# jeffpeterson/hypermerge

Hardware: AMD Instinct MI355X
Metric: merged changes/sec (1M docs×8 actors) at 1/2/4/8 GPUs + % HBM roofline (higher is better)
Workload: dtype u32; 1 GPU; C4: 1000000 docs/GPU x 8 actors x 64 changes/doc, map LWW sets; docs_per_gpu=1000000, changes_per_gpu=64000000, ops_per_gpu=96000538, parallelism=doc-shard1

## Files before the change

hypermerge_amd/csrc/engine.cpp:

```cpp
#include <hip/hip_runtime.h>
#include <cstdio>
#include <cstring>
#include <cstdlib>
#include <string>
#include <vector>
#include <algorithm>
#include <new>
#include "../../include/hypermerge_amd.h"
#include "merge_kernels.h"
#include "engine_internal.h"
#include "waiting_kernels.h"

struct hm_engine {
    int device = 0;
    int flags = 0;
    hipStream_t stream = nullptr;
    hipEvent_t ev[4] = {};
    float last_ms[2] = {0, 0};
    int n_last = 0;
    int num_cus = 256;
    std::string err;
    void *dbuf = nullptr;
    size_t dbuf_size = 0;
    void *pool = nullptr;
    size_t pool_size = 0;
    hipStream_t h2d = nullptr, d2h = nullptr;
    const char *last_scratch = nullptr;
};

namespace {

int fail(hm_engine *e, int status, const std::string &msg) {
    if (e) e->err = msg;
    return status;
}

int hip_fail(hm_engine *e, hipError_t r, const char *what) {
    return fail(e, HM_ERR_DEVICE, std::string(what) + ": " + hipGetErrorString(r));
}

#define HIPCHK(e, call)                                   \
    do {                                                  \
        hipError_t _r = (call);                           \
        if (_r != hipSuccess) return hip_fail(e, _r, #call); \
    } while (0)

struct Caps { uint32_t opl, cls; bool lists, counters; };

Caps launch_caps(const hm_batch *b) {
    Caps c;
    uint32_t mo = b->max_ops;
    c.opl = mo <= 64 ? 1 : (mo <= 128 ? 2 : (mo <= 192 ? 3 : 4));
    c.cls = (b->max_regs && b->max_objs && b->max_deps) ? hm_small_class(b->max_regs, b->max_objs, b->max_deps) : 1u;
    c.lists = (b->doc_flags & HM_DOC_HAS_LISTS) != 0;
    c.counters = (b->doc_flags & HM_DOC_HAS_COUNTERS) != 0;
    return c;
}

int launch_merge(hm_engine *e, const hm_batch *b, const hm_results *o, hipStream_t s, const uint32_t *doc_slot,
                 const hm_extents *ext, void *scratch, uint32_t *epos = nullptr) {
    Caps c = launch_caps(b);
    SmallParams p;
    p.res_epos = epos;
    p.docs = b->docs; p.changes = b->changes; p.deps = b->deps; p.ops = b->ops; p.min_clock = b->min_clock;
    p.res_docs = o->docs; p.res_clock = o->clock; p.res_back_clock = o->back_clock; p.res_heads = o->heads;
    p.res_hist = o->hist; p.res_all_deps = o->all_deps; p.res_regs = o->regs; p.res_surv = o->surv;
    p.n_docs = b->n_docs; p.a_stride = b->a_stride; p.cap_regs = 0; p.cap_objs = 0; p.cap_deps = 0;
    p.counters = c.counters ? 1u : 0u;
    p.general_only = (e->flags & HM_CFG_GENERAL_ONLY) ? 1u : 0u;
    {
        static const int remap = [] { const char *v = getenv("HM_XCD_REMAP"); return v ? atoi(v) : 1; }();
        p.xcd_remap = remap ? 1u : 0u;
    }
    p.doc_slot = doc_slot;
    p.lim_changes = ext ? ext->n_changes : b->n_changes; p.lim_deps = ext ? ext->n_deps : b->n_deps;
    p.lim_ops = ext ? ext->n_ops : b->n_ops; p.lim_regs = ext ? ext->n_regs : b->n_regs;
    if (b->n_docs == 0) { e->n_last = 0; return HM_OK; }
    const size_t list_bytes = ((size_t)b->n_docs * 4 + 255) & ~(size_t)255;
    const size_t need = hm_launch_scratch_bytes(b);
    const size_t pool_bytes = need - 256 - list_bytes;
    char *pb = (char *)scratch;
    if (!pb) {
        if (need > e->pool_size) {
            if (e->pool) { HIPCHK(e, hipDeviceSynchronize()); HIPCHK(e, hipFree(e->pool)); }
            e->pool = nullptr; e->pool_size = 0;
            if (hipMalloc(&e->pool, need) != hipSuccess) return fail(e, HM_ERR_NOMEM, "hipMalloc scratch pool");
            e->pool_size = need;
        }
        pb = (char *)e->pool;
    }
    p.large_cursor = (uint32_t *)pb;
    unsigned long long *pool_used = (unsigned long long *)(pb + 8);
    p.n_deferred = (uint32_t *)(pb + 16);
    p.deferred = (uint32_t *)(pb + 256);
    HIPCHK(e, hipMemsetAsync(pb, 0, 32, s));
    const uint32_t per_cu = hm_small_occupancy(c.opl, c.cls, c.lists, c.counters);
    uint32_t grid = std::min<uint32_t>(b->n_docs, (uint32_t)e->num_cus * per_cu);
    HIPCHK(e, hipEventRecord(e->ev[0], s));
    hipError_t r = hm_launch_small(p, c.opl, c.cls, c.lists, grid, s);
    if (r != hipSuccess) return hip_fail(e, r, "merge_small_kernel launch");
    HIPCHK(e, hipEventRecord(e->ev[1], s));
    HIPCHK(e, hipEventRecord(e->ev[2], s));
    r = hm_launch_large(p, pb + 256 + list_bytes, pool_bytes, pool_used, (uint32_t)e->num_cus * 4, s);
    if (r != hipSuccess) return hip_fail(e, r, "merge_large_kernel launch");
    HIPCHK(e, hipEventRecord(e->ev[3], s));
    e->n_last = 2;
    e->last_scratch = scratch ? nullptr : pb;
    return HM_OK;
}

}

size_t hm_launch_scratch_bytes(const hm_batch *b) {
    const size_t list_bytes = ((size_t)b->n_docs * 4 + 255) & ~(size_t)255;
    return 256 + list_bytes + hm_large_scratch_bound(b);
}

namespace {

uint32_t host_chunks(const hm_batch *b) {
    const uint32_t per = 1u << 16;
    if (b->n_docs < 2 * per || !b->docs || !b->changes || !b->ops) return 1;
    uint64_t c = 0, p = 0, o = 0, r = 0;
    for (uint32_t i = 0; i < b->n_docs; i++) {
        const hm_doc_row &d = b->docs[i];
        if (d.change_off != c || d.dep_off != p || d.op_off != o || d.reg_off != r) return 1;
        c += d.n_changes; p += d.n_deps; o += d.n_ops; r += d.n_regs;
    }
    if (c != b->n_changes || p != b->n_deps || o != b->n_ops) return 1;
    return std::min<uint32_t>(16, b->n_docs / per);
}

int check_batch(hm_engine *e, const hm_batch *b) {
    if (!b || b->a_stride == 0 || b->a_stride > HM_MAX_STRIDE) return fail(e, HM_ERR_INVALID, "a_stride must be in [1,256]");
    if (b->n_docs && !b->docs) return fail(e, HM_ERR_INVALID, "docs table missing");
    if ((b->n_changes && !b->changes) || (b->n_deps && !b->deps) || (b->n_ops && !b->ops))
        return fail(e, HM_ERR_INVALID, "row table missing");
    return HM_OK;
}

}

int hm_engine_launch_merge(hm_engine *e, const hm_batch *b, const hm_results *o, const uint32_t *doc_slot,
                           const hm_extents *ext, uint32_t *epos) {
    return launch_merge(e, b, o, e->stream, doc_slot, ext, nullptr, epos);
}
hipStream_t hm_engine_stream(hm_engine *e) { return e->stream; }
int hm_engine_device(hm_engine *e) { return e->device; }
int hm_engine_fail(hm_engine *e, int status, const char *msg) { return fail(e, status, msg); }

extern "C" {

uint32_t hm_abi_version(void) { return HM_ABI_VERSION; }

const char *hm_status_message(int status) {
    switch (status) {
    case HM_OK: return "ok";
    case HM_ERR_INCONSISTENT_SEQ: return "Inconsistent reuse of sequence number";
    case HM_ERR_UNKNOWN_OBJECT: return "Modification of unknown object";
    case HM_ERR_DUPLICATE_OBJECT: return "Duplicate creation of object";
    case HM_ERR_DUPLICATE_ELEM: return "Duplicate list element ID";
    case HM_ERR_MISSING_ELEM: return "Missing index entry for list element";
    case HM_ERR_UNSUPPORTED: return "document outside the engine envelope";
    case HM_ERR_INVALID: return "invalid batch";
    case HM_ERR_DEVICE: return "HIP device error";
    case HM_ERR_NOMEM: return "out of memory";
    default: return "unknown status";
    }
}

int hm_engine_create(const hm_config *cfg, hm_engine **out) {
    if (!out) return HM_ERR_INVALID;
    *out = nullptr;
    hm_engine *e = new (std::nothrow) hm_engine();
    if (!e) return HM_ERR_NOMEM;
    e->device = cfg ? cfg->device : 0;
    e->flags = cfg ? cfg->flags : 0;
    int n = 0;
    auto fail = [&](const char *what, hipError_t r) {
        fprintf(stderr, "hm_engine_create: %s failed: %s (device %d, %d devices)\n", what, hipGetErrorString(r), e->device, n);
        delete e;
        return HM_ERR_DEVICE;
    };
    hipError_t r = hipGetDeviceCount(&n);
    if (r != hipSuccess) return fail("hipGetDeviceCount", r);
    if (n <= e->device) return fail("device ordinal", hipErrorInvalidDevice);
    if ((r = hipSetDevice(e->device)) != hipSuccess) return fail("hipSetDevice", r);
    hipDeviceProp_t prop;
    if (hipGetDeviceProperties(&prop, e->device) == hipSuccess) e->num_cus = prop.multiProcessorCount;
    {
        size_t lim = 0, need = hm_large_stack_bytes();
        if (hipDeviceGetLimit(&lim, hipLimitStackSize) == hipSuccess && need > lim &&
            (r = hipDeviceSetLimit(hipLimitStackSize, need)) != hipSuccess) return fail("hipDeviceSetLimit(stack)", r);
    }
    if ((r = hipStreamCreateWithFlags(&e->stream, hipStreamNonBlocking)) != hipSuccess) return fail("hipStreamCreate", r);
    for (auto &ev : e->ev)
        if ((r = hipEventCreate(&ev)) != hipSuccess) return fail("hipEventCreate", r);
    *out = e;
    return HM_OK;
}

void hm_engine_destroy(hm_engine *e) {
    if (!e) return;
    (void)hipSetDevice(e->device);
    if (e->dbuf) (void)hipFree(e->dbuf);
    if (e->pool) (void)hipFree(e->pool);
    for (auto &ev : e->ev) if (ev) (void)hipEventDestroy(ev);
    if (e->stream) (void)hipStreamDestroy(e->stream);
    if (e->h2d) (void)hipStreamDestroy(e->h2d);
    if (e->d2h) (void)hipStreamDestroy(e->d2h);
    delete e;
}

const char *hm_engine_last_error(const hm_engine *e) { return e ? e->err.c_str() : "no engine"; }

size_t hm_scratch_bytes(const hm_batch *b) { return b ? hm_launch_scratch_bytes(b) : 0; }

int hm_merge_device(hm_engine *e, const hm_batch *b, const hm_results *o, void *scratch, void *stream) {
    try {
        if (!e || !o) return HM_ERR_INVALID;
        int st = check_batch(e, b);
        if (st) return st;
        if (b->n_docs && (!b->max_changes && !b->max_ops && !b->max_regs && !b->max_objs))
            return fail(e, HM_ERR_INVALID, "device batches must carry max_* launch hints");
        HIPCHK(e, hipSetDevice(e->device));
        return launch_merge(e, b, o, stream ? (hipStream_t)stream : e->stream, nullptr, nullptr, scratch);
    } catch (...) {
        return fail(e, HM_ERR_DEVICE, "exception in hm_merge_device");
    }
}

int hm_merge_host(hm_engine *e, const hm_batch *hb, const hm_results *ho) {
    try {
        if (!e || !hb || !ho) return HM_ERR_INVALID;
        int st = check_batch(e, hb);
        if (st) return st;
        HIPCHK(e, hipSetDevice(e->device));
        hm_batch b = *hb;
        if (!b.max_changes && !b.max_ops && !b.max_regs && !b.max_objs) {
            for (uint32_t d = 0; d < b.n_docs; d++) {
                b.max_changes = std::max(b.max_changes, hb->docs[d].n_changes);
                b.max_ops = std::max(b.max_ops, hb->docs[d].n_ops);
                b.max_regs = std::max(b.max_regs, hb->docs[d].n_regs);
                b.max_objs = std::max(b.max_objs, hb->docs[d].n_objs);
                b.max_deps = std::max(b.max_deps, hb->docs[d].n_deps);
                b.doc_flags |= hb->docs[d].flags;
            }
        }
        const size_t S = b.a_stride;
        struct Seg { size_t bytes; size_t off; };
        auto al = [](size_t x) { return (x + 255) & ~(size_t)255; };
        size_t sz[13] = {
            b.n_docs * sizeof(hm_doc_row), b.n_changes * sizeof(hm_change_row), b.n_deps * sizeof(hm_dep_row),
            b.n_ops * sizeof(hm_op_row), hb->min_clock ? b.n_docs * S * 4 : 0,
            b.n_docs * sizeof(hm_doc_result), b.n_docs * S * 4, b.n_docs * S * 4, b.n_docs * S * 4,
            b.n_changes * 4, b.n_changes * S * 4, b.n_regs * sizeof(hm_reg_result), b.n_ops * sizeof(hm_surv_result)};
        size_t off[13], total = 0;
        for (int i = 0; i < 13; i++) { off[i] = total; total += al(sz[i] ? sz[i] : 1); }
        if (total > e->dbuf_size) {
            if (e->dbuf) (void)hipFree(e->dbuf);
            e->dbuf = nullptr; e->dbuf_size = 0;
            if (hipMalloc(&e->dbuf, total) != hipSuccess) return fail(e, HM_ERR_NOMEM, "hipMalloc staging");
            e->dbuf_size = total;
        }
        char *base = (char *)e->dbuf;
        auto P = [&](int i) { return (void *)(base + off[i]); };
        hipStream_t s = e->stream;
        b.docs = (const hm_doc_row *)P(0); b.changes = (const hm_change_row *)P(1);
        b.deps = (const hm_dep_row *)P(2); b.ops = (const hm_op_row *)P(3);
        b.min_clock = hb->min_clock ? (const uint32_t *)P(4) : nullptr;
        hm_results d;
        d.docs = (hm_doc_result *)P(5); d.clock = (uint32_t *)P(6); d.back_clock = (uint32_t *)P(7);
        d.heads = (uint32_t *)P(8); d.hist = (int32_t *)P(9); d.all_deps = (uint32_t *)P(10);
        d.regs = (hm_reg_result *)P(11); d.surv = (hm_surv_result *)P(12);
        const void *src[5] = {hb->docs, hb->changes, hb->deps, hb->ops, hb->min_clock};
        void *dst[8] = {ho->docs, ho->clock, ho->back_clock, ho->heads, ho->hist, ho->all_deps, ho->regs, ho->surv};
        const uint32_t nchunk = host_chunks(hb);
        if (nchunk <= 1) {
            for (int i = 0; i < 5; i++)
                if (sz[i]) HIPCHK(e, hipMemcpyAsync(P(i), src[i], sz[i], hipMemcpyHostToDevice, s));
            if (sz[12]) HIPCHK(e, hipMemsetAsync(P(12), 0, sz[12], s));
            st = launch_merge(e, &b, &d, s, nullptr, nullptr, nullptr);
            if (st) return st;
            for (int i = 0; i < 8; i++)
                if (sz[5 + i] && dst[i]) HIPCHK(e, hipMemcpyAsync(dst[i], P(5 + i), sz[5 + i], hipMemcpyDeviceToHost, s));
            HIPCHK(e, hipStreamSynchronize(s));
            return HM_OK;
        }
        if (!e->h2d) HIPCHK(e, hipStreamCreateWithFlags(&e->h2d, hipStreamNonBlocking));
        if (!e->d2h) HIPCHK(e, hipStreamCreateWithFlags(&e->d2h, hipStreamNonBlocking));
        std::vector<hipEvent_t> evs(2 * nchunk, nullptr);
        int rc = HM_OK;
        auto cleanup = [&]() {
            (void)hipStreamSynchronize(e->h2d); (void)hipStreamSynchronize(s); (void)hipStreamSynchronize(e->d2h);
            for (auto ev : evs) if (ev) (void)hipEventDestroy(ev);
        };
        for (auto &ev : evs)
            if (hipEventCreateWithFlags(&ev, hipEventDisableTiming) != hipSuccess) { cleanup(); return fail(e, HM_ERR_DEVICE, "hipEventCreate"); }
        const hm_doc_row *hd = hb->docs;
        const uint32_t nd = b.n_docs;
        auto H2D = [&](void *dp, const void *hp, size_t bytes) {
            return bytes ? hipMemcpyAsync(dp, hp, bytes, hipMemcpyHostToDevice, e->h2d) : hipSuccess; };
        auto D2H = [&](void *hp, const void *dp, size_t bytes) {
            return (bytes && hp) ? hipMemcpyAsync(hp, dp, bytes, hipMemcpyDeviceToHost, e->d2h) : hipSuccess; };
#define HM_CK(x) do { hipError_t _r = (x); if (_r != hipSuccess) { rc = hip_fail(e, _r, #x); goto done; } } while (0)
        for (uint32_t k = 0; k < nchunk; k++) {
            const uint32_t d0 = (uint32_t)((uint64_t)nd * k / nchunk), d1 = (uint32_t)((uint64_t)nd * (k + 1) / nchunk);
            const uint32_t l = d1 - 1;
            const size_t c0 = hd[d0].change_off, c1 = (size_t)hd[l].change_off + hd[l].n_changes;
            const size_t p0 = hd[d0].dep_off, p1 = (size_t)hd[l].dep_off + hd[l].n_deps;
            const size_t o0 = hd[d0].op_off, o1 = (size_t)hd[l].op_off + hd[l].n_ops;
            const size_t r0 = hd[d0].reg_off, r1 = (size_t)hd[l].reg_off + hd[l].n_regs;
            char *dc = (char *)P(1), *dp = (char *)P(2), *dop = (char *)P(3);
            HM_CK(H2D((char *)P(0) + d0 * sizeof(hm_doc_row), hd + d0, (size_t)(d1 - d0) * sizeof(hm_doc_row)));
            HM_CK(H2D(dc + c0 * sizeof(hm_change_row), hb->changes + c0, (c1 - c0) * sizeof(hm_change_row)));
            HM_CK(H2D(dp + p0 * sizeof(hm_dep_row), hb->deps + p0, (p1 - p0) * sizeof(hm_dep_row)));
            HM_CK(H2D(dop + o0 * sizeof(hm_op_row), hb->ops + o0, (o1 - o0) * sizeof(hm_op_row)));
            if (hb->min_clock) HM_CK(H2D((char *)P(4) + d0 * S * 4, hb->min_clock + d0 * S, (d1 - d0) * S * 4));
            HM_CK(hipEventRecord(evs[2 * k], e->h2d));
            HM_CK(hipStreamWaitEvent(s, evs[2 * k], 0));
            HM_CK(hipMemsetAsync((char *)P(12) + o0 * sizeof(hm_surv_result), 0, (o1 - o0) * sizeof(hm_surv_result), s));
            {
                hm_batch cb = b;
                cb.n_docs = d1 - d0;
                cb.docs = b.docs + d0;
                cb.min_clock = b.min_clock ? b.min_clock + d0 * S : nullptr;
                hm_results co = d;
                co.docs = d.docs + d0; co.clock = d.clock + d0 * S; co.back_clock = d.back_clock + d0 * S;
                co.heads = d.heads + d0 * S;
                rc = launch_merge(e, &cb, &co, s, nullptr, nullptr, nullptr);
                if (rc) goto done;
            }
            HM_CK(hipEventRecord(evs[2 * k + 1], s));
            HM_CK(hipStreamWaitEvent(e->d2h, evs[2 * k + 1], 0));
            HM_CK(D2H(ho->docs ? ho->docs + d0 : nullptr, d.docs + d0, (size_t)(d1 - d0) * sizeof(hm_doc_result)));
            HM_CK(D2H(ho->clock ? ho->clock + d0 * S : nullptr, d.clock + d0 * S, (d1 - d0) * S * 4));
            HM_CK(D2H(ho->back_clock ? ho->back_clock + d0 * S : nullptr, d.back_clock + d0 * S, (d1 - d0) * S * 4));
            HM_CK(D2H(ho->heads ? ho->heads + d0 * S : nullptr, d.heads + d0 * S, (d1 - d0) * S * 4));
            HM_CK(D2H(ho->hist ? ho->hist + c0 : nullptr, d.hist + c0, (c1 - c0) * 4));
            HM_CK(D2H(ho->all_deps ? ho->all_deps + c0 * S : nullptr, d.all_deps + c0 * S, (c1 - c0) * S * 4));
            HM_CK(D2H(ho->regs ? ho->regs + r0 : nullptr, d.regs + r0, (r1 - r0) * sizeof(hm_reg_result)));
            HM_CK(D2H(ho->surv ? ho->surv + o0 : nullptr, d.surv + o0, (o1 - o0) * sizeof(hm_surv_result)));
        }
#undef HM_CK
    done:
        cleanup();
        return rc;
    } catch (...) {
        return fail(e, HM_ERR_DEVICE, "exception in hm_merge_host");
    }
}

static int check_waiting_batch(hm_engine *e, const hm_batch *b) {
    if (!b || b->a_stride == 0 || b->a_stride > HM_MAX_STRIDE) return fail(e, HM_ERR_INVALID, "a_stride must be in [1,256]");
    if ((b->n_docs && !b->docs) || (b->n_changes && !b->changes) || (b->n_deps && !b->deps))
        return fail(e, HM_ERR_INVALID, "row table missing");
    return HM_OK;
}

int hm_missing_deps_device(hm_engine *e, const hm_batch *b, const hm_results *r, uint32_t *out_missing, void *stream) {
    try {
        if (!e || !r) return HM_ERR_INVALID;
        int st = check_waiting_batch(e, b);
        if (st) return st;
        if (!b->n_docs) return HM_OK;
        if (!out_missing || !r->docs || !r->clock || (b->n_changes && !r->hist))
            return fail(e, HM_ERR_INVALID, "hm_missing_deps needs the results' docs, clock and hist tables");
        HIPCHK(e, hipSetDevice(e->device));
        hipError_t hr = hm_launch_waiting_batch(b, r, out_missing, stream ? (hipStream_t)stream : e->stream);
        return hr == hipSuccess ? HM_OK : hip_fail(e, hr, "waiting_batch_kernel launch");
    } catch (...) {
        return fail(e, HM_ERR_DEVICE, "exception in hm_missing_deps_device");
    }
}

int hm_missing_deps_host(hm_engine *e, const hm_batch *hb, const hm_results *hr, uint32_t *out_missing) {
    try {
        if (!e || !hr) return HM_ERR_INVALID;
        int st = check_waiting_batch(e, hb);
        if (st) return st;
        if (!hb->n_docs) return HM_OK;
        if (!out_missing || !hr->docs || !hr->clock || (hb->n_changes && !hr->hist))
            return fail(e, HM_ERR_INVALID, "hm_missing_deps needs the results' docs, clock and hist tables");
        HIPCHK(e, hipSetDevice(e->device));
        const size_t S = hb->a_stride, n = hb->n_docs;
        auto al = [](size_t x) { return (x + 255) & ~(size_t)255; };
        const size_t sz[7] = {n * sizeof(hm_doc_row), hb->n_changes * sizeof(hm_change_row), hb->n_deps * sizeof(hm_dep_row),
                              n * sizeof(hm_doc_result), n * S * 4, (size_t)hb->n_changes * 4, n * S * 4};
        const void *src[6] = {hb->docs, hb->changes, hb->deps, hr->docs, hr->clock, hr->hist};
        size_t off[7], total = 0;
        for (int i = 0; i < 7; i++) { off[i] = total; total += al(sz[i] ? sz[i] : 1); }
        char *base = nullptr;
        if (hipMalloc((void **)&base, total) != hipSuccess) return fail(e, HM_ERR_NOMEM, "hipMalloc missing-deps staging");
        hipStream_t s = e->stream;
        hm_batch b = *hb;
        b.docs = (const hm_doc_row *)(base + off[0]); b.changes = (const hm_change_row *)(base + off[1]);
        b.deps = (const hm_dep_row *)(base + off[2]);
        hm_results d = {};
        d.docs = (hm_doc_result *)(base + off[3]); d.clock = (uint32_t *)(base + off[4]); d.hist = (int32_t *)(base + off[5]);
        hipError_t r = hipSuccess;
        for (int i = 0; i < 6 && r == hipSuccess; i++)
            if (sz[i]) r = hipMemcpyAsync(base + off[i], src[i], sz[i], hipMemcpyHostToDevice, s);
        if (r == hipSuccess) r = hm_launch_waiting_batch(&b, &d, (uint32_t *)(base + off[6]), s);
        if (r == hipSuccess) r = hipMemcpyAsync(out_missing, base + off[6], sz[6], hipMemcpyDeviceToHost, s);
        if (r == hipSuccess) r = hipStreamSynchronize(s);
        (void)hipFree(base);
        return r == hipSuccess ? HM_OK : hip_fail(e, r, "hm_missing_deps_host");
    } catch (...) {
        return fail(e, HM_ERR_DEVICE, "exception in hm_missing_deps_host");
    }
}

int hm_last_kernel_ms(hm_engine *e, float *ms, int max_kernels) {
    if (!e || !ms) return 0;
    int n = std::min(max_kernels, e->n_last);
    for (int i = 0; i < n; i++) {
        if (hipEventSynchronize(e->ev[2 * i + 1]) != hipSuccess) return 0;
        if (hipEventElapsedTime(&ms[i], e->ev[2 * i], e->ev[2 * i + 1]) != hipSuccess) return 0;
    }
    return n;
}

int hm_last_deferred(hm_engine *e, uint32_t *out_docs, uint32_t cap) {
    if (!e) return -HM_ERR_INVALID;
    if (e->n_last < 2) return 0;
    if (!e->last_scratch) return -fail(e, HM_ERR_INVALID, "the last launch used caller scratch: its deferred list is the caller's");
    if (hipEventSynchronize(e->ev[3]) != hipSuccess) return -HM_ERR_DEVICE;
    uint32_t n = 0;
    if (hipMemcpy(&n, e->last_scratch + 16, 4, hipMemcpyDeviceToHost) != hipSuccess) return -HM_ERR_DEVICE;
    const uint32_t k = std::min(n, cap);
    if (k && out_docs && hipMemcpy(out_docs, e->last_scratch + 256, (size_t)k * 4, hipMemcpyDeviceToHost) != hipSuccess)
        return -HM_ERR_DEVICE;
    return (int)n;
}

int hm_clock_cmp_device(hm_engine *e, const uint32_t *a, const uint32_t *b, uint8_t *out, uint32_t n_docs,
                        uint32_t a_stride, void *stream) {
    if (!e) return HM_ERR_INVALID;
    hipError_t r = hm_launch_clock(0, a, b, out, n_docs, a_stride, stream ? (hipStream_t)stream : e->stream);
    return r == hipSuccess ? HM_OK : hip_fail(e, r, "clock_cmp");
}

int hm_clock_union_device(hm_engine *e, const uint32_t *a, const uint32_t *b, uint32_t *c, uint32_t n_docs,
                          uint32_t a_stride, void *stream) {
    if (!e) return HM_ERR_INVALID;
    hipError_t r = hm_launch_clock(1, a, b, c, n_docs, a_stride, stream ? (hipStream_t)stream : e->stream);
    return r == hipSuccess ? HM_OK : hip_fail(e, r, "clock_union");
}

int hm_clock_intersection_device(hm_engine *e, const uint32_t *a, const uint32_t *b, uint32_t *c,
                                 uint32_t n_docs, uint32_t a_stride, void *stream) {
    if (!e) return HM_ERR_INVALID;
    hipError_t r = hm_launch_clock(2, a, b, c, n_docs, a_stride, stream ? (hipStream_t)stream : e->stream);
    return r == hipSuccess ? HM_OK : hip_fail(e, r, "clock_intersection");
}

}
```

hypermerge_amd/csrc/merge_kernels.h:

```cpp
#pragma once
#include <hip/hip_runtime.h>
#include "../../include/hypermerge_amd.h"

struct SmallParams {
    const hm_doc_row *docs;
    const hm_change_row *changes;
    const hm_dep_row *deps;
    const hm_op_row *ops;
    const uint32_t *min_clock;
    hm_doc_result *res_docs;
    uint32_t *res_clock, *res_back_clock, *res_heads;
    int32_t *res_hist;
    uint32_t *res_all_deps;
    hm_reg_result *res_regs;
    hm_surv_result *res_surv;
    uint32_t n_docs, a_stride;
    uint32_t cap_regs, cap_objs;
    uint32_t cap_deps;
    uint32_t counters;
    uint32_t *large_cursor;
    uint32_t *n_deferred;
    uint32_t *deferred;
    uint32_t general_only;
    uint32_t xcd_remap;
    const uint32_t *doc_slot;
    uint32_t lim_changes, lim_deps, lim_ops, lim_regs;
    uint32_t *res_epos;
};
#ifdef __HIPCC__
__device__ __forceinline__ bool hm_doc_row_ok(const SmallParams &p, const hm_doc_row &d) {
    return (unsigned long long)d.change_off + d.n_changes <= p.lim_changes &&
           (unsigned long long)d.dep_off + d.n_deps <= p.lim_deps &&
           (unsigned long long)d.op_off + d.n_ops <= p.lim_ops &&
           (unsigned long long)d.reg_off + d.n_regs <= p.lim_regs && d.n_actors <= p.a_stride;
}
#endif
#ifdef __HIPCC__
__device__ __forceinline__ uint32_t hm_slot(const SmallParams &p, uint32_t d) { return p.doc_slot ? p.doc_slot[d] : d; }
#endif

#define HM_DEFERRED 0x7FFFFFFF

size_t hm_launch_scratch_bytes(const hm_batch *b);

size_t hm_large_scratch_bound(const hm_batch *b);
size_t hm_large_stack_bytes();
hipError_t hm_launch_large(const SmallParams &p, void *pool, size_t pool_bytes, unsigned long long *pool_used,
                           uint32_t grid, hipStream_t s);
uint32_t hm_small_class(uint32_t max_regs, uint32_t max_objs, uint32_t max_deps);
size_t hm_small_lds_bytes(uint32_t opl, uint32_t cls, bool lists, bool counters);
uint32_t hm_small_occupancy(uint32_t opl, uint32_t cls, bool lists, bool counters);
hipError_t hm_launch_small(const SmallParams &p, uint32_t opl, uint32_t cls, bool lists, uint32_t grid, hipStream_t s);
hipError_t hm_launch_clock(int which, const uint32_t *a, const uint32_t *b, void *out, uint32_t n_docs,
                           uint32_t S, hipStream_t s);
```

hypermerge_amd/csrc/merge_kernels.hip:

```cpp
#include <hip/hip_runtime.h>
#include <stdint.h>
#include "../../include/hypermerge_amd.h"
#include "merge_kernels.h"

#ifndef HM_ABLATE
#define HM_ABLATE 0
#endif
#ifndef HM_STAMPS
#define HM_STAMPS 0
#endif
#define HM_NSTAMP 20
#ifndef HM_PREFETCH_EARLY
#define HM_PREFETCH_EARLY 0
#endif
#ifndef HM_WAVES_PER_EU_OPL4
#define HM_WAVES_PER_EU_OPL4 3
#endif
#ifndef HM_WAVES_PER_EU_LIST3
#define HM_WAVES_PER_EU_LIST3 3
#endif
#ifndef HM_PRIO_PUSH
#define HM_PRIO_PUSH 2
#endif
#ifndef HM_PRIO_IO
#define HM_PRIO_IO 1
#endif
#ifndef HM_PRIO_HIST
#define HM_PRIO_HIST 3
#endif
#ifndef HM_PRIO_RANK
#define HM_PRIO_RANK 2
#endif
#ifndef HM_PRIO_FOLD
#define HM_PRIO_FOLD 0
#endif
#ifndef HM_PRIO_K3
#define HM_PRIO_K3 0
#endif
#ifndef HM_PRIO_K2
#define HM_PRIO_K2 2
#endif
#ifndef HM_PUSH_BPERM
#define HM_PUSH_BPERM 0
#endif
#ifndef HM_KARG_RELOAD
#define HM_KARG_RELOAD 1
#endif
#ifndef HM_HIST_DP
#define HM_HIST_DP 1
#endif
#ifndef HM_HIST_REGS
#define HM_HIST_REGS 1
#endif
#ifndef HM_PRIO_K1
#define HM_PRIO_K1 3
#endif
#ifndef HM_FENCE_MCMP
#define HM_FENCE_MCMP 1
#endif
#ifndef HM_STAGE_FIRST
#define HM_STAGE_FIRST 0
#endif
#ifndef HM_ASYNC_NEXT
#define HM_ASYNC_NEXT 1
#endif
#ifndef HM_ASYNC_MAX_OPL
#define HM_ASYNC_MAX_OPL 2
#endif
#ifndef HM_ASYNC_STORES
#define HM_ASYNC_STORES 10
#endif
#ifndef HM_NT_OUT
#define HM_NT_OUT 0
#endif
#ifndef HM_NT_IN
#define HM_NT_IN 0
#endif
#ifndef HM_ASYNC_CHECK
#define HM_ASYNC_CHECK 0
#endif
#ifndef HM_OPAQUE_LANE
#define HM_OPAQUE_LANE 1
#endif
#ifndef HM_WAVES_PER_EU
#define HM_WAVES_PER_EU 4
#endif
#define WAVE 64
#define NA_MAX 8
#define NDEP_MAX 1024
typedef unsigned long long u64;
#if defined(__HIP_DEVICE_COMPILE__)
#define LDS __attribute__((address_space(3)))
#else
#define LDS
#endif

namespace hm {

__device__ __forceinline__ u64 readlane64(u64 v, int l) {
    const uint32_t lo = __builtin_amdgcn_readlane((int)(uint32_t)v, l);
    const uint32_t hi = __builtin_amdgcn_readlane((int)(uint32_t)(v >> 32), l);
    return ((u64)hi << 32) | lo;
}
__device__ __forceinline__ uint32_t shfl32(uint32_t v, int src) {
    return (uint32_t)__builtin_amdgcn_ds_bpermute(src << 2, (int)v);
}
__device__ __forceinline__ u64 shfl64(u64 v, int src) {
    return ((u64)shfl32((uint32_t)(v >> 32), src) << 32) | shfl32((uint32_t)v, src);
}
__device__ __forceinline__ u64 wave_or64(u64 v) {
    for (int o = 1; o < WAVE; o <<= 1) v |= shfl64(v, (int)(threadIdx.x ^ o));
    return v;
}
#define DPP_ROW_SHR(n) (0x110 + (n))
#define DPP_WAVE_SHR1 0x138
#define DPP_ROW_BCAST15 0x142
#define DPP_ROW_BCAST31 0x143
__device__ __forceinline__ uint32_t wave_excl_scan(uint32_t v, uint32_t *total) {
    uint32_t x = v;
    x += (uint32_t)__builtin_amdgcn_update_dpp(0, (int)x, DPP_ROW_SHR(1), 0xF, 0xF, false);
    x += (uint32_t)__builtin_amdgcn_update_dpp(0, (int)x, DPP_ROW_SHR(2), 0xF, 0xF, false);
    x += (uint32_t)__builtin_amdgcn_update_dpp(0, (int)x, DPP_ROW_SHR(4), 0xF, 0xF, false);
    x += (uint32_t)__builtin_amdgcn_update_dpp(0, (int)x, DPP_ROW_SHR(8), 0xF, 0xF, false);
    x += (uint32_t)__builtin_amdgcn_update_dpp(0, (int)x, DPP_ROW_BCAST15, 0xA, 0xF, false);
    x += (uint32_t)__builtin_amdgcn_update_dpp(0, (int)x, DPP_ROW_BCAST31, 0xC, 0xF, false);
    *total = (uint32_t)__builtin_amdgcn_readlane((int)x, WAVE - 1);
    return x - v;
}
__device__ __forceinline__ uint32_t wave_max(uint32_t v) {
    uint32_t x = v, y;
    y = (uint32_t)__builtin_amdgcn_update_dpp(0, (int)x, DPP_ROW_SHR(1), 0xF, 0xF, false); x = x > y ? x : y;
    y = (uint32_t)__builtin_amdgcn_update_dpp(0, (int)x, DPP_ROW_SHR(2), 0xF, 0xF, false); x = x > y ? x : y;
    y = (uint32_t)__builtin_amdgcn_update_dpp(0, (int)x, DPP_ROW_SHR(4), 0xF, 0xF, false); x = x > y ? x : y;
    y = (uint32_t)__builtin_amdgcn_update_dpp(0, (int)x, DPP_ROW_SHR(8), 0xF, 0xF, false); x = x > y ? x : y;
    y = (uint32_t)__builtin_amdgcn_update_dpp(0, (int)x, DPP_ROW_BCAST15, 0xA, 0xF, false); x = x > y ? x : y;
    y = (uint32_t)__builtin_amdgcn_update_dpp(0, (int)x, DPP_ROW_BCAST31, 0xC, 0xF, false); x = x > y ? x : y;
    return (uint32_t)__builtin_amdgcn_readlane((int)x, WAVE - 1);
}
__device__ __forceinline__ uint32_t bytesum64(u64 x) {
    return __builtin_amdgcn_sad_u8((uint32_t)x, 0u, __builtin_amdgcn_sad_u8((uint32_t)(x >> 32), 0u, 0u));
}
__device__ __forceinline__ uint32_t prev_lane(uint32_t v) {
    return (uint32_t)__builtin_amdgcn_update_dpp(0, (int)v, DPP_WAVE_SHR1, 0xF, 0xF, false);
}
__device__ __forceinline__ uint32_t fresh_lane() {
#if HM_OPAQUE_LANE
    uint32_t l;
    asm volatile("v_mov_b32 %0, %1" : "=v"(l) : "v"((uint32_t)threadIdx.x));
    return l;
#else
    return threadIdx.x;
#endif
}
__device__ __forceinline__ void wave_sync() {
    __builtin_amdgcn_fence(__ATOMIC_SEQ_CST, "wavefront");
    __builtin_amdgcn_wave_barrier();
}

__device__ __forceinline__ u64 err_key(uint32_t h, uint32_t op_plus1, uint32_t arr, uint32_t code) {
    return ((u64)h << 40) | ((u64)(op_plus1 & 0xFFFF) << 24) | ((u64)(arr & 0xFFFF) << 8) | code;
}

struct SmallLds {
    LDS u64 *anc, *chain, *segor, *errkey, *cov;
    LDS u64 *opval;
    LDS u64 *survpk;
    LDS int64_t *survsum;
    LDS uint32_t *first, *base, *bclock, *headv, *objslot, *segcnt, *survcnt, *regoff, *regobj, *insmin;
    LDS uint32_t *flags, *deps, *depinfo;
    LDS uint8_t *seglist;
    LDS uint16_t *survp;
    LDS uint32_t *opmeta;
    LDS uint32_t *opro;
    LDS uint32_t *opelem;
    LDS int32_t *hist_of;
    LDS uint16_t *survop, *opbase, *oppar;
    LDS uint8_t *h2a, *chactor, *objtype;
    LDS uint16_t *opchg;
    LDS uint32_t *nins, *pcount, *nodekey, *tour0, *listbase;
    LDS uint16_t *poff;
    LDS uint16_t *nodeop, *nodepi, *regnode, *plist, *fc, *ns, *listid;
    LDS u64 *stamps;
};
#define PAR_HEAD 0xFFFFu

template <int CLS> struct SizeClass;
template <> struct SizeClass<0> { static constexpr uint32_t NR = 32, NO = 16, ND = 128; };
template <> struct SizeClass<1> { static constexpr uint32_t NR = 256, NO = 64, ND = 512; };
template <> struct SizeClass<2> { static constexpr uint32_t NR = 128, NO = 32, ND = 256; };

template <typename L_t, typename P>
__host__ __device__ inline size_t small_carve(P base, uint32_t NOp, uint32_t NR, uint32_t NO, uint32_t ND,
                                              bool lists, bool counters, L_t *L) {
    size_t o = 0;
#define TAKE(f, T, cnt) do { L->f = (decltype(L->f))(base + o); o = (o + (size_t)(cnt) * sizeof(T) + 15) & ~(size_t)15; } while (0)
    TAKE(anc, u64, 64);          TAKE(chain, u64, NA_MAX);     TAKE(opval, u64, NOp);
    TAKE(errkey, u64, 1);        TAKE(base, uint32_t, NA_MAX * 3);
    TAKE(survcnt, uint32_t, NR); TAKE(regoff, uint32_t, NR);   TAKE(regobj, uint32_t, NR);
    TAKE(insmin, uint32_t, NR);  TAKE(flags, uint32_t, 2);
    TAKE(opmeta, uint32_t, NOp); TAKE(opro, uint32_t, NOp);
    TAKE(survop, uint16_t, NOp); TAKE(chactor, uint8_t, 64);   TAKE(objtype, uint8_t, NO);
    if (lists) {
        TAKE(opelem, uint32_t, NOp);
        L->nodekey = L->opelem;
        TAKE(nins, uint32_t, 1);
    }
    TAKE(stamps, u64, HM_STAMPS ? HM_NSTAMP + 1 : 0);
    const size_t dead_at = o;
    TAKE(hist_of, int32_t, 64);  TAKE(cov, u64, 1);            TAKE(opbase, uint16_t, 64);
    TAKE(oppar, uint16_t, NOp);  TAKE(h2a, uint8_t, 64);       TAKE(opchg, uint16_t, NOp);
    const size_t k1_at = o;
    TAKE(first, uint32_t, NA_MAX * 64);
    TAKE(deps, uint32_t, ND > NOp ? ND : NOp);
    TAKE(depinfo, uint32_t, ND);
    const size_t k1_end = o;
    o = k1_at;
    TAKE(segor, u64, NR);        TAKE(survpk, u64, NR);        TAKE(segcnt, uint32_t, NR);
    TAKE(objslot, uint32_t, NO);
    if (o < k1_end) o = k1_end;
    L->seglist = (decltype(L->seglist))L->first; L->survp = (decltype(L->survp))L->first;
    if (lists) {
        const uint32_t NP = NR + NO, NE = 2 * (NOp + NO);
        size_t q = dead_at;
#define TAKEK(f, T, cnt) do { L->f = (decltype(L->f))(base + q); q = (q + (size_t)(cnt) * sizeof(T) + 15) & ~(size_t)15; } while (0)
        TAKEK(tour0, uint32_t, NE);     TAKEK(pcount, uint32_t, NP);  TAKEK(listbase, uint32_t, NO + 1);
        TAKEK(poff, uint16_t, NP + 1);  TAKEK(survp, uint16_t, NOp);
        TAKEK(nodeop, uint16_t, NOp);   TAKEK(nodepi, uint16_t, NOp); TAKEK(regnode, uint16_t, NR);
        TAKEK(plist, uint16_t, NOp);    TAKEK(fc, uint16_t, NP);      TAKEK(ns, uint16_t, NOp);
        TAKEK(listid, uint16_t, NO);    TAKEK(seglist, uint8_t, NOp);
#undef TAKEK
        if (q > o) o = q;
    }
    TAKE(survsum, int64_t, counters ? NOp : 0);
#undef TAKE
    L->bclock = L->base + NA_MAX;
    L->headv = L->base + 2 * NA_MAX;
    return o;
}

template <typename T> struct Id { typedef T type; };
template <typename T> __device__ __forceinline__ T lds_or(LDS T *p, typename Id<T>::type v) { return __atomic_fetch_or(p, v, __ATOMIC_RELAXED); }
template <typename T> __device__ __forceinline__ T lds_min(LDS T *p, typename Id<T>::type v) { return __atomic_fetch_min(p, v, __ATOMIC_RELAXED); }
template <typename T> __device__ __forceinline__ T lds_max(LDS T *p, typename Id<T>::type v) { return __atomic_fetch_max(p, v, __ATOMIC_RELAXED); }
template <typename T> __device__ __forceinline__ T lds_add(LDS T *p, typename Id<T>::type v) { return __atomic_fetch_add(p, v, __ATOMIC_RELAXED); }

#if HM_STAMPS
__device__ unsigned long long hm_stamp_acc[HM_NSTAMP];
__device__ __forceinline__ u64 stamp_now() {
    u64 t;
    __builtin_amdgcn_sched_barrier(0);
    asm volatile("s_memtime %0\n\ts_waitcnt lgkmcnt(0)" : "=s"(t) :: "memory");
    __builtin_amdgcn_sched_barrier(0);
    return t;
}
#define STAMP(L_, i) do { const u64 t_ = stamp_now(); if (threadIdx.x == 0) { (L_).stamps[i] += t_ - (L_).stamps[HM_NSTAMP]; (L_).stamps[HM_NSTAMP] = t_; } } while (0)
#elif defined(HM_MARKS)
#define STAMP(L_, i) asm volatile(";HMMARK " #i)
#else
#define STAMP(L_, i) do { } while (0)
#endif

enum : uint32_t { FL_UNSUPPORTED = 1u };
enum Outcome { OUT_OK = 0, OUT_ERROR = 1, OUT_UNSUPPORTED = 2, OUT_INVALID = 3 };

__device__ __forceinline__ void need_set(uint32_t &lo, uint32_t &hi, uint32_t a, uint32_t v) {
    const uint32_t sh = (a & 3) * 8;
    const uint32_t w = a < 4 ? lo : hi;
    const uint32_t cur = (w >> sh) & 0xFF;
    const uint32_t nw = v > cur ? ((w & ~(0xFFu << sh)) | (v << sh)) : w;
    lo = a < 4 ? nw : lo;
    hi = a < 4 ? hi : nw;
}


__device__ __forceinline__ uint32_t fidx(uint32_t a, uint32_t s) { return (s & 63) * NA_MAX + (a & (NA_MAX - 1)); }
__device__ __forceinline__ void clear_first(LDS uint32_t *first) {
    static_assert(NA_MAX * 64 == 2 * WAVE * 4, "first-table size");
    LDS uint4 *f4 = (LDS uint4 *)first;
    const uint4 ones = make_uint4(~0u, ~0u, ~0u, ~0u);
    f4[threadIdx.x] = ones;
    f4[threadIdx.x + WAVE] = ones;
}

__device__ __forceinline__ uint32_t tie_order(uint32_t pc) { return (pc & 1) ? (0x10000u - pc) : (0x20000u + pc); }


template <int OPL>
__device__ __forceinline__ void rga_order(const SmallLds &L, uint32_t R, uint32_t O,
                                          const uint32_t (&oreg)[OPL], const uint32_t (&oobj)[OPL],
                                          const uint32_t (&opar)[OPL], const uint32_t (&oact)[OPL],
                                          const uint32_t (&oelem)[OPL], const uint32_t (&oarr)[OPL],
                                          const int32_t (&oh)[OPL], uint32_t *epos) {
    const uint32_t lane = threadIdx.x;
    const uint32_t NP = R + O;
    constexpr uint32_t END = 0xFFFFu;
    for (uint32_t i = lane; i < NP; i += WAVE) { L.pcount[i] = 0; L.fc[i] = 0xFFFFu; }
    for (uint32_t i = lane; i < R; i += WAVE) L.regnode[i] = 0xFFFFu;
    if (lane == 0) *L.nins = 0;
    uint32_t nl = 0;
    for (uint32_t o0 = 0; o0 < O; o0 += WAVE) {
        const uint32_t o = o0 + lane;
        const uint32_t ot = o < O ? L.objtype[o] : 0xFFu;
        const bool isl = ot == HM_MAKE_LIST || ot == HM_MAKE_TEXT;
        const u64 mk = __ballot(isl);
        if (o < O) L.listid[o] = isl ? (uint16_t)(nl + __popcll(mk & ((1ull << lane) - 1))) : (uint16_t)0xFFFFu;
        nl += (uint32_t)__popcll(mk);
    }
    wave_sync();
#pragma unroll
    for (int t = 0; t < OPL; t++) {
        if (oh[t] < 0 || oact[t] != HM_INS) continue;
        const uint32_t i = lds_add(L.nins, 1u);
        const uint32_t pi = opar[t] == HM_HEAD ? R + oobj[t] : opar[t];
        L.nodeop[i] = (uint16_t)(lane + WAVE * t);
        L.nodepi[i] = (uint16_t)pi;
        L.nodekey[i] = (oelem[t] << 8) | L.chactor[oarr[t]];
        L.regnode[oreg[t]] = (uint16_t)i;
        lds_add(&L.pcount[pi], 1u);
    }
    wave_sync();
    STAMP(L, 16);
    const uint32_t N = *L.nins;
    uint32_t tot = 0;
    for (uint32_t r0 = 0; r0 < NP; r0 += WAVE) {
        const uint32_t r = r0 + lane;
        uint32_t tt;
        const uint32_t ex = wave_excl_scan(r < NP ? L.pcount[r] : 0u, &tt);
        if (r < NP) L.poff[r] = tot + ex;
        tot += tt;
    }
    if (lane == 0) L.poff[NP] = tot;
    wave_sync();
    for (uint32_t i = lane; i < N; i += WAVE) {
        const uint32_t pi = L.nodepi[i];
        L.plist[L.poff[pi] + lds_add(&L.pcount[pi], 0xFFFFFFFFu) - 1u] = (uint16_t)i;
    }
    wave_sync();
    for (uint32_t i = lane; i < N; i += WAVE) {
        const uint32_t pi = L.nodepi[i], key = L.nodekey[i];
        const uint32_t q0 = L.poff[pi], qn = L.poff[pi + 1] - q0;
        uint32_t best = 0xFFFFu, bkey = 0;
        bool firstc = true;
        for (uint32_t q = 0; q < qn; q++) {
            const uint32_t j = L.plist[q0 + q], kj = L.nodekey[j];
            if (kj > key) firstc = false;
            else if (kj < key && (best == 0xFFFFu || kj > bkey)) { best = j; bkey = kj; }
        }
        L.ns[i] = (uint16_t)best;
        if (firstc) L.fc[pi] = (uint16_t)i;
    }
    wave_sync();
    STAMP(L, 17);
    const uint32_t E = 2 * (N + nl);
    for (uint32_t i = lane; i < N; i += WAVE) {
        const uint32_t reg = (L.opro[L.nodeop[i]] & 0xFFFFu);
        const uint32_t hd = N + L.listid[L.regobj[reg]];
        const uint32_t f = L.fc[reg];
        const uint32_t sd = f != 0xFFFFu ? 2 * f : 2 * i + 1;
        const uint32_t pi = L.nodepi[i];
        const uint32_t su = L.ns[i] != 0xFFFFu ? 2u * L.ns[i] : (pi >= R ? 2 * hd + 1 : 2u * L.regnode[pi] + 1);
        L.tour0[2 * i] = (sd << 16) | 1u;
        L.tour0[2 * i + 1] = su << 16;
    }
    for (uint32_t o = lane; o < O; o += WAVE) {
        const uint32_t l = L.listid[o];
        if (l == 0xFFFFu) continue;
        const uint32_t h = N + l, f = L.fc[R + o];
        L.tour0[2 * h] = (f != 0xFFFFu ? 2 * f : 2 * h + 1) << 16;
        L.tour0[2 * h + 1] = END << 16;
    }
    wave_sync();
    LDS uint32_t *cur = L.tour0;
    const uint32_t rounds = E ? (33 - __builtin_clz(E)) / 2 : 0;
    for (uint32_t rd = 0; rd < rounds; rd++) {
        for (uint32_t e = lane; e < E; e += WAVE) {
            const uint32_t x = cur[e];
            uint32_t nx = x >> 16, sum = x & 0xFFFFu;
#pragma unroll
            for (int hop = 0; hop < 3; hop++) {
                if (nx == END) break;
                const uint32_t y = cur[nx];
                sum += y & 0xFFFFu;
                nx = y >> 16;
            }
            cur[e] = (nx << 16) | sum;
        }
        wave_sync();
    }
    STAMP(L, 18);
    uint32_t lb = 0;
    for (uint32_t l0 = 0; l0 < nl; l0 += WAVE) {
        const uint32_t l = l0 + lane;
        uint32_t tt;
        const uint32_t ex = wave_excl_scan(l < nl ? (cur[2 * (N + l)] & 0xFFFFu) : 0u, &tt);
        if (l < nl) L.listbase[l] = lb + ex;
        lb += tt;
    }
    wave_sync();
    for (uint32_t i = lane; i < N; i += WAVE) {
        const uint32_t reg = (L.opro[L.nodeop[i]] & 0xFFFFu);
        const uint32_t l = L.listid[L.regobj[reg]];
        const uint32_t total = cur[2 * (N + l)] & 0xFFFFu;
        const uint32_t pos = L.listbase[l] + total - (cur[2 * i] & 0xFFFFu);
        L.seglist[pos] = L.survcnt[reg] > 0 ? 1u : 0u;
        L.nodekey[i] = pos;
        if (epos) epos[reg] = pos - L.listbase[l];
        L.insmin[reg] = 0xFFFFFFFFu;
    }
    wave_sync();
    uint32_t vc = 0;
    for (uint32_t q0 = 0; q0 < N; q0 += WAVE) {
        const uint32_t q = q0 + lane;
        uint32_t tt;
        const uint32_t ex = wave_excl_scan(q < N ? L.seglist[q] : 0u, &tt);
        if (q < N) L.survp[q] = vc + ex;
        vc += tt;
    }
    wave_sync();
    for (uint32_t i = lane; i < N; i += WAVE) {
        const uint32_t reg = (L.opro[L.nodeop[i]] & 0xFFFFu);
        const uint32_t pos = L.nodekey[i];
        if (L.seglist[pos]) {
            const uint32_t l = L.listid[L.regobj[reg]];
            const uint32_t first_pos = L.listbase[l];
            L.insmin[reg] = L.survp[pos] - (first_pos < N ? L.survp[first_pos] : vc);
        }
    }
    wave_sync();
    STAMP(L, 19);
}


struct FoldView {
    LDS u64 *anc, *chain;
    LDS uint32_t *first, *base, *deps;
    LDS int32_t *hist_of;
};
__device__ __forceinline__ uint32_t fc_of(FoldView L, uint32_t h, uint32_t x) {
    return (uint32_t)__popcll((L.anc[h] | (1ull << h)) & L.chain[x]);
}
__device__ __forceinline__ uint32_t hpos_of(FoldView L, uint32_t a, uint32_t s) {
    return (uint32_t)L.hist_of[L.first[fidx(a, (s - L.base[a]))]];
}
__device__ __noinline__ bool fold_differs(FoldView L, uint32_t dep0, uint32_t nd, uint32_t actor, uint32_t seq) {
    uint32_t ex[NA_MAX + 1], es[NA_MAX + 1], eh[NA_MAX + 1], k = 0;
    bool own = false;
    for (uint32_t j = 0; j < nd && k < NA_MAX; j++) {
        const uint32_t pk = L.deps[dep0 + j];
        uint32_t a = pk >> 24, sq = pk & 0xFFFFFF;
        if (a == actor) { sq = seq - 1; own = true; }
        if (sq == 0) continue;
        ex[k] = a; es[k] = sq; eh[k] = hpos_of(L, a, sq); k++;
    }
    if (!own && seq > 1) { ex[k] = actor; es[k] = seq - 1; eh[k] = hpos_of(L, actor, seq - 1); k++; }
    for (uint32_t j = 0; j < k; j++) {
        uint32_t before = 0, after = 0;
        for (uint32_t i = 0; i < k; i++) {
            if (i == j) continue;
            const uint32_t f = fc_of(L, eh[i], ex[j]);
            if (i < j) before = before > f ? before : f; else after = after > f ? after : f;
        }
        if (before > (es[j] > after ? es[j] : after)) return true;
    }
    return false;
}

struct Rows {
    uint4 c01;
    uint2 c2;
    uint4 a0, b0, a1, b1, a2, b2, a3, b3;
    uint2 d0, d1;
};
__device__ __forceinline__ bool check_doc(const SmallParams &p, hm_doc_row &r) {
    const bool ok = hm_doc_row_ok(p, r);
    if (!ok) r = hm_doc_row{};
    return ok;
}
__device__ __forceinline__ void load_op(const SmallParams &p, const hm_doc_row &doc, uint32_t k, uint4 &a, uint4 &b) {
    a = make_uint4(0, 0, 0, 0); b = a;
    if (k < doc.n_ops) {
        const uint4 *src = reinterpret_cast<const uint4 *>(p.ops + doc.op_off + k);
        a = src[0]; b = src[1];
    }
}
template <int OPL>
__device__ __forceinline__ Rows load_rows(const SmallParams &p, const hm_doc_row &doc) {
    const uint32_t lane = threadIdx.x;
    Rows r;
    r.c01 = make_uint4(0, 0, 0, 0);
    r.c2 = r.d0 = r.d1 = make_uint2(0, 0);
    if (lane < doc.n_changes) {
        const uint2 *cs = reinterpret_cast<const uint2 *>(p.changes + doc.change_off + lane);
        const uint2 x0 = cs[0], x1 = cs[1];
        r.c01 = make_uint4(x0.x, x0.y, x1.x, x1.y); r.c2 = cs[2];
    }
    load_op(p, doc, lane, r.a0, r.b0);
    if (OPL > 1) load_op(p, doc, lane + WAVE, r.a1, r.b1);
    if (OPL > 2) load_op(p, doc, lane + 2 * WAVE, r.a2, r.b2);
    if (OPL > 3) load_op(p, doc, lane + 3 * WAVE, r.a3, r.b3);
    const hm_dep_row *dp = p.deps + doc.dep_off;
    if (lane < doc.n_deps) r.d0 = *reinterpret_cast<const uint2 *>(dp + lane);
    if (lane + WAVE < doc.n_deps) r.d1 = *reinterpret_cast<const uint2 *>(dp + lane + WAVE);
    return r;
}
#if HM_ASYNC_CHECK
__device__ unsigned long long hm_async_checked, hm_async_bad;
template <int OPL>
__device__ __forceinline__ void async_check(const SmallParams &p, const hm_doc_row &doc, const Rows &got) {
    const Rows want = load_rows<OPL>(p, doc);
    auto ne4 = [](uint4 a, uint4 b) { return a.x != b.x || a.y != b.y || a.z != b.z || a.w != b.w; };
    auto ne2 = [](uint2 a, uint2 b) { return a.x != b.x || a.y != b.y; };
    bool bad = ne4(want.c01, got.c01) || ne2(want.c2, got.c2) || ne4(want.a0, got.a0) || ne4(want.b0, got.b0) ||
               ne2(want.d0, got.d0) || ne2(want.d1, got.d1);
    if (OPL > 1) bad = bad || ne4(want.a1, got.a1) || ne4(want.b1, got.b1);
    if (OPL > 2) bad = bad || ne4(want.a2, got.a2) || ne4(want.b2, got.b2);
    if (OPL > 3) bad = bad || ne4(want.a3, got.a3) || ne4(want.b3, got.b3);
    const unsigned long long m = __ballot(bad);
    if (threadIdx.x == 0) {
        atomicAdd(&hm_async_checked, 1ull);
        if (m) atomicAdd(&hm_async_bad, 1ull);
    }
}
#endif
#if HM_ASYNC_NEXT
typedef uint32_t u32x2 __attribute__((ext_vector_type(2)));
typedef uint32_t u32x4 __attribute__((ext_vector_type(4)));
struct AsyncRows { u32x2 c0, c1, c2; u32x4 a0, b0, a1, b1, a2, b2, a3, b3; u32x2 d0, d1; };
#if HM_NT_IN
#define HM_AL_POL " nt"
#else
#define HM_AL_POL ""
#endif
__device__ __forceinline__ u32x2 aload2(const void *p) {
    u32x2 v;
    asm volatile("global_load_dwordx2 %0, %1, off" HM_AL_POL : "=v"(v) : "v"(p) : "memory");
    return v;
}
__device__ __forceinline__ u32x4 aload4(const void *p) {
    u32x4 v;
    asm volatile("global_load_dwordx4 %0, %1, off" HM_AL_POL : "=v"(v) : "v"(p) : "memory");
    return v;
}
template <int OPL>
__device__ __forceinline__ AsyncRows load_rows_async(const SmallParams &p, const hm_doc_row &doc) {
    const uint32_t lane = threadIdx.x;
    AsyncRows r;
    r.c0 = r.c1 = r.c2 = r.d0 = r.d1 = u32x2{0u, 0u};
    r.a0 = r.b0 = r.a1 = r.b1 = r.a2 = r.b2 = r.a3 = r.b3 = u32x4{0u, 0u, 0u, 0u};
    if (doc.n_changes) {
        const uint32_t i = lane < doc.n_changes ? lane : doc.n_changes - 1u;
        const uint2 *cs = reinterpret_cast<const uint2 *>(p.changes + doc.change_off + i);
        r.c0 = aload2(cs); r.c1 = aload2(cs + 1); r.c2 = aload2(cs + 2);
    }
    if (doc.n_ops) {
        const uint32_t i0 = lane < doc.n_ops ? lane : doc.n_ops - 1u;
        const uint4 *o0 = reinterpret_cast<const uint4 *>(p.ops + doc.op_off + i0);
        r.a0 = aload4(o0); r.b0 = aload4(o0 + 1);
        if (OPL > 1) {
            const uint32_t i1 = lane + WAVE < doc.n_ops ? lane + WAVE : doc.n_ops - 1u;
            const uint4 *o1 = reinterpret_cast<const uint4 *>(p.ops + doc.op_off + i1);
            r.a1 = aload4(o1); r.b1 = aload4(o1 + 1);
        }
        if (OPL > 2) {
            const uint32_t i2 = lane + 2 * WAVE < doc.n_ops ? lane + 2 * WAVE : doc.n_ops - 1u;
            const uint4 *o2 = reinterpret_cast<const uint4 *>(p.ops + doc.op_off + i2);
            r.a2 = aload4(o2); r.b2 = aload4(o2 + 1);
        }
        if (OPL > 3) {
            const uint32_t i3 = lane + 3 * WAVE < doc.n_ops ? lane + 3 * WAVE : doc.n_ops - 1u;
            const uint4 *o3 = reinterpret_cast<const uint4 *>(p.ops + doc.op_off + i3);
            r.a3 = aload4(o3); r.b3 = aload4(o3 + 1);
        }
    }
    if (doc.n_deps) {
        const uint32_t i0 = lane < doc.n_deps ? lane : doc.n_deps - 1u, i1 = lane + WAVE < doc.n_deps ? lane + WAVE : doc.n_deps - 1u;
        r.d0 = aload2(p.deps + doc.dep_off + i0); r.d1 = aload2(p.deps + doc.dep_off + i1);
    }
    return r;
}
template <int OPL>
__device__ __forceinline__ Rows take_rows_async(AsyncRows &r, const hm_doc_row &doc, bool padded) {
#define HM_AW2 "+v"(r.c0), "+v"(r.c1), "+v"(r.c2), "+v"(r.a0), "+v"(r.b0), "+v"(r.a1), "+v"(r.b1), "+v"(r.d0), "+v"(r.d1)
#define HM_AW3 HM_AW2, "+v"(r.a2), "+v"(r.b2)
#define HM_AW4 HM_AW3, "+v"(r.a3), "+v"(r.b3)
    if constexpr (OPL <= 2) {
        if (padded) asm volatile("s_waitcnt vmcnt(%9)" : HM_AW2 : "n"(HM_ASYNC_STORES) : "memory");
        else asm volatile("s_waitcnt vmcnt(0)" : HM_AW2 :: "memory");
    } else if constexpr (OPL == 3) {
        if (padded) asm volatile("s_waitcnt vmcnt(%11)" : HM_AW3 : "n"(HM_ASYNC_STORES) : "memory");
        else asm volatile("s_waitcnt vmcnt(0)" : HM_AW3 :: "memory");
    } else {
        if (padded) asm volatile("s_waitcnt vmcnt(%13)" : HM_AW4 : "n"(HM_ASYNC_STORES) : "memory");
        else asm volatile("s_waitcnt vmcnt(0)" : HM_AW4 :: "memory");
    }
#undef HM_AW4
#undef HM_AW3
#undef HM_AW2
    const uint32_t lane = threadIdx.x;
    Rows o;
    const bool c = lane < doc.n_changes, k0 = lane < doc.n_ops, k1 = lane + WAVE < doc.n_ops;
    o.c01 = c ? make_uint4(r.c0.x, r.c0.y, r.c1.x, r.c1.y) : make_uint4(0u, 0u, 0u, 0u);
    o.c2 = c ? make_uint2(r.c2.x, r.c2.y) : make_uint2(0u, 0u);
    o.a0 = k0 ? make_uint4(r.a0.x, r.a0.y, r.a0.z, r.a0.w) : make_uint4(0u, 0u, 0u, 0u);
    o.b0 = k0 ? make_uint4(r.b0.x, r.b0.y, r.b0.z, r.b0.w) : make_uint4(0u, 0u, 0u, 0u);
    o.a1 = k1 ? make_uint4(r.a1.x, r.a1.y, r.a1.z, r.a1.w) : make_uint4(0u, 0u, 0u, 0u);
    o.b1 = k1 ? make_uint4(r.b1.x, r.b1.y, r.b1.z, r.b1.w) : make_uint4(0u, 0u, 0u, 0u);
    const bool k2 = lane + 2 * WAVE < doc.n_ops, k3 = lane + 3 * WAVE < doc.n_ops;
    o.a2 = k2 ? make_uint4(r.a2.x, r.a2.y, r.a2.z, r.a2.w) : make_uint4(0u, 0u, 0u, 0u);
    o.b2 = k2 ? make_uint4(r.b2.x, r.b2.y, r.b2.z, r.b2.w) : make_uint4(0u, 0u, 0u, 0u);
    o.a3 = k3 ? make_uint4(r.a3.x, r.a3.y, r.a3.z, r.a3.w) : make_uint4(0u, 0u, 0u, 0u);
    o.b3 = k3 ? make_uint4(r.b3.x, r.b3.y, r.b3.z, r.b3.w) : make_uint4(0u, 0u, 0u, 0u);
    o.d0 = lane < doc.n_deps ? make_uint2(r.d0.x, r.d0.y) : make_uint2(0u, 0u);
    o.d1 = lane + WAVE < doc.n_deps ? make_uint2(r.d1.x, r.d1.y) : make_uint2(0u, 0u);
    return o;
}
#endif
__device__ __forceinline__ u64 op_value(const SmallLds &L, uint32_t k) { return L.opval[k]; }
__device__ __forceinline__ uint32_t pack_dep(uint2 w) {
    const uint32_t a = w.x & 0xFFFF;
    return (w.y < (1u << 24) && a < 256) ? ((a << 24) | w.y) : 0xFFFFFFFFu;
}
template <bool LISTS>
__device__ __forceinline__ void stage_op(const SmallLds &L, uint32_t k, uint32_t m, uint4 a, uint4 b) {
    if (k >= m) return;
    const uint32_t obj = a.x < 0xFFFFu ? a.x : 0xFFFFu, reg = a.y < 0xFFFFu ? a.y : 0xFFFFu;
    L.opro[k] = reg | (obj << 16);
    L.oppar[k] = (uint16_t)(a.z == HM_HEAD ? PAR_HEAD : (a.z < 0xFFFEu ? a.z : 0xFFFEu));
    L.opmeta[k] = b.x & 0xFFFFFFu;
    L.opval[k] = ((u64)b.w << 32) | b.z;
    if (LISTS) L.opelem[k] = a.w;
}
template <int OPL, bool LISTS>
__device__ __forceinline__ void stage_rows(const SmallParams &p, const SmallLds &L, const hm_doc_row &doc, const Rows &r,
                                           uint32_t cap_deps) {
    const uint32_t lane = threadIdx.x, m = doc.n_ops;
    stage_op<LISTS>(L, lane, m, r.a0, r.b0);
    if (OPL > 1) stage_op<LISTS>(L, lane + WAVE, m, r.a1, r.b1);
    if (OPL > 2) stage_op<LISTS>(L, lane + 2 * WAVE, m, r.a2, r.b2);
    if (OPL > 3) stage_op<LISTS>(L, lane + 3 * WAVE, m, r.a3, r.b3);
    const uint32_t nd = doc.n_deps < cap_deps ? doc.n_deps : cap_deps;
    if (lane < nd) L.deps[lane] = pack_dep(r.d0);
    if (lane + WAVE < nd) L.deps[lane + WAVE] = pack_dep(r.d1);
    for (uint32_t i = lane + 2 * WAVE; i < nd; i += WAVE)
        L.deps[i] = pack_dep(*reinterpret_cast<const uint2 *>(p.deps + doc.dep_off + i));
}
__device__ __forceinline__ hm_change_row change_of(uint2 w0, uint2 w1, uint2 w2) {
    hm_change_row c;
    c.actor = (uint16_t)(w0.x & 0xFFFF); c.n_deps = (uint16_t)(w0.x >> 16); c.seq = w0.y;
    c.dep_off = w1.x; c.n_ops = w1.y; c.op_first = w2.x; c.content_id = w2.y;
    return c;
}
struct DocState {
    int32_t hist;
    uint32_t H, total;
    bool doc_lists;
};

struct OpCheck { uint32_t err; bool surv, has_list, late; };
__device__ __forceinline__ OpCheck op_check(const SmallLds &L, int32_t ohv, uint32_t act, uint32_t obj, uint32_t reg,
                                            uint32_t par, uint32_t okey, uint32_t R, uint32_t O) {
    const bool asg = ohv >= 0 && act >= HM_INS && act <= HM_INC && reg < R;
    const uint32_t oi = obj < O ? obj : 0u, ri = reg < R ? reg : 0u;
    const uint32_t pi = par < R ? par : 0u;
    const uint32_t os = obj < O ? L.objslot[oi] : 0xFFFFFFFFu;
    const uint32_t ot = L.objtype[oi], im = L.insmin[ri], ip = L.insmin[pi];
    const u64 so = L.segor[ri];
    const uint32_t h = ohv < 0 ? 0u : (uint32_t)ohv;
    const bool unknown = asg && (os == 0xFFFFFFFFu || os > okey);
    const bool known = asg && !unknown;
    const bool is_list = ot == HM_MAKE_LIST || ot == HM_MAKE_TEXT;
    const bool ins = known && act == HM_INS;
    const bool sl = known && (act == HM_SET || act == HM_LINK);
    OpCheck r;
    r.has_list = ins || (known && is_list);
    r.surv = sl && !((so >> h) & 1);
    r.late = ins && par != HM_HEAD && !(ip <= okey);
    uint32_t e = 0;
    if (sl && is_list && !(im <= okey)) e = HM_ERR_MISSING_ELEM;
    if (ins && im != okey + 1) e = HM_ERR_DUPLICATE_ELEM;
    if (unknown) e = HM_ERR_UNKNOWN_OBJECT;
    r.err = e;
    return r;
}

template <int OPL, bool LISTS>
__device__ __forceinline__ Outcome merge_doc_small(const SmallParams &p, const SmallLds &L, const hm_doc_row &doc,
                                                   const uint2 w0, const uint2 w1, const uint2 w2, DocState &st) {
    const uint32_t lane = threadIdx.x;
    const uint32_t n = doc.n_changes, A = doc.n_actors, m = doc.n_ops, R = doc.n_regs, O = doc.n_objs;
    st.hist = -1; st.H = 0; st.total = 0; st.doc_lists = false;

    if (HM_ABLATE & 8) return OUT_UNSUPPORTED;
    STAMP(L, 0);
    if (HM_PRIO_K1) __builtin_amdgcn_s_setprio(HM_PRIO_K1);
    const bool act = lane < n;
    const hm_change_row c = change_of(w0, w1, w2);
    clear_first(L.first);
    if (lane < NA_MAX) { L.base[lane] = 0xFFFFFFFFu; L.bclock[lane] = 0; L.headv[lane] = 0; L.chain[lane] = 0; }
    if (lane == 0) { *L.errkey = ~0ull; L.flags[0] = 0; L.flags[1] = 0; *L.cov = 0; }
    const uint32_t dep_lo = doc.dep_off, ndep = doc.n_deps;
    wave_sync();
    const uint32_t actor = c.actor, seq = c.seq;
    const uint32_t my_dep0 = c.dep_off - dep_lo;
    const uint32_t op_end = c.op_first + c.n_ops, dep_end = c.dep_off + c.n_deps;
    const uint32_t prev_op = prev_lane(op_end), prev_dep = prev_lane(dep_end);
    bool bad = (n == 0 && (m || ndep)) ||
               (act && (c.op_first != (lane ? prev_op : doc.op_off) || c.dep_off != (lane ? prev_dep : dep_lo) ||
                        (lane == n - 1 && (op_end != doc.op_off + m || dep_end != dep_lo + ndep))));
    const bool rowok = act && !(actor >= A || seq == 0 || c.dep_off < dep_lo || my_dep0 + c.n_deps > ndep);
    bad |= act && !rowok;
    bad |= act && (c.op_first < doc.op_off || c.op_first - doc.op_off + c.n_ops > m);
    const uint32_t a8 = actor & (NA_MAX - 1);
    lds_min(&L.base[a8], rowok ? seq : 0xFFFFFFFFu);
    lds_max(&L.bclock[a8], rowok ? seq : 0u);
    L.chactor[lane] = (uint8_t)actor;
    L.opbase[lane] = (uint16_t)(c.op_first - doc.op_off);
    if (__ballot(bad)) return OUT_UNSUPPORTED;
    wave_sync();
    const uint32_t mybase = act ? L.base[a8] : 0;
    const uint32_t slot = seq - mybase;
    if (__ballot(act && slot >= 64)) return OUT_UNSUPPORTED;
    lds_min(&L.first[fidx(a8, (slot & 63))], act ? lane : 0xFFFFFFFFu);
    {
        const uint32_t o0 = c.op_first - doc.op_off;
        if (act) for (uint32_t j = 0; j < c.n_ops; j++) L.opchg[o0 + j] = (uint16_t)(lane | (a8 << 8));
    }
    wave_sync();

    STAMP(L, 1);
    if (HM_ABLATE & 16) return OUT_UNSUPPORTED;
    {
        bool bad_dep = false;
        for (uint32_t i = lane; i < ndep; i += WAVE) {
            const uint32_t pk = L.deps[i];
            const uint32_t a = pk >> 24, s = pk & 0xFFFFFF;
            bad_dep |= pk == 0xFFFFFFFFu || a >= A;
            const uint32_t ad = a & (NA_MAX - 1);
            const uint32_t b = L.base[ad];
            const bool inwin = b != 0xFFFFFFFFu && s >= b && s - b < 64;
            const uint32_t f = L.first[fidx(ad, ((s - b) & 63))];
            const uint32_t rel = s == 0 ? 0u : (inwin ? s - b + 1 : 0x7Fu);
            L.depinfo[i] = (inwin && f < 64 ? f : 0x7Fu) | (rel << 8) | (ad << 16);
        }
        if (__ballot(bad_dep)) return OUT_UNSUPPORTED;
    }
    const uint32_t first_me = act ? L.first[fidx(actor, slot)] : lane;
    const bool dup = act && first_me != lane;
    const uint32_t cid_first = shfl32(c.content_id, (int)(first_me & 63));
    u64 dmask = 0;
    uint32_t pred_arr = 0xFFu;
    bool ok = true;
    bool own_row = false;
    wave_sync();
    {
        const uint32_t maxd = wave_max(act ? (uint32_t)c.n_deps : 0u);
        for (uint32_t j0 = 0; j0 < maxd; j0 += 2) {
            uint32_t inf[2];
#pragma unroll
            for (int u = 0; u < 2; u++) {
                const bool live = act && j0 + u < c.n_deps;
                inf[u] = L.depinfo[live ? my_dep0 + j0 + u : 0u];
            }
#pragma unroll
            for (int u = 0; u < 2; u++) {
                const bool live = act && j0 + u < c.n_deps;
                const uint32_t a = (inf[u] >> 16) & (NA_MAX - 1), rel = (inf[u] >> 8) & 0x7F, f = inf[u] & 0x7F;
                own_row |= live && a == actor;
                const bool use = live && a != actor && rel != 0;
                ok = ok && !(use && (rel == 0x7F || f >= lane));
                dmask |= (use && rel != 0x7F && f < lane) ? (1ull << f) : 0ull;
            }
        }
        const uint32_t ps = seq - 1;
        const bool hp = act && ps != 0, inb = ps >= mybase;
        const uint32_t f = L.first[fidx(a8, ((ps - mybase) & 63))];
        ok = ok && !(hp && (!inb || f >= lane));
        const bool pv = hp && inb && f < lane;
        dmask |= pv ? (1ull << (f & 63)) : 0ull;
        pred_arr = pv ? f : pred_arr;
        ok = ok && !(dup && cid_first != c.content_id);
    }
    wave_sync();

    STAMP(L, 2);
    if (HM_ABLATE & 32) return OUT_UNSUPPORTED;
    int32_t hist = -1;
    uint32_t H = 0;
    bool identity = false;
    if (HM_PRIO_K1) __builtin_amdgcn_s_setprio(0);
    const bool queued_doc = __ballot(act && !ok) != 0;
    if (HM_PRIO_HIST && queued_doc) __builtin_amdgcn_s_setprio(HM_PRIO_HIST);
    if (!queued_doc) {
        const u64 appl = __ballot(act && !dup);
        if (act) hist = dup ? -2 : (int32_t)__popcll(appl & ((1ull << lane) - 1));
        H = (uint32_t)__popcll(appl);
        identity = __ballot(dup) == 0;
    } else if (__ballot(dup && cid_first != c.content_id) == 0) {
        u64 dall = 0;
        bool never = false;
        uint32_t pred_any = 0xFFu;
        {
            const uint32_t maxd = wave_max(act ? (uint32_t)c.n_deps : 0u);
            for (uint32_t j = 0; j < maxd; j++) {
                const bool live = act && j < c.n_deps;
                const uint32_t inf = L.depinfo[live ? my_dep0 + j : 0u];
                const uint32_t a = (inf >> 16) & (NA_MAX - 1), rel = (inf >> 8) & 0x7F, f = inf & 0x7F;
                const bool use = live && a != actor && rel != 0;
                never |= use && (rel == 0x7F || f == 0x7F);
                dall |= (use && rel != 0x7F && f != 0x7F) ? (1ull << f) : 0ull;
            }
            const uint32_t ps = seq - 1;
            const bool hp = act && ps != 0, inb = ps >= mybase;
            const uint32_t f = L.first[fidx(a8, ((ps - mybase) & 63))];
            never |= hp && (!inb || f >= 64);
            dall |= (hp && inb && f < 64) ? (1ull << f) : 0ull;
            pred_any = (hp && inb && f < 64) ? f : 0xFFu;
        }
        const u64 dupm = __ballot(dup), nodupm = __ballot(act && !dup);
        const u64 below = (1ull << lane) - 1;
        const uint32_t key = first_me & 63;
        u64 applied = 0, queue = 0;
        bool copy_applied = false;
        bool solved = false;
        if (HM_HIST_DP) {
            LDS uint32_t *tx = (LDS uint32_t *)L.hist_of;
            LDS uint32_t *tm = (LDS uint32_t *)L.anc;
            const uint32_t INF = 0xFFu;
            const bool has_dup = dupm != 0;
            const bool kl = act && !dup;
            uint32_t t = (!kl || never) ? INF : lane;
            const bool regdp = HM_HIST_REGS && __ballot(act && __popcll(dall) > 4) == 0;
            uint32_t sl0 = lane, sl1 = lane, sl2 = lane, sl3 = lane;
            if (regdp) {
                u64 m = dall;
                sl0 = m ? (uint32_t)__builtin_ctzll(m) : lane; m &= m - 1;
                sl1 = m ? (uint32_t)__builtin_ctzll(m) : lane; m &= m - 1;
                sl2 = m ? (uint32_t)__builtin_ctzll(m) : lane; m &= m - 1;
                sl3 = m ? (uint32_t)__builtin_ctzll(m) : lane;
                for (uint32_t it = 0; it <= n; it++) {
                    const uint32_t x0 = shfl32(t, (int)sl0), x1 = shfl32(t, (int)sl1);
                    const uint32_t x2 = shfl32(t, (int)sl2), x3 = shfl32(t, (int)sl3);
                    uint32_t nt = t;
                    nt = nt > x0 ? nt : x0; nt = nt > x1 ? nt : x1; nt = nt > x2 ? nt : x2; nt = nt > x3 ? nt : x3;
                    nt = (kl && t != INF) ? nt : t;
                    const bool grew = nt != t;
                    t = nt;
                    if (__ballot(grew) == 0) break;
                }
            } else {
                for (uint32_t it = 0; it <= n; it++) {
                    tx[lane] = t;
                    wave_sync();
                    uint32_t nt = t;
                    if (kl && t != INF)
                        for (u64 m = dall; m; m &= m - 1) { const uint32_t x = tx[__builtin_ctzll(m)]; nt = nt > x ? nt : x; }
                    wave_sync();
                    const bool grew = nt != t;
                    t = nt;
                    if (__ballot(grew) == 0) break;
                }
            }
            STAMP(L, 13);
            tx[lane] = t;
            wave_sync();
            const uint32_t tk = act ? tx[key] : INF;
            wave_sync();
            uint32_t w = (!kl || t == INF) ? 0xFFFFFFFFu : ((t << 16) | ((t == lane ? 1u : 2u) << 8) | lane);
            bool conv = false;
            if (regdp) {
                const bool queued_copy = act && tk != INF && tk != key && lane < tk;
                const uint32_t nsl = (uint32_t)__popcll(dall);
                for (uint32_t it = 0; it <= n + 1; it++) {
                    const uint32_t y0 = shfl32(w, (int)sl0), y1 = shfl32(w, (int)sl1);
                    const uint32_t y2 = shfl32(w, (int)sl2), y3 = shfl32(w, (int)sl3);
                    uint32_t pc = 2;
                    auto fold = [&](uint32_t wd, uint32_t k) {
                        const uint32_t v = ((wd >> 8) & 0xFFu) + ((wd & 0xFFu) > lane ? 1u : 0u);
                        pc = (k < nsl && (wd >> 16) == tk && v > pc) ? v : pc;
                    };
                    fold(y0, 0); fold(y1, 1); fold(y2, 2); fold(y3, 3);
                    const uint32_t cand = queued_copy ? ((tk << 16) | ((pc > 0xFEu ? 0xFEu : pc) << 8) | lane) : 0xFFFFFFFFu;
                    uint32_t nw = w;
                    if (has_dup) {
                        tm[lane] = 0xFFFFFFFFu;
                        wave_sync();
                        if (cand != 0xFFFFFFFFu) lds_min(&tm[key], cand);
                        wave_sync();
                        if (kl && t != INF && t != lane) nw = tm[lane];
                    } else if (kl && t != INF && t != lane) nw = cand;
                    const bool grew = nw != w;
                    w = nw;
                    if (__ballot(grew) == 0) { conv = true; break; }
                }
            }
            for (uint32_t it = 0; !regdp && it <= n + 1; it++) {
                tx[lane] = w;
                if (has_dup) tm[lane] = 0xFFFFFFFFu;
                wave_sync();
                uint32_t cand = 0xFFFFFFFFu;
                if (act && tk != INF && tk != key && lane < tk) {
                    uint32_t pc = 2;
                    for (u64 m = dall; m; m &= m - 1) {
                        const uint32_t wd = tx[__builtin_ctzll(m)];
                        if ((wd >> 16) == tk) {
                            const uint32_t v = ((wd >> 8) & 0xFFu) + ((wd & 0xFFu) > lane ? 1u : 0u);
                            pc = pc > v ? pc : v;
                        }
                    }
                    cand = (tk << 16) | ((pc > 0xFEu ? 0xFEu : pc) << 8) | lane;
                }
                wave_sync();
                uint32_t nw = w;
                if (has_dup) {
                    if (cand != 0xFFFFFFFFu) lds_min(&tm[key], cand);
                    wave_sync();
                    if (kl && t != INF && t != lane) nw = tm[lane];
                } else if (kl && t != INF && t != lane) nw = cand;
                const bool grew = nw != w;
                w = nw;
                if (__ballot(grew) == 0) { conv = true; break; }
            }
            STAMP(L, 14);
            tx[lane] = w;
            wave_sync();
            const uint32_t wk = act && tk != INF ? tx[key] : 0xFFFFFFFFu;
            const bool apl = wk != 0xFFFFFFFFu && (wk & 0xFFu) == lane;
            const uint32_t hk = apl ? wk : 0xFFFFFFFFu;
            bool bad = false;
            if (apl)
                for (u64 m = dall; m; m &= m - 1) bad |= tx[__builtin_ctzll(m)] >= hk;
            wave_sync();
            if (conv && __ballot(bad) == 0) {
                const u64 A = __ballot(apl);
                u64 eq = apl ? A : 0ull;
                uint32_t rank = 0;
                const uint32_t tmax = wave_max(apl ? (hk >> 16) : 0u), pmax = wave_max(apl ? ((hk >> 8) & 0xFFu) : 0u);
                auto rbit = [&](uint32_t b) {
                    const bool one = (hk >> b) & 1u;
                    const u64 B = __ballot(apl && one);
                    rank += one ? (uint32_t)__popcll(eq & ~B) : 0u;
                    eq &= one ? B : ~B;
                };
                for (int b = 16 + (31 - __builtin_clz(tmax | 1u)); b >= 16; b--) rbit((uint32_t)b);
                for (int b = 8 + (31 - __builtin_clz(pmax | 1u)); b >= 8; b--) rbit((uint32_t)b);
                rank += (uint32_t)__popcll(eq & below);
                hist = apl ? (int32_t)rank : (act && tk != INF ? -2 : -1);
                H = (uint32_t)__popcll(__ballot(apl));
                if (apl && dup) L.first[fidx(a8, (slot & 63))] = lane;
                copy_applied = __ballot(apl && dup) != 0;
                solved = true;
            }
            STAMP(L, 15);
        }
        for (uint32_t i = 0; i < n && !solved; i++) {
            queue |= 1ull << i;
            u64 P = __ballot(lane == i && !never && (dall & ~applied) == 0);
            while (P) {
                u64 ap = P & nodupm & ~applied, keys = ap;
                for (u64 dm = P & dupm; dm; dm &= dm - 1) {
                    const uint32_t d = (uint32_t)__builtin_ctzll(dm);
                    const uint32_t kd = (uint32_t)__builtin_amdgcn_readlane((int)key, (int)d);
                    if (!((applied | keys) >> kd & 1)) {
                        ap |= 1ull << d; keys |= 1ull << kd; copy_applied = true;
                        if (lane == d) L.first[fidx(a8, (slot & 63))] = lane;
                    }
                }
                if ((P >> lane) & 1) hist = ((ap >> lane) & 1) ? (int32_t)(H + (uint32_t)__popcll(ap & below)) : -2;
                H += (uint32_t)__popcll(ap);
                applied |= keys;
                queue &= ~P;
                u64 np = 0;
                for (;;) {
                    u64 kb = np & nodupm & below;
                    for (u64 dm = np & dupm; dm; dm &= dm - 1) {
                        const uint32_t d = (uint32_t)__builtin_ctzll(dm);
                        const uint32_t kd = (uint32_t)__builtin_amdgcn_readlane((int)key, (int)d);
                        kb |= d < lane ? (1ull << kd) : 0ull;
                    }
                    const u64 nx = __ballot(((queue >> lane) & 1) && !never && ((dall & ~applied) & ~kb) == 0);
                    if (nx == np) break;
                    np = nx;
                }
                P = np;
            }
        }
        const bool ap = act && hist >= 0;
        dmask = ap ? dall : 0ull;
        pred_arr = ap ? pred_any : 0xFFu;
        if (copy_applied) {
            wave_sync();
            dmask = 0; pred_arr = 0xFFu;
            if (ap) {
                for (uint32_t j = 0; j < c.n_deps; j++) {
                    const uint32_t pk = L.deps[my_dep0 + j];
                    const uint32_t a = pk >> 24, s = pk & 0xFFFFFF;
                    if (a == actor || s == 0) continue;
                    dmask |= 1ull << L.first[fidx(a, (s - L.base[a]))];
                }
                if (seq - 1 != 0) { pred_arr = L.first[fidx(actor, (seq - 1 - mybase))]; dmask |= 1ull << pred_arr; }
            }
        }
    } else {
        uint32_t need_lo = 0, need_hi = 0;
        if (act) {
            for (uint32_t j = 0; j < c.n_deps; j++) {
                const uint32_t inf = L.depinfo[my_dep0 + j];
                const uint32_t a = (inf >> 16) & (NA_MAX - 1), rel = (inf >> 8) & 0x7F;
                need_set(need_lo, need_hi, a, (a != actor && rel != 0) ? rel : 0u);
            }
            const uint32_t ps = seq - 1;
            need_set(need_lo, need_hi, a8, ps != 0 ? (ps >= mybase ? ps - mybase + 1 : 0x7Fu) : 0u);
        }
        clear_first(L.first);
        wave_sync();
        uint32_t crel_lo = 0, crel_hi = 0;
        u64 queued = 0;
        bool stop = false;
        for (uint32_t i = 0; i < n && !stop; i++) {
            queued |= 1ull << i;
            u64 above = 0;
            bool first_pass = true;
            for (;;) {
                bool progress = false;
                for (;;) {
                    const uint32_t x0 = ((crel_lo | 0x80808080u) - need_lo) & 0x80808080u;
                    const uint32_t x1 = ((crel_hi | 0x80808080u) - need_hi) & 0x80808080u;
                    u64 r = __ballot(act && x0 == 0x80808080u && x1 == 0x80808080u) & queued;
                    r &= first_pass ? (1ull << i) : above;
                    if (!r) break;
                    const uint32_t j = (uint32_t)__builtin_ctzll(r);
                    const uint32_t aj = (uint32_t)__builtin_amdgcn_readlane((int)actor, (int)j);
                    const uint32_t sj = (uint32_t)__builtin_amdgcn_readlane((int)slot, (int)j);
                    const uint32_t sh = (aj & 3) * 8;
                    const uint32_t cur = (((aj < 4) ? crel_lo : crel_hi) >> sh) & 0xFF;
                    queued &= ~(1ull << j);
                    progress = true;
                    above = (j >= 63) ? 0 : (~0ull << (j + 1));
                    if (sj + 1 <= cur) {
                        const uint32_t k = L.first[fidx(aj, sj)];
                        const uint32_t ck = (uint32_t)__builtin_amdgcn_readlane((int)c.content_id, (int)k);
                        const uint32_t cj = (uint32_t)__builtin_amdgcn_readlane((int)c.content_id, (int)j);
                        if (lane == j) hist = -2;
                        if (ck != cj) {
                            if (lane == 0) lds_min(L.errkey, err_key(H, 0, j, HM_ERR_INCONSISTENT_SEQ));
                            stop = true;
                            break;
                        }
                        if (first_pass) break;
                        continue;
                    }
                    if (aj < 4) crel_lo = (crel_lo & ~(0xFFu << sh)) | ((sj + 1) << sh);
                    else        crel_hi = (crel_hi & ~(0xFFu << sh)) | ((sj + 1) << sh);
                    if (lane == 0) L.first[fidx(aj, sj)] = j;
                    if (lane == j) hist = (int32_t)H;
                    H++;
                    if (first_pass) break;
                }
                if (stop || !progress) break;
                first_pass = false;
                above = ~0ull;
            }
        }
        wave_sync();
        dmask = 0; pred_arr = 0xFFu;
        if (act && hist >= 0) {
            for (uint32_t j = 0; j < c.n_deps; j++) {
                const uint32_t pk = L.deps[my_dep0 + j];
                const uint32_t a = pk >> 24, s = pk & 0xFFFFFF;
                if (a == actor || s == 0) continue;
                dmask |= 1ull << L.first[fidx(a, (s - L.base[a]))];
            }
            if (seq - 1 != 0) { pred_arr = L.first[fidx(actor, (seq - 1 - mybase))]; dmask |= 1ull << pred_arr; }
        }
    }

    if (HM_PRIO_HIST && queued_doc) __builtin_amdgcn_s_setprio(0);
    STAMP(L, 3);
    if (HM_ABLATE & 512) return OUT_UNSUPPORTED;
    if (act) L.hist_of[lane] = hist;
    if (act && hist >= 0) L.h2a[hist] = (uint8_t)lane;
    wave_sync();
    const bool hv = lane < H;
    uint32_t ai = lane, hactor = actor, hseq = seq, hpred = pred_arr;
    u64 dm_arr = dmask;
    if (!identity) {
        ai = hv ? L.h2a[lane] : 0;
        dm_arr = shfl64(dmask, (int)ai);
        hactor = shfl32(actor, (int)ai); hseq = shfl32(seq, (int)ai); hpred = shfl32(pred_arr, (int)ai);
    }
    u64 D = 0, Dnp = 0;
    if (identity) {
        D = hv ? dm_arr : 0ull;
        Dnp = hv && hpred != 0xFFu ? D & ~(1ull << hpred) : D;
    } else if (hv) {
        u64 x = dm_arr;
        while (x) {
            const uint32_t j = (uint32_t)__builtin_ctzll(x);
            x &= x - 1;
            const u64 bit = 1ull << (uint32_t)L.hist_of[j];
            D |= bit;
            if (j != hpred) Dnp |= bit;
        }
    }
    if (hv) { lds_or(L.cov, D); lds_or(&L.chain[hactor], 1ull << lane); }
    uint32_t alo = hv && lane < 32 ? 1u << lane : 0u, ahi = hv && lane >= 32 ? 1u << (lane - 32) : 0u;
    if (HM_ABLATE & 1024) return OUT_UNSUPPORTED;
    {
        if (HM_PRIO_PUSH) __builtin_amdgcn_s_setprio(HM_PRIO_PUSH);
        const uint32_t Hs = (uint32_t)__builtin_amdgcn_readfirstlane((int)H);
        const uint32_t Dlo = (uint32_t)D, Dhi = (uint32_t)(D >> 32);
        const uint32_t H1 = Hs < 32 ? Hs : 32;
#if HM_PUSH_BPERM
#define PUSH_BC(v, k) ((uint32_t)__builtin_amdgcn_ds_bpermute((k) << 2, (int)(v)))
#else
#define PUSH_BC(v, k) ((uint32_t)__builtin_amdgcn_readlane((int)(v), (int)(k)))
#endif
#define PUSH_LO(k) alo |= PUSH_BC(alo, (k)) & (uint32_t)__builtin_amdgcn_sbfe((int)Dlo, (k), 1)
#define PUSH_HI(k) do { const uint32_t m_ = (uint32_t)__builtin_amdgcn_sbfe((int)Dhi, (k) - 32, 1);          \
                        const uint32_t bl_ = PUSH_BC(alo, (k)), bh_ = PUSH_BC(ahi, (k));                   \
                        alo |= bl_ & m_; ahi |= bh_ & m_; } while (0)
#pragma unroll
        for (int g = 0; g < 32; g += 8) {
            if ((uint32_t)g >= H1) break;
            PUSH_LO(g); PUSH_LO(g + 1); PUSH_LO(g + 2); PUSH_LO(g + 3);
            PUSH_LO(g + 4); PUSH_LO(g + 5); PUSH_LO(g + 6); PUSH_LO(g + 7);
        }
#pragma unroll
        for (int g = 32; g < 64; g += 8) {
            if ((uint32_t)g >= Hs) break;
            PUSH_HI(g); PUSH_HI(g + 1); PUSH_HI(g + 2); PUSH_HI(g + 3);
            PUSH_HI(g + 4); PUSH_HI(g + 5); PUSH_HI(g + 6); PUSH_HI(g + 7);
        }
#undef PUSH_LO
#undef PUSH_HI
#undef PUSH_BC
        if (HM_PRIO_PUSH && !HM_PRIO_FOLD) __builtin_amdgcn_s_setprio(0);
    }
    const u64 anc = hv ? ((((u64)ahi << 32) | alo) & ~(1ull << lane)) : 0ull;
    if (hv) L.anc[lane] = anc;
    wave_sync();
    STAMP(L, 4);
    if (HM_ABLATE & 64) return OUT_UNSUPPORTED;
    const u64 covered = *L.cov;
    bool suspect = false;
    if (hv && (Dnp & (Dnp - 1))) {
        u64 x = Dnp;
        while (x) {
            const uint32_t i2 = (uint32_t)__builtin_ctzll(x);
            x &= x - 1;
            if (L.anc[i2] & Dnp) suspect = true;
        }
    }
    uint32_t h_own_row = own_row ? 1u : 0u, h_dep0 = my_dep0, h_nd = c.n_deps;
    if (!identity) {
        h_own_row = shfl32(h_own_row, (int)ai); h_dep0 = shfl32(my_dep0, (int)ai); h_nd = shfl32(c.n_deps, (int)ai);
    }
    suspect |= hv && h_own_row != 0;
#ifdef HM_DEV_NOFOLD
    suspect = false;
#endif
    if (suspect) {
        const FoldView fv = {L.anc, L.chain, L.first, L.base, L.deps, L.hist_of};
        if (fold_differs(fv, h_dep0, h_nd, hactor, hseq)) lds_or(L.flags, FL_UNSUPPORTED);
    }
    if (hv && !((covered >> lane) & 1)) L.headv[hactor] = hseq;
    for (uint32_t i = lane; i < O; i += WAVE) { L.objslot[i] = i == 0 ? 0u : 0xFFFFFFFFu; L.objtype[i] = i == 0 ? HM_MAKE_MAP : 0xFF; }
    for (uint32_t i = lane; i < R; i += WAVE) {
        L.segor[i] = 0; L.segcnt[i] = 0; L.survpk[i] = 0; L.insmin[i] = 0xFFFFFFFFu; L.regobj[i] = HM_NONE;
    }
    wave_sync();

    STAMP(L, 5);
    if (HM_PRIO_FOLD && !HM_PRIO_K2) __builtin_amdgcn_s_setprio(0);
    if (HM_PRIO_K2) __builtin_amdgcn_s_setprio(HM_PRIO_K2);
    if (HM_ABLATE & 2) return OUT_UNSUPPORTED;
    uint32_t oreg[OPL], oobj[OPL], opar[OPL], oact[OPL], okey[OPL], oarr[OPL], oelem[OPL], oactor[OPL];
    int32_t oh[OPL];
    bool counter_ops = false, malformed = false;
#pragma unroll
    for (int t = 0; t < OPL; t++) {
        const uint32_t k = lane + WAVE * t;
        oh[t] = -1; okey[t] = 0; oarr[t] = 0; oreg[t] = 0; oobj[t] = 0; opar[t] = 0; oact[t] = 0xFF; oelem[t] = 0; oactor[t] = 0;
        if (k < m) {
            const uint32_t meta = L.opmeta[k], ro = L.opro[k], pr = L.oppar[k];
            const uint32_t cw = L.opchg[k], ch = cw & 0xFFu;
            oarr[t] = ch; oactor[t] = cw >> 8; oh[t] = identity ? (int32_t)ch : L.hist_of[ch];
            oreg[t] = ro & 0xFFFFu; oobj[t] = ro >> 16; oact[t] = meta & 0xFF;
            opar[t] = pr == PAR_HEAD ? HM_HEAD : pr;
            if (LISTS) {
                oelem[t] = L.opelem[k];
                if (oact[t] == HM_INS && oelem[t] >= (1u << 24)) lds_or(L.flags, FL_UNSUPPORTED);
            }
            counter_ops |= oact[t] == HM_INC || ((meta >> 8) & 0xFF) == HM_DT_COUNTER;
            okey[t] = ((uint32_t)(oh[t] < 0 ? 0 : oh[t]) << 16) | (k - L.opbase[ch]);
            const uint32_t a = oact[t];
            const bool bad = a <= HM_MAKE_TEXT ? oobj[t] >= O
                           : (a <= HM_INC ? (oreg[t] >= R || (a == HM_INS && opar[t] != HM_HEAD && opar[t] >= R)) : true);
            malformed |= bad;
            if (oh[t] >= 0 && !bad) {
                if (a <= HM_MAKE_TEXT) lds_min(&L.objslot[oobj[t]], okey[t] + 1);
                else if (oobj[t] < O) {
                    L.regobj[oreg[t]] = oobj[t];
                    if (a == HM_INS) lds_min(&L.insmin[oreg[t]], okey[t] + 1);
                    else {
                        lds_add(&L.segcnt[oreg[t]], 1u);
                        if (a != HM_INC) lds_or(&L.segor[oreg[t]], L.anc[oh[t]]);
                    }
                }
            }
        }
    }
    STAMP(L, 6);
    if (HM_ABLATE & 128) return OUT_UNSUPPORTED;
    if (__ballot(malformed)) return OUT_UNSUPPORTED;
    if (!p.counters && __ballot(counter_ops)) lds_or(L.flags, FL_UNSUPPORTED);
    wave_sync();
#pragma unroll
    for (int t = 0; t < OPL; t++)
        if (oh[t] >= 0 && oact[t] <= HM_MAKE_TEXT && oobj[t] < O) {
            if (L.objslot[oobj[t]] != okey[t] + 1)
                lds_min(L.errkey, err_key((uint32_t)oh[t], (okey[t] & 0xFFFF) + 1, oarr[t], HM_ERR_DUPLICATE_OBJECT));
            else L.objtype[oobj[t]] = (uint8_t)oact[t];
        }
    wave_sync();
    bool surv[OPL];
    bool has_list = false, anyerr = false, late = false;
#pragma unroll
    for (int t = 0; t < OPL; t++) {
        const OpCheck ck = op_check(L, oh[t], oact[t], oobj[t], oreg[t], opar[t], okey[t], R, O);
        has_list |= ck.has_list;
        anyerr |= ck.err != 0;
        late |= ck.late;
        surv[t] = ck.surv;
        if (surv[t]) lds_add(&L.survpk[oreg[t]], 1ull << (8 * oactor[t]));
    }
    if (__ballot(late)) return OUT_UNSUPPORTED;
    if (__ballot(anyerr)) {
        u64 errk = ~0ull;
#pragma unroll
        for (int t = 0; t < OPL; t++) {
            const OpCheck ck = op_check(L, oh[t], oact[t], oobj[t], oreg[t], opar[t], okey[t], R, O);
            const uint32_t h = oh[t] < 0 ? 0u : (uint32_t)oh[t], kk = (okey[t] & 0xFFFF) + 1;
            const u64 ek = ck.err ? err_key(h, kk, oarr[t], ck.err) : ~0ull;
            errk = errk < ek ? errk : ek;
        }
        lds_min(L.errkey, errk);
    }
    const bool doc_lists = __ballot(has_list) != 0;
    if (!LISTS && doc_lists) lds_or(L.flags, FL_UNSUPPORTED);
    wave_sync();
    if (*L.errkey != ~0ull) return OUT_ERROR;
    if (*L.flags & FL_UNSUPPORTED) return OUT_UNSUPPORTED;

    STAMP(L, 7);
    if (HM_PRIO_K2 && !HM_PRIO_RANK) __builtin_amdgcn_s_setprio(0);
    if (HM_PRIO_RANK) __builtin_amdgcn_s_setprio(HM_PRIO_RANK);
    if (HM_ABLATE & 4) return OUT_UNSUPPORTED;
    uint32_t total = 0;
    const uint32_t lane_s = LISTS ? lane : fresh_lane();
    for (uint32_t r0 = 0; r0 < R; r0 += WAVE) {
        const uint32_t r = r0 + lane_s;
        uint32_t tot;
        const uint32_t cnt = r < R ? bytesum64(L.survpk[r]) : 0u;
        const uint32_t ex = wave_excl_scan(cnt, &tot);
        if (r < R) { L.regoff[r] = total + ex; L.survcnt[r] = cnt; }
        total += tot;
    }
    wave_sync();
    uint32_t my_act[OPL], rb0[OPL], rank[OPL];
    bool tie[OPL];
#pragma unroll
    for (int t = 0; t < OPL; t++) {
        const uint32_t ri = surv[t] ? oreg[t] : 0u;
        my_act[t] = surv[t] ? oactor[t] : 0u;
        rb0[t] = L.regoff[ri];
        const u64 pk = L.survpk[ri];
        const uint32_t sh = 8 * (my_act[t] + 1);
        rank[t] = surv[t] ? bytesum64(sh >= 64 ? 0ull : pk >> sh) : 0u;
        tie[t] = surv[t] && ((pk >> (8 * my_act[t])) & 0xFF) > 1;
    }
    bool anytie = false;
#pragma unroll
    for (int t = 0; t < OPL; t++) anytie |= tie[t];
    if (__ballot(anytie)) {
        uint32_t myt[OPL];
        bool oddn[OPL];
#pragma unroll
        for (int t = 0; t < OPL; t++) {
            myt[t] = 0;
            oddn[t] = tie[t] && (L.segcnt[tie[t] ? oreg[t] : 0u] & 1);
            u64 tm = __ballot(tie[t]);
            while (tm) {
                const int j = (int)__builtin_ctzll(tm);
                tm &= tm - 1;
                const uint32_t rj = (uint32_t)__builtin_amdgcn_readlane((int)oreg[t], j);
                const uint32_t kj = (uint32_t)__builtin_amdgcn_readlane((int)okey[t], j);
                uint32_t pc = 0;
#pragma unroll
                for (int t2 = 0; t2 < OPL; t2++)
                    pc += (uint32_t)__popcll(__ballot(oh[t2] >= 0 && oact[t2] >= HM_SET && oact[t2] <= HM_INC &&
                                                      oreg[t2] == rj && okey[t2] < kj));
                if ((int)lane == j) myt[t] = tie_order(pc);
            }
        }
#pragma unroll
        for (int t = 0; t < OPL; t++) {
            u64 tm = __ballot(tie[t]);
            while (tm) {
                const int j = (int)__builtin_ctzll(tm);
                tm &= tm - 1;
                const uint32_t rj = (uint32_t)__builtin_amdgcn_readlane((int)oreg[t], j);
                const uint32_t aj = (uint32_t)__builtin_amdgcn_readlane((int)my_act[t], j);
                const uint32_t tj = (uint32_t)__builtin_amdgcn_readlane((int)myt[t], j);
#pragma unroll
                for (int t2 = 0; t2 < OPL; t2++) {
                    const bool peer = tie[t2] && oreg[t2] == rj && my_act[t2] == aj && !(t2 == t && (int)lane == j);
                    rank[t2] += (peer && (oddn[t2] ? (tj > myt[t2]) : (tj < myt[t2]))) ? 1u : 0u;
                }
            }
        }
    }
#pragma unroll
    for (int t = 0; t < OPL; t++) {
        if (!surv[t]) continue;
        const uint32_t pos = rb0[t] + rank[t];
        uint32_t tag = 0;
        if (p.counters) {
            const uint32_t mt = L.opmeta[lane + WAVE * t], vt = (mt >> 16) & 0xFF;
            const bool cset = (mt & 0xFF) == HM_SET && ((mt >> 8) & 0xFF) == HM_DT_COUNTER && (vt == HM_V_INT || vt == HM_V_FLOAT);
            tag = cset ? (0x8000u | (vt == HM_V_INT ? 0x4000u : 0u) | ((uint32_t)oh[t] << 8)) : 0u;
            L.survsum[pos] = 0;
        }
        L.survop[pos] = (uint16_t)((lane + WAVE * t) | tag);
    }
    wave_sync();
    if (HM_PRIO_RANK) __builtin_amdgcn_s_setprio(0);
    STAMP(L, 8);
    if (HM_ABLATE & 256) return OUT_UNSUPPORTED;
    if constexpr (LISTS) {
        if (doc_lists) {
            if (HM_PRIO_K3) __builtin_amdgcn_s_setprio(HM_PRIO_K3);
            rga_order<OPL>(L, R, O, oreg, oobj, opar, oact, oelem, oarr, oh, p.res_epos ? p.res_epos + doc.reg_off : nullptr);
            if (HM_PRIO_K3) __builtin_amdgcn_s_setprio(0);
        }
    }
    if (p.counters && __ballot(counter_ops)) {
        bool outside = false;
        int64_t incv[OPL];
        u64 basev[OPL];
#pragma unroll
        for (int t = 0; t < OPL; t++) {
            incv[t] = (oh[t] >= 0 && oact[t] == HM_INC) ? (int64_t)op_value(L, lane + WAVE * t) : 0;
            const uint32_t q = lane + WAVE * t;
            basev[t] = 0;
            if (q < total) {
                const uint32_t sw = L.survop[q];
                if ((sw & 0xC000u) == 0xC000u) basev[t] = op_value(L, sw & 0xFFu);
            }
        }
#pragma unroll
        for (int t = 0; t < OPL; t++) {
            if (oh[t] < 0 || oact[t] != HM_INC) continue;
            const uint32_t k = lane + WAVE * t;
            const uint32_t reg = oreg[t], b0 = L.regoff[reg], cnt = L.survcnt[reg];
            const u64 an = L.anc[oh[t]];
            const uint32_t my_vtag = (L.opmeta[k] >> 16) & 0xFF;
            const int64_t v = incv[t];
            for (uint32_t q = 0; q < cnt; q++) {
                const uint32_t sw = L.survop[b0 + q];
                if (!(sw & 0x8000u)) continue;
                if (!((an >> ((sw >> 8) & 63u)) & 1)) continue;
                if (!(sw & 0x4000u) || my_vtag != HM_V_INT || (u64)(v < 0 ? -v : v) >= (1ull << 44)) { outside = true; continue; }
                lds_add((LDS u64 *)&L.survsum[b0 + q], (unsigned long long)v);
            }
        }
#pragma unroll
        for (int t = 0; t < OPL; t++) {
            const int64_t b = (int64_t)basev[t];
            outside |= (u64)(b < 0 ? -b : b) >= (1ull << 52);
        }
        if (__ballot(outside)) return OUT_UNSUPPORTED;
        wave_sync();
    }
    st.hist = hist; st.H = H; st.total = total; st.doc_lists = doc_lists;
    return OUT_OK;
}

__device__ __forceinline__ uint32_t min_cmp_of(const SmallParams &p, const SmallLds &L, const hm_doc_row &doc, uint32_t mc) {
    const uint32_t lane = threadIdx.x, S = p.a_stride;
    const uint32_t bc = (lane < S && lane < doc.n_actors) ? L.bclock[lane] : 0u;
    const bool aGTE = __ballot(lane < S && bc < mc) == 0;
    const bool bGTE = __ballot(lane < S && mc < bc) == 0;
    return p.min_clock ? ((aGTE && bGTE) ? 0u : (aGTE ? 1u : (bGTE ? 2u : 3u))) : 0u;
}

template <int OPL> struct SurvRows { hm_surv_result r[OPL]; };
template <int OPL>
__device__ __forceinline__ SurvRows<OPL> surv_rows(const SmallParams &p, const SmallLds &L, const DocState &st) {
    const uint32_t lane = threadIdx.x;
    SurvRows<OPL> o;
#pragma unroll
    for (int t = 0; t < OPL; t++) {
        const uint32_t q = lane + WAVE * t;
        const uint32_t k = q < st.total ? (L.survop[q] & 0xFFu) : 0u, mt = L.opmeta[k];
        hm_surv_result sr;
        sr.op = k; sr.vtag = (mt >> 16) & 0xFF; sr.value = op_value(L, k);
        if (p.counters && q < st.total && (mt & 0xFF) == HM_SET && ((mt >> 8) & 0xFF) == HM_DT_COUNTER && sr.vtag == HM_V_INT)
            sr.value = (u64)((int64_t)sr.value + L.survsum[q]);
        o.r[t] = sr;
    }
    return o;
}

__device__ __forceinline__ void st16(void *dst, uint4 v) {
#if HM_NT_OUT
    typedef uint32_t v4u __attribute__((ext_vector_type(4)));
    const v4u x = {v.x, v.y, v.z, v.w};
    __builtin_nontemporal_store(x, reinterpret_cast<v4u *>(dst));
#else
    *reinterpret_cast<uint4 *>(dst) = v;
#endif
}
__device__ __forceinline__ void st4(void *dst, uint32_t v) {
#if HM_NT_OUT
    __builtin_nontemporal_store(v, reinterpret_cast<uint32_t *>(dst));
#else
    *reinterpret_cast<uint32_t *>(dst) = v;
#endif
}
template <int OPL, bool LISTS>
__device__ __forceinline__ void write_outputs(const SmallParams &p, const SmallLds &L, uint32_t d, uint32_t ds,
                                              const hm_doc_row &doc, Outcome oc, const DocState &st, uint32_t mcmp,
                                              const SurvRows<OPL> &sv) {
    const uint32_t lane = threadIdx.x;
    const uint32_t S = p.a_stride;
    const uint32_t n = doc.n_changes, A = doc.n_actors, R = doc.n_regs;
    hm_doc_result *dres = p.res_docs + ds;
    if (oc == OUT_ERROR) {
        const u64 ek = *L.errkey;
        if (lane == 0) {
            hm_doc_result r = {};
            r.status = (int32_t)(ek & 0xFF);
            r.err_change = (uint32_t)((ek >> 8) & 0xFFFF);
            const uint32_t opp1 = (uint32_t)((ek >> 24) & 0xFFFF);
            r.err_op = opp1 ? opp1 - 1 : HM_NONE;
            if (r.status == HM_ERR_UNSUPPORTED) { r.err_change = HM_NONE; r.err_op = HM_NONE; }
            *dres = r;
        }
        return;
    }
    if (oc == OUT_INVALID) {
        if (lane == 0) {
            hm_doc_result r = {};
            r.status = HM_ERR_INVALID; r.err_change = HM_NONE; r.err_op = HM_NONE;
            *dres = r;
        }
        for (uint32_t a = lane; a < S; a += WAVE) {
            p.res_clock[(size_t)ds * S + a] = 0u; p.res_heads[(size_t)ds * S + a] = 0u;
            p.res_back_clock[(size_t)ds * S + a] = 0u;
        }
        return;
    }
    if (oc == OUT_UNSUPPORTED) {
        if (lane == 0) {
            hm_doc_result r = {};
            r.status = HM_DEFERRED; r.err_change = HM_NONE; r.err_op = HM_NONE;
            *dres = r;
#if !HM_ABLATE
            p.deferred[atomicAdd(p.n_deferred, 1u)] = d;
#endif
        }
        return;
    }
    for (uint32_t r = lane; r < R; r += WAVE) {
        const int32_t li = (LISTS && st.doc_lists) ? (int32_t)L.insmin[r] : -1;
        st16(p.res_regs + doc.reg_off + r, make_uint4(L.survcnt[r], L.regoff[r], (uint32_t)li, L.regobj[r]));
    }
    if (lane < n) {
        const u64 an = st.hist >= 0 ? L.anc[st.hist] : 0ull;
        uint32_t *row = p.res_all_deps + (size_t)(doc.change_off + lane) * S;
        if (S == 8 || S == 4) {
            uint32_t v[NA_MAX];
#pragma unroll
            for (int a = 0; a < NA_MAX; a++) v[a] = (uint32_t)__popcll(an & L.chain[a]);
            st16(row, make_uint4(v[0], v[1], v[2], v[3]));
            if (S == 8) st16(row + 4, make_uint4(v[4], v[5], v[6], v[7]));
        } else {
            for (uint32_t a = 0; a < S; a++) row[a] = a < NA_MAX ? (uint32_t)__popcll(an & L.chain[a]) : 0u;
        }
    }
    if (lane < S) {
        const bool ar = lane < A;
        p.res_clock[(size_t)ds * S + lane] = ar ? (uint32_t)__popcll(L.chain[lane]) : 0u;
        p.res_heads[(size_t)ds * S + lane] = ar ? L.headv[lane] : 0u;
        p.res_back_clock[(size_t)ds * S + lane] = ar ? L.bclock[lane] : 0u;
    }
    for (uint32_t a = WAVE + lane; a < S; a += WAVE) {
        p.res_clock[(size_t)ds * S + a] = 0u; p.res_heads[(size_t)ds * S + a] = 0u; p.res_back_clock[(size_t)ds * S + a] = 0u;
    }
    const bool act = lane < n;
    const u64 q = __ballot(act && st.hist == -1);
    if (act) st4(p.res_hist + doc.change_off + lane, (uint32_t)st.hist);
    if (lane == 0) {
        hm_doc_result r = {};
        r.status = HM_OK; r.err_change = HM_NONE; r.err_op = HM_NONE;
        r.hist_len = st.H; r.n_queued = (uint32_t)__popcll(q); r.n_surv = st.total;
        r.min_cmp = mcmp;
        *dres = r;
    }
#pragma unroll
    for (int t = 0; t < OPL; t++) {
        const uint32_t q = lane + WAVE * t;
        if (q < st.total) st16(p.res_surv + doc.op_off + q, make_uint4(sv.r[t].op, sv.r[t].vtag, (uint32_t)sv.r[t].value,
                                                                       (uint32_t)(sv.r[t].value >> 32)));
    }
}

#if HM_ASYNC_NEXT
template <int OPL>
__device__ __forceinline__ uint32_t out_stores_min(const SmallParams &p, const hm_doc_row &doc, const DocState &st) {
    const uint32_t S = p.a_stride, n = doc.n_changes;
    uint32_t c = (doc.n_regs + WAVE - 1) / WAVE;
    if (n) c += (S == 8 ? 2u : 1u) + 1u;
    c += 3u + 2u;
    c += (st.total + WAVE - 1) / WAVE < (uint32_t)OPL ? (st.total + WAVE - 1) / WAVE : (uint32_t)OPL;
    return c;
}
template <int OPL>
__device__ __forceinline__ void pad_stores(const SmallParams &p, const hm_doc_row &doc, const DocState &st, uint32_t ds) {
    uint32_t *pad = &p.res_docs[ds].pad;
    const uint32_t zero = 0u;
    for (uint32_t c = out_stores_min<OPL>(p, doc, st); c < HM_ASYNC_STORES; c++)
        asm volatile("global_store_dword %0, %1, off" :: "v"(pad), "v"(zero) : "memory");
}
#endif

template <int OPL, bool LISTS, int CLS>
__global__ __launch_bounds__(WAVE) __attribute__((amdgpu_waves_per_eu(OPL >= 3 ? (LISTS ? (OPL == 3 ? HM_WAVES_PER_EU_LIST3 : HM_WAVES_PER_EU_OPL4 - 1) : HM_WAVES_PER_EU_OPL4) : HM_WAVES_PER_EU)))
void merge_small_kernel(SmallParams p) {
    extern __shared__ __align__(16) uint8_t lds_raw[];
    typedef SizeClass<CLS> C;
    SmallLds L;
    small_carve((LDS uint8_t *)lds_raw, WAVE * OPL, C::NR, C::NO, C::ND, LISTS, true, &L);
    p.cap_regs = C::NR; p.cap_objs = C::NO; p.cap_deps = C::ND;
#if HM_KARG_RELOAD
    typedef __attribute__((address_space(4))) const SmallParams KParams;
    KParams *kp = (KParams *)__builtin_amdgcn_kernarg_segment_ptr();
#endif
    uint32_t d = blockIdx.x;
    if (p.xcd_remap && (gridDim.x & 7) == 0) d = (blockIdx.x & 7) * (gridDim.x >> 3) + (blockIdx.x >> 3);
    if (d >= p.n_docs) return;
#if HM_STAMPS
    if (threadIdx.x == 0) { for (int i = 0; i < HM_NSTAMP; i++) L.stamps[i] = 0; L.stamps[HM_NSTAMP] = stamp_now(); }
#endif
    hm_doc_row doc = p.docs[d];
    bool dok = check_doc(p, doc);
    uint2 w0, w1, w2;
    {
        const Rows r = load_rows<OPL>(p, doc);
        stage_rows<OPL, LISTS>(p, L, doc, r, C::ND);
        w0 = make_uint2(r.c01.x, r.c01.y); w1 = make_uint2(r.c01.z, r.c01.w); w2 = r.c2;
    }
    wave_sync();
    for (;;) {
#if HM_KARG_RELOAD
        asm volatile("" : "+s"(kp));
        const SmallParams &p = *(const SmallParams *)kp;
#endif
        const uint32_t dn = d + gridDim.x;
        const bool more = dn < p.n_docs;
        bool dokn = true;
        hm_doc_row docn = {};
        static_assert(sizeof(hm_doc_row) == 12 * sizeof(uint32_t), "doc row words");
        uint32_t docw = 0;
        if (more && threadIdx.x < 12) docw = reinterpret_cast<const uint32_t *>(p.docs + dn)[threadIdx.x];
        auto take_docn = [&]() {
            uint32_t w[12];
#pragma unroll
            for (int j = 0; j < 12; j++) w[j] = (uint32_t)__builtin_amdgcn_readlane((int)docw, j);
            __builtin_memcpy(&docn, w, sizeof docn);
        };
        Rows next;
#if HM_ASYNC_NEXT
        AsyncRows anext;
        constexpr bool ASY = OPL <= HM_ASYNC_MAX_OPL && !HM_PREFETCH_EARLY && !HM_STAGE_FIRST;
#else
        constexpr bool ASY = false;
#endif
#if HM_PREFETCH_EARLY
        if (more) { take_docn(); dokn = check_doc(p, docn); next = load_rows<OPL>(p, docn); }
#endif
        const bool in_env = doc.n_changes <= 64 && doc.n_actors <= NA_MAX && doc.n_ops <= WAVE * OPL && doc.n_ops < 256 &&
                            doc.n_regs <= C::NR && doc.n_objs <= C::NO && doc.n_objs >= 1 &&
                            doc.n_deps <= C::ND && !p.general_only;
        DocState st;
        const uint32_t ds = hm_slot(p, d);
        uint32_t mc = 0;
        if (p.min_clock && threadIdx.x < p.a_stride) mc = p.min_clock[(size_t)ds * p.a_stride + threadIdx.x];
        if (p.min_clock && p.a_stride > WAVE) {
            uint32_t extra = 0;
            for (uint32_t a = WAVE + threadIdx.x; a < p.a_stride; a += WAVE) extra |= p.min_clock[(size_t)ds * p.a_stride + a];
            if (__ballot(extra != 0) && threadIdx.x == NA_MAX) mc |= 1u;
        }
        const Outcome oc = !dok ? OUT_INVALID : in_env ? merge_doc_small<OPL, LISTS>(p, L, doc, w0, w1, w2, st) : OUT_UNSUPPORTED;
        STAMP(L, 9);
        uint32_t mcmp = oc == OUT_OK ? min_cmp_of(p, L, doc, mc) : 0u;
#if HM_FENCE_MCMP
        asm volatile("" : "+s"(mcmp) :: "memory");
#endif
#if !HM_PREFETCH_EARLY
        if (more) {
            take_docn();
            dokn = check_doc(p, docn);
#if HM_ASYNC_NEXT
            if constexpr (ASY) anext = load_rows_async<OPL>(p, docn);
            else
#endif
            next = load_rows<OPL>(p, docn);
        }
#endif
        STAMP(L, 12);
        if (HM_PRIO_IO) __builtin_amdgcn_s_setprio(HM_PRIO_IO);
        const SurvRows<OPL> sv = surv_rows<OPL>(p, L, st);
#if HM_STAGE_FIRST
        wave_sync();
        if (more) stage_rows<OPL, LISTS>(p, L, docn, next, C::ND);
        STAMP(L, 11);
        write_outputs<OPL, LISTS>(p, L, d, ds, doc, oc, st, mcmp, sv);
        if (HM_PRIO_IO) __builtin_amdgcn_s_setprio(0);
        wave_sync();
        STAMP(L, 10);
        if (!more) break;
#else
        write_outputs<OPL, LISTS>(p, L, d, ds, doc, oc, st, mcmp, sv);
#if HM_ASYNC_NEXT
        if constexpr (ASY) { if (more && oc == OUT_OK) pad_stores<OPL>(p, doc, st, ds); }
#endif
        wave_sync();
        STAMP(L, 10);
        if (!more) break;
#if HM_ASYNC_NEXT
        if constexpr (ASY) {
            next = take_rows_async<OPL>(anext, docn, oc == OUT_OK);
#if HM_ASYNC_CHECK
            async_check<OPL>(p, docn, next);
#endif
        }
#endif
        stage_rows<OPL, LISTS>(p, L, docn, next, C::ND);
        if (HM_PRIO_IO) __builtin_amdgcn_s_setprio(0);
        wave_sync();
        STAMP(L, 11);
#endif
        w0 = make_uint2(next.c01.x, next.c01.y); w1 = make_uint2(next.c01.z, next.c01.w); w2 = next.c2;
        d = dn;
        doc = docn;
        dok = dokn;
    }
#if HM_STAMPS
    if (threadIdx.x == 0)
        for (int i = 0; i < HM_NSTAMP; i++) atomicAdd(&hm_stamp_acc[i], (unsigned long long)L.stamps[i]);
#endif
}

__global__ void clock_cmp_kernel(const uint32_t *a, const uint32_t *b, uint8_t *out, uint32_t n_docs, uint32_t S) {
    const uint32_t lane = threadIdx.x & 63, wave = (blockIdx.x * blockDim.x + threadIdx.x) >> 6;
    const uint32_t rows_per_wave = WAVE / S;
    const uint32_t row = wave * rows_per_wave + lane / S, col = lane % S;
    const bool v = row < n_docs && lane < rows_per_wave * S;
    const uint32_t x = v ? a[(size_t)row * S + col] : 0, y = v ? b[(size_t)row * S + col] : 0;
    const u64 lt = __ballot(v && x < y), gt = __ballot(v && y < x);
    if (v && col == 0) {
        const u64 mask = (S >= 64 ? ~0ull : ((1ull << S) - 1)) << lane;
        const bool aGTE = (lt & mask) == 0, bGTE = (gt & mask) == 0;
        out[row] = (aGTE && bGTE) ? 0 : (aGTE ? 1 : (bGTE ? 2 : 3));
    }
}
__global__ void clock_union_kernel(const uint32_t *a, const uint32_t *b, uint32_t *c, size_t n) {
    for (size_t i = blockIdx.x * (size_t)blockDim.x + threadIdx.x; i < n; i += (size_t)gridDim.x * blockDim.x)
        c[i] = a[i] > b[i] ? a[i] : b[i];
}
__global__ void clock_intersection_kernel(const uint32_t *a, const uint32_t *b, uint32_t *c, size_t n) {
    for (size_t i = blockIdx.x * (size_t)blockDim.x + threadIdx.x; i < n; i += (size_t)gridDim.x * blockDim.x)
        c[i] = a[i] < b[i] ? a[i] : b[i];
}

}

extern "C" int hm_debug_async_check(unsigned long long *out2, int reset) {
#if HM_ASYNC_CHECK && HM_ASYNC_NEXT
    if (!out2 || hipDeviceSynchronize() != hipSuccess) return -1;
    if (hipMemcpyFromSymbol(&out2[0], HIP_SYMBOL(hm::hm_async_checked), 8) != hipSuccess ||
        hipMemcpyFromSymbol(&out2[1], HIP_SYMBOL(hm::hm_async_bad), 8) != hipSuccess) return -1;
    if (reset) {
        const unsigned long long z = 0;
        if (hipMemcpyToSymbol(HIP_SYMBOL(hm::hm_async_checked), &z, 8) != hipSuccess ||
            hipMemcpyToSymbol(HIP_SYMBOL(hm::hm_async_bad), &z, 8) != hipSuccess) return -1;
    }
    return 1;
#else
    (void)out2; (void)reset;
    return 0;
#endif
}
#if HM_STAMPS
extern "C" int hm_debug_stamps(unsigned long long *out, int n, int reset) {
    if (n > HM_NSTAMP) n = HM_NSTAMP;
    if (hipDeviceSynchronize() != hipSuccess) return -1;
    if (hipMemcpyFromSymbol(out, HIP_SYMBOL(hm::hm_stamp_acc), n * sizeof(unsigned long long)) != hipSuccess) return -1;
    if (reset) {
        unsigned long long z[HM_NSTAMP] = {};
        if (hipMemcpyToSymbol(HIP_SYMBOL(hm::hm_stamp_acc), z, sizeof z) != hipSuccess) return -1;
    }
    return n;
}
#endif
uint32_t hm_small_class(uint32_t max_regs, uint32_t max_objs, uint32_t max_deps) {
    typedef hm::SizeClass<0> S0;
    typedef hm::SizeClass<2> S2;
    if (max_regs <= S0::NR && max_objs <= S0::NO && max_deps <= S0::ND) return 0u;
    if (max_regs <= S2::NR && max_objs <= S2::NO && max_deps <= S2::ND) return 2u;
    return 1u;
}

template <int CLS> static size_t carve_of(uint32_t opl, bool lists, bool counters) {
    hm::SmallLds L;
    typedef hm::SizeClass<CLS> C;
    return hm::small_carve((uintptr_t)0, 64 * opl, C::NR, C::NO, C::ND, lists, counters, &L);
}

size_t hm_small_lds_bytes(uint32_t opl, uint32_t cls, bool lists, bool counters) {
    return cls == 0 ? carve_of<0>(opl, lists, counters) : cls == 2 ? carve_of<2>(opl, lists, counters) : carve_of<1>(opl, lists, counters);
}

uint32_t hm_small_occupancy(uint32_t opl, uint32_t cls, bool lists, bool counters) {
    const size_t lds = hm_small_lds_bytes(opl, cls, lists, counters);
    int n = 0;
    const int by_lds = (int)(160u * 1024u / ((lds + 511) & ~(size_t)511));
#define HM_OCC(O_, L_, C_) (void)hipOccupancyMaxActiveBlocksPerMultiprocessor(&n, hm::merge_small_kernel<O_, L_, C_>, WAVE, lds)
#define HM_OCC_OPL(L_, C_) switch (opl) { case 1: HM_OCC(1, L_, C_); break; case 2: HM_OCC(2, L_, C_); break; case 3: HM_OCC(3, L_, C_); break; default: HM_OCC(4, L_, C_); }
    if (cls == 0)      { if (lists) { HM_OCC_OPL(true, 0) } else { HM_OCC_OPL(false, 0) } }
    else if (cls == 2) { if (lists) { HM_OCC_OPL(true, 2) } else { HM_OCC_OPL(false, 2) } }
    else               { if (lists) { HM_OCC_OPL(true, 1) } else { HM_OCC_OPL(false, 1) } }
#undef HM_OCC_OPL
#undef HM_OCC
    if (n > by_lds) n = by_lds;
    return n > 0 ? (uint32_t)n : 1u;
}

hipError_t hm_launch_small(const SmallParams &p, uint32_t opl, uint32_t cls, bool lists, uint32_t grid, hipStream_t s) {
    const size_t lds = hm_small_lds_bytes(opl, cls, lists, p.counters != 0);
#define HM_LAUNCH(O_, L_, C_) hipLaunchKernelGGL((hm::merge_small_kernel<O_, L_, C_>), dim3(grid), dim3(WAVE), lds, s, p)
#define HM_OPL(L_, C_) switch (opl) { case 1: HM_LAUNCH(1, L_, C_); break; case 2: HM_LAUNCH(2, L_, C_); break; case 3: HM_LAUNCH(3, L_, C_); break; default: HM_LAUNCH(4, L_, C_); }
    if (cls == 0)      { if (lists) { HM_OPL(true, 0) } else { HM_OPL(false, 0) } }
    else if (cls == 2) { if (lists) { HM_OPL(true, 2) } else { HM_OPL(false, 2) } }
    else               { if (lists) { HM_OPL(true, 1) } else { HM_OPL(false, 1) } }
#undef HM_OPL
#undef HM_LAUNCH
    return hipGetLastError();
}

hipError_t hm_launch_clock(int which, const uint32_t *a, const uint32_t *b, void *out, uint32_t n_docs,
                           uint32_t S, hipStream_t s) {
    if (which == 0) {
        if (S == 0 || S > HM_MAX_STRIDE) return hipErrorInvalidValue;
        const uint32_t rows_per_wave = 64 / S;
        const uint32_t waves = (n_docs + rows_per_wave - 1) / rows_per_wave;
        const uint32_t blocks = (waves + 3) / 4;
        hipLaunchKernelGGL(hm::clock_cmp_kernel, dim3(blocks ? blocks : 1), dim3(256), 0, s, a, b, (uint8_t *)out, n_docs, S);
    } else {
        const size_t n = (size_t)n_docs * S;
        uint32_t blocks = (uint32_t)((n + 255) / 256);
        if (blocks > 8192) blocks = 8192;
        if (which == 1) hipLaunchKernelGGL(hm::clock_union_kernel, dim3(blocks ? blocks : 1), dim3(256), 0, s, a, b, (uint32_t *)out, n);
        else hipLaunchKernelGGL(hm::clock_intersection_kernel, dim3(blocks ? blocks : 1), dim3(256), 0, s, a, b, (uint32_t *)out, n);
    }
    return hipGetLastError();
}
```

hypermerge_amd/engine.py:

```python
from __future__ import annotations

import ctypes
import sys
import os
from typing import Optional, Sequence

import numpy as np

from .columnar import Batch, Results, CBatch, CResults

_HERE = os.path.dirname(os.path.abspath(__file__))
LIB = os.environ.get("HMGPU_LIB") or os.path.join(_HERE, "_lib", "libhmgpu.so")

EXPORTS = ("hm_abi_version", "hm_status_message", "hm_engine_create", "hm_engine_destroy",
           "hm_engine_last_error", "hm_merge_host", "hm_scratch_bytes", "hm_merge_device",
           "hm_last_kernel_ms", "hm_last_deferred", "hm_clock_cmp_device", "hm_clock_union_device",
           "hm_clock_intersection_device", "hm_store_create", "hm_store_destroy", "hm_doc_open",
           "hm_batch_submit", "hm_batch_wait", "hm_doc_info", "hm_doc_read", "hm_doc_log",
           "hm_doc_history_prefix", "hm_doc_set_min_clock", "hm_store_clock_update", "hm_sync_ranges_device",
           "hm_comm_unique_id", "hm_comm_create", "hm_comm_destroy", "hm_comm_group_start", "hm_comm_group_end",
           "hm_clock_records_scratch_bytes", "hm_clock_records_device", "hm_clock_count_allgather",
           "hm_clock_allgather", "hm_clock_min_allreduce", "hm_comm_create_local", "hm_clock_exchange_host",
           "hm_clock_min_host", "hm_decode_blocks", "hm_decoded_batch", "hm_decoded_status", "hm_decoded_n_strings",
           "hm_decoded_string", "hm_decoded_actor", "hm_decoded_obj", "hm_decoded_reg", "hm_decoded_free",
           "hm_store_set_incremental", "hm_store_last_routing", "hm_store_last_kernel_ms", "hm_store_inc_states", "hm_debug_async_check", "hm_doc_open_n", "hm_doc_reset", "hm_store_read_regs", "hm_store_read_history",
           "hm_cursors_create", "hm_cursors_destroy", "hm_cursors_reserve", "hm_cursors_update", "hm_cursors_get",
           "hm_cursors_entry", "hm_cursors_docs_with_actors", "hm_docset_create", "hm_docset_destroy",
           "hm_docset_engine", "hm_docset_open", "hm_docset_apply", "hm_text_data", "hm_text_results", "hm_text_free",
           "hm_docset_doc_info", "hm_docset_history_prefix", "hm_docset_clock_update", "hm_docset_view",
           "hm_docset_stats", "hm_docset_routing", "hm_docset_handles", "hm_sync_ranges_host", "hm_batch_submit_device", "hm_batch_wait_device",
           "hm_batch_undo", "hm_store_blocked", "hm_store_waiting", "hm_store_read_queue", "hm_missing_deps_device",
           "hm_missing_deps_host", "hm_docset_blocked", "hm_docset_waiting")

_lib = None


class EngineError(RuntimeError):
    pass


def lib():
    global _lib
    if _lib is None:
        if not os.path.exists(LIB):
            raise EngineError(f"{LIB} is missing: run __graft_entry__.build() (no CPU fallback exists)")
        try:
            import torch
        except ImportError:
            pass
        L = ctypes.CDLL(LIB)
        L.hm_abi_version.restype = ctypes.c_uint32
        L.hm_status_message.argtypes = [ctypes.c_int]
        L.hm_status_message.restype = ctypes.c_char_p
        L.hm_engine_create.argtypes = [ctypes.c_void_p, ctypes.POINTER(ctypes.c_void_p)]
        L.hm_engine_destroy.argtypes = [ctypes.c_void_p]
        L.hm_engine_last_error.argtypes = [ctypes.c_void_p]
        L.hm_engine_last_error.restype = ctypes.c_char_p
        L.hm_merge_host.argtypes = [ctypes.c_void_p, ctypes.POINTER(CBatch), ctypes.POINTER(CResults)]
        L.hm_merge_device.argtypes = [ctypes.c_void_p, ctypes.POINTER(CBatch), ctypes.POINTER(CResults),
                                      ctypes.c_void_p, ctypes.c_void_p]
        L.hm_scratch_bytes.argtypes = [ctypes.POINTER(CBatch)]
        L.hm_scratch_bytes.restype = ctypes.c_size_t
        L.hm_last_kernel_ms.argtypes = [ctypes.c_void_p, ctypes.POINTER(ctypes.c_float), ctypes.c_int]
        L.hm_last_deferred.argtypes = [ctypes.c_void_p, ctypes.c_void_p, ctypes.c_uint32]
        for f in ("hm_clock_cmp_device", "hm_clock_union_device", "hm_clock_intersection_device"):
            getattr(L, f).argtypes = [ctypes.c_void_p] + [ctypes.c_void_p] * 3 + [ctypes.c_uint32] * 2 + [ctypes.c_void_p]
        vp, u32 = ctypes.c_void_p, ctypes.c_uint32
        sig = {
            "hm_store_create": [vp, vp, vp], "hm_store_destroy": [vp], "hm_doc_open": [vp, vp],
            "hm_batch_submit": [vp, vp, vp, vp, vp], "hm_batch_wait": [vp, ctypes.c_uint64, vp, vp, vp, vp],
            "hm_batch_submit_device": [vp, vp, vp, vp, vp], "hm_batch_wait_device": [vp, ctypes.c_uint64, vp, vp],
            "hm_batch_undo": [vp, ctypes.c_uint64],
            "hm_doc_info": [vp, u32, vp], "hm_doc_read": [vp, u32] + [vp] * 7, "hm_doc_log": [vp, u32, vp, vp, vp],
            "hm_doc_history_prefix": [vp, u32, u32, vp], "hm_doc_set_min_clock": [vp, u32, vp],
            "hm_store_clock_update": [vp, u32, vp, vp, vp, vp],
            "hm_sync_ranges_device": [vp, vp, vp, vp, vp, vp, u32, vp],
            "hm_comm_unique_id": [vp], "hm_comm_create": [vp, ctypes.c_int, ctypes.c_int, vp, vp],
            "hm_comm_destroy": [vp], "hm_comm_group_start": [], "hm_comm_group_end": [],
            "hm_clock_records_scratch_bytes": [u32, u32],
            "hm_clock_records_device": [vp, vp, vp, vp, vp, u32, u32, vp, vp, vp, vp],
            "hm_clock_count_allgather": [vp, ctypes.c_uint64, vp, vp],
            "hm_clock_allgather": [vp, vp, vp, vp, vp], "hm_clock_min_allreduce": [vp, vp, ctypes.c_uint64, vp],
            "hm_comm_create_local": [vp, ctypes.c_int, vp],
            "hm_clock_exchange_host": [vp, ctypes.c_int, vp, vp, vp, ctypes.c_uint64, vp],
            "hm_clock_min_host": [vp, ctypes.c_int, vp, ctypes.c_uint64],
            "hm_decode_blocks": [vp, vp, vp, u32, u32, ctypes.c_int, vp], "hm_decoded_batch": [vp, vp],
            "hm_decoded_status": [vp], "hm_decoded_n_strings": [vp], "hm_decoded_string": [vp, u32, vp],
            "hm_decoded_actor": [vp, u32, u32, vp], "hm_decoded_free": [vp],
            "hm_decoded_obj": [vp, u32, u32, vp], "hm_decoded_reg": [vp, u32, u32, vp, vp],
            "hm_store_set_incremental": [vp, ctypes.c_int], "hm_store_last_routing": [vp, vp], "hm_store_last_kernel_ms": [vp, vp], "hm_store_inc_states": [vp, vp], "hm_debug_async_check": [vp, ctypes.c_int],
            "hm_doc_open_n": [vp, u32, vp], "hm_doc_reset": [vp, vp, u32], "hm_store_read_regs": [vp, u32, vp, vp, vp, vp, u32, vp],
            "hm_store_read_history": [vp, u32, vp, vp, vp, vp, vp, vp],
            "hm_cursors_create": [vp, u32, vp], "hm_cursors_destroy": [vp], "hm_cursors_reserve": [vp, u32],
            "hm_cursors_update": [vp, u32, vp, vp, vp, vp, vp], "hm_cursors_get": [vp, u32, vp, vp, vp, vp],
            "hm_cursors_entry": [vp, u32, vp, vp, vp],
            "hm_cursors_docs_with_actors": [vp, u32, vp, vp, u32, vp, vp, vp, vp],
            "hm_docset_create": [vp, vp, vp], "hm_docset_destroy": [vp], "hm_docset_engine": [vp],
            "hm_docset_open": [vp, u32, vp], "hm_docset_apply": [vp, vp, vp, vp, vp, u32, vp],
            "hm_text_data": [vp, vp], "hm_text_results": [vp, vp], "hm_text_free": [vp],
            "hm_docset_doc_info": [vp, u32, vp], "hm_docset_history_prefix": [vp, u32, u32, vp],
            "hm_docset_clock_update": [vp, u32, vp, vp, vp, vp], "hm_docset_view": [vp, u32, vp],
            "hm_docset_stats": [vp, vp], "hm_docset_routing": [vp, vp], "hm_docset_handles": [vp, u32, vp, vp], "hm_sync_ranges_host": [vp, vp, vp, vp, vp, vp, u32, u32],
            "hm_store_blocked": [vp, vp, u32, vp], "hm_store_waiting": [vp, u32, vp, vp, vp, vp],
            "hm_store_read_queue": [vp, u32, vp, vp, vp],
            "hm_missing_deps_device": [vp, ctypes.POINTER(CBatch), ctypes.POINTER(CResults), vp, vp],
            "hm_missing_deps_host": [vp, ctypes.POINTER(CBatch), ctypes.POINTER(CResults), vp],
            "hm_docset_blocked": [vp, vp, u32, vp], "hm_docset_waiting": [vp, u32, vp, vp],
        }
        for f, a in sig.items():
            getattr(L, f).argtypes = a
        L.hm_store_destroy.restype = None
        L.hm_cursors_destroy.restype = None
        L.hm_comm_destroy.restype = None
        L.hm_decoded_status.restype = ctypes.POINTER(ctypes.c_int32)
        L.hm_decoded_n_strings.restype = ctypes.c_uint32
        L.hm_decoded_string.restype = ctypes.c_void_p
        L.hm_decoded_actor.restype = ctypes.c_void_p
        L.hm_decoded_obj.restype = ctypes.c_void_p
        L.hm_decoded_reg.restype = ctypes.c_void_p
        L.hm_decoded_free.restype = None
        L.hm_clock_records_scratch_bytes.restype = ctypes.c_size_t
        L.hm_docset_destroy.restype = None
        L.hm_docset_engine.restype = ctypes.c_void_p
        L.hm_text_data.restype = ctypes.c_void_p
        L.hm_text_results.restype = ctypes.c_void_p
        L.hm_text_free.restype = None
        _lib = L
    return _lib


class _Config(ctypes.Structure):
    _fields_ = [("device", ctypes.c_int), ("flags", ctypes.c_int)]


GENERAL_ONLY = 1


class Engine:
    def __init__(self, device: int = 0, flags: int = 0):
        L = lib()
        h = ctypes.c_void_p()
        cfg = _Config(device, flags)
        st = L.hm_engine_create(ctypes.byref(cfg), ctypes.byref(h))
        if st != 0:
            raise EngineError(f"hm_engine_create failed: {L.hm_status_message(st).decode()}")
        self._h = h
        self._L = L
        self.device = device

    def close(self) -> None:
        if getattr(self, "_h", None):
            self._L.hm_engine_destroy(self._h)
            self._h = None

    def __del__(self):
        if sys.is_finalizing():
            return
        try:
            self.close()
        except Exception:
            pass

    def _check(self, st: int, what: str) -> None:
        if st != 0:
            msg = self._L.hm_engine_last_error(self._h).decode()
            raise EngineError(f"{what}: {self._L.hm_status_message(st).decode()} ({msg})")

    def merge(self, batch: Batch, results: Optional[Results] = None) -> Results:
        if results is None:
            results = Results.alloc(batch)
        cb, cr = batch.c_struct(), results.c_struct()
        self._check(self._L.hm_merge_host(self._h, ctypes.byref(cb), ctypes.byref(cr)), "hm_merge_host")
        return results

    def merge_device(self, cbatch: CBatch, cresults: CResults, stream: int = 0) -> None:
        self._check(self._L.hm_merge_device(self._h, ctypes.byref(cbatch), ctypes.byref(cresults), None,
                                            ctypes.c_void_p(stream) if stream else None), "hm_merge_device")

    def missing_deps(self, batch: Batch, results: Results) -> np.ndarray:
        out = np.zeros((batch.n_docs, batch.a_stride), np.uint32)
        cb, cr = batch.c_struct(), results.c_struct()
        self._check(self._L.hm_missing_deps_host(self._h, ctypes.byref(cb), ctypes.byref(cr), out.ctypes.data),
                    "hm_missing_deps_host")
        return out

    def missing_deps_device(self, cbatch: CBatch, cresults: CResults, out_ptr: int, stream: int = 0) -> None:
        self._check(self._L.hm_missing_deps_device(self._h, ctypes.byref(cbatch), ctypes.byref(cresults),
                                                   ctypes.c_void_p(out_ptr), ctypes.c_void_p(stream) if stream else None),
                    "hm_missing_deps_device")

    def last_kernel_ms(self) -> Sequence[float]:
        buf = (ctypes.c_float * 4)()
        n = self._L.hm_last_kernel_ms(self._h, buf, 4)
        return [float(buf[i]) for i in range(n)]

    def last_deferred(self, n_docs: int) -> np.ndarray:
        out = np.zeros(max(n_docs, 1), np.uint32)
        n = self._L.hm_last_deferred(self._h, out.ctypes.data, len(out))
        if n < 0:
            self._check(-n, "hm_last_deferred")
        return out[:min(n, len(out))].copy()

    def clock_op(self, which: str, a_ptr: int, b_ptr: int, out_ptr: int, n_docs: int, a_stride: int,
                 stream: int = 0) -> None:
        f = {"cmp": self._L.hm_clock_cmp_device, "union": self._L.hm_clock_union_device,
             "intersection": self._L.hm_clock_intersection_device}[which]
        self._check(f(self._h, a_ptr, b_ptr, out_ptr, n_docs, a_stride, stream or None), f"clock_{which}")
```

include/hypermerge_amd.h:

```cpp
#ifndef HYPERMERGE_AMD_H
#define HYPERMERGE_AMD_H

#include <stdint.h>
#include <stddef.h>

#ifdef __cplusplus
extern "C" {
#endif

#define HM_ABI_VERSION 4u

typedef enum {
    HM_OK = 0,
    HM_ERR_INCONSISTENT_SEQ = 1,
    HM_ERR_UNKNOWN_OBJECT = 2,
    HM_ERR_DUPLICATE_OBJECT = 3,
    HM_ERR_DUPLICATE_ELEM = 4,
    HM_ERR_MISSING_ELEM = 5,
    HM_ERR_UNSUPPORTED = 16,
    HM_ERR_INVALID = 32,
    HM_ERR_DEVICE = 33,
    HM_ERR_NOMEM = 34
} hm_status;

enum {
    HM_MAKE_MAP = 0, HM_MAKE_TABLE = 1, HM_MAKE_LIST = 2, HM_MAKE_TEXT = 3,
    HM_INS = 4, HM_SET = 5, HM_DEL = 6, HM_LINK = 7, HM_INC = 8
};
enum { HM_DT_NONE = 0, HM_DT_COUNTER = 1, HM_DT_TIMESTAMP = 2 };
enum {
    HM_V_NULL = 0, HM_V_FALSE = 1, HM_V_TRUE = 2,
    HM_V_INT = 3,
    HM_V_FLOAT = 4,
    HM_V_STR = 5,
    HM_V_OBJ = 6
};
#define HM_HEAD 0xFFFFFFFFu
#define HM_NONE 0xFFFFFFFFu


typedef struct {
    uint32_t change_off;
    uint32_t n_changes;
    uint32_t dep_off;
    uint32_t n_deps;
    uint32_t op_off;
    uint32_t n_ops;
    uint32_t reg_off;
    uint32_t n_regs;
    uint32_t n_objs;
    uint16_t n_actors;
    uint16_t flags;
    uint32_t reserved[2];
} hm_doc_row;
#define HM_DOC_HAS_LISTS 1u
#define HM_DOC_HAS_COUNTERS 2u

typedef struct {
    uint16_t actor;
    uint16_t n_deps;
    uint32_t seq;
    uint32_t dep_off;
    uint32_t n_ops;
    uint32_t op_first;
    uint32_t content_id;
} hm_change_row;

typedef struct {
    uint16_t actor;
    uint16_t pad;
    uint32_t seq;
} hm_dep_row;

typedef struct {
    uint32_t obj;
    uint32_t reg;
    uint32_t parent;
    uint32_t elem;
    uint8_t  action;
    uint8_t  datatype;
    uint8_t  vtag;
    uint8_t  pad;
    uint32_t key;
    uint64_t value;
} hm_op_row;

#define HM_MAX_STRIDE 256u

typedef struct {
    uint32_t n_docs, n_changes, n_deps, n_ops, n_regs;
    uint32_t a_stride;
    uint32_t max_changes, max_ops, max_regs, max_objs;
    uint32_t doc_flags;
    uint32_t max_deps;
    const hm_doc_row    *docs;
    const hm_change_row *changes;
    const hm_dep_row    *deps;
    const hm_op_row     *ops;
    const uint32_t      *min_clock;
} hm_batch;

typedef struct {
    int32_t  status;
    uint32_t err_change;
    uint32_t err_op;
    uint32_t hist_len;
    uint32_t n_queued;
    uint32_t n_surv;
    uint32_t min_cmp;
    uint32_t pad;
} hm_doc_result;

typedef struct {
    uint32_t n_surv;
    uint32_t surv_off;
    int32_t  list_index;
    uint32_t obj;
} hm_reg_result;

typedef struct {
    uint32_t op;
    uint32_t vtag;
    uint64_t value;
} hm_surv_result;

typedef struct {
    hm_doc_result  *docs;
    uint32_t       *clock;
    uint32_t       *back_clock;
    uint32_t       *heads;
    int32_t        *hist;
    uint32_t       *all_deps;
    hm_reg_result  *regs;
    hm_surv_result *surv;
} hm_results;

typedef struct hm_engine hm_engine;

typedef struct {
    int device;
    int flags;
} hm_config;
#define HM_CFG_GENERAL_ONLY 1

uint32_t hm_abi_version(void);
const char *hm_status_message(int status);

int  hm_engine_create(const hm_config *cfg, hm_engine **out);
void hm_engine_destroy(hm_engine *e);
const char *hm_engine_last_error(const hm_engine *e);

int hm_merge_host(hm_engine *e, const hm_batch *batch, const hm_results *out);

size_t hm_scratch_bytes(const hm_batch *batch);
int hm_merge_device(hm_engine *e, const hm_batch *batch, const hm_results *out,
                    void *scratch, void *stream);

int hm_last_kernel_ms(hm_engine *e, float *ms, int max_kernels);
int hm_last_deferred(hm_engine *e, uint32_t *out_docs, uint32_t cap);

int hm_clock_cmp_device(hm_engine *e, const uint32_t *a, const uint32_t *b, uint8_t *out,
                        uint32_t n_docs, uint32_t a_stride, void *stream);
int hm_clock_union_device(hm_engine *e, const uint32_t *a, const uint32_t *b, uint32_t *c,
                          uint32_t n_docs, uint32_t a_stride, void *stream);
int hm_clock_intersection_device(hm_engine *e, const uint32_t *a, const uint32_t *b, uint32_t *c,
                                 uint32_t n_docs, uint32_t a_stride, void *stream);

typedef struct hm_store hm_store;

typedef struct {
    uint32_t a_stride;
    uint32_t reserved;
} hm_store_config;

int  hm_store_create(hm_engine *e, const hm_store_config *cfg, hm_store **out);
void hm_store_destroy(hm_store *s);

int hm_doc_open(hm_store *s, uint32_t *out_doc);

int hm_doc_open_n(hm_store *s, uint32_t n, uint32_t *out_first);

int hm_doc_reset(hm_store *s, const uint32_t *doc_handles, uint32_t n);

int hm_batch_submit(hm_store *s, const hm_batch *b, const uint32_t *doc_handles,
                    const uint8_t *actor_remap, uint64_t *out_batch_id);

int hm_batch_wait(hm_store *s, uint64_t batch_id, hm_doc_result *out_docs,
                  uint32_t *out_clock, uint32_t *out_back_clock, uint32_t *out_heads);

int hm_batch_submit_device(hm_store *s, const hm_batch *b, const uint32_t *doc_handles,
                           const uint8_t *actor_remap, uint64_t *out_batch_id);

int hm_batch_wait_device(hm_store *s, uint64_t batch_id, void *out_dev, uint32_t *out_n_failed);

int hm_batch_undo(hm_store *s, uint64_t batch_id);

int hm_store_set_incremental(hm_store *s, int on);
int hm_store_last_routing(const hm_store *s, uint32_t *out3);
int hm_store_last_kernel_ms(const hm_store *s, float *out2);
int hm_store_inc_states(hm_store *s, uint32_t *out);

int hm_debug_async_check(unsigned long long *out2, int reset);

typedef struct {
    uint32_t n_changes, n_deps, n_ops, n_regs, n_objs, n_actors;
    uint32_t hist_len, n_queued, n_surv;
    int32_t  status;
} hm_doc_info_t;
int hm_doc_info(hm_store *s, uint32_t doc, hm_doc_info_t *out);

int hm_doc_read(hm_store *s, uint32_t doc, int32_t *hist, uint32_t *all_deps, hm_reg_result *regs,
                hm_surv_result *surv, uint32_t *clock, uint32_t *back_clock, uint32_t *heads);

int hm_store_read_regs(hm_store *s, uint32_t n, const uint32_t *doc_handles, const uint32_t *regs,
                       hm_reg_result *out_regs, hm_surv_result *out_surv, uint32_t surv_cap, uint32_t *out_n_surv);

int hm_doc_log(hm_store *s, uint32_t doc, hm_change_row *changes, hm_dep_row *deps, hm_op_row *ops);

int hm_doc_history_prefix(hm_store *s, uint32_t doc, uint32_t n, uint32_t *out_log_index);

int hm_store_read_history(hm_store *s, uint32_t n, const uint32_t *doc_handles, const uint32_t *from, const uint32_t *to,
                          const uint32_t *out_off, uint32_t *out_log_index, uint32_t *out_all_deps);

int hm_store_blocked(hm_store *s, uint32_t *out_handles, uint32_t cap, uint32_t *out_n);
int hm_store_waiting(hm_store *s, uint32_t n, const uint32_t *doc_handles,
                     uint32_t *out_missing , uint32_t *out_unmet_min , uint32_t *out_n_queued );
int hm_store_read_queue(hm_store *s, uint32_t n, const uint32_t *doc_handles, const uint32_t *out_off, uint32_t *out_log_index);
int hm_missing_deps_device(hm_engine *e, const hm_batch *b, const hm_results *r, uint32_t *out_missing, void *stream);
int hm_missing_deps_host(hm_engine *e, const hm_batch *b, const hm_results *r, uint32_t *out_missing);

int hm_doc_set_min_clock(hm_store *s, uint32_t doc, const uint32_t *clock);

int hm_store_clock_update(hm_store *s, uint32_t n, const uint32_t *docs, uint8_t *out_written,
                          uint8_t *out_differs, uint32_t *out_stored);

typedef struct hm_cursors hm_cursors;
int  hm_cursors_create(hm_engine *e, uint32_t max_actors_per_doc, hm_cursors **out);
void hm_cursors_destroy(hm_cursors *c);
int  hm_cursors_reserve(hm_cursors *c, uint32_t n_rows);
int  hm_cursors_update(hm_cursors *c, uint32_t n_docs, const uint32_t *rows, const uint32_t *entry_off,
                       const uint64_t *actor_keys, const double *seqs, uint8_t *out_differs);
int  hm_cursors_get(hm_cursors *c, uint32_t n, const uint32_t *rows, uint32_t *out_count, uint64_t *out_actor,
                    uint64_t *out_seq);
int  hm_cursors_entry(hm_cursors *c, uint32_t n, const uint32_t *rows, const uint64_t *actor_keys, uint64_t *out_seq);
int  hm_cursors_docs_with_actors(hm_cursors *c, uint32_t n_actors, const uint64_t *actor_keys, const double *min_seqs,
                                 uint32_t cap, uint32_t *out_row, uint32_t *out_actor, uint64_t *out_seq,
                                 uint32_t *out_n);

int hm_sync_ranges_device(hm_engine *e, const uint64_t *present, const uint64_t *word_off,
                          const uint32_t *lo, const uint32_t *hi, uint32_t *out_end, uint32_t n,
                          void *stream);
int hm_sync_ranges_host(hm_engine *e, const uint64_t *present, const uint64_t *word_off, const uint32_t *lo,
                        const uint32_t *hi, uint32_t *out_end, uint32_t n, uint32_t n_words);

typedef struct hm_decoded hm_decoded;
int hm_decode_blocks(const uint8_t *data, const uint64_t *block_off, const uint32_t *doc_block, uint32_t n_docs,
                     uint32_t a_stride, int threads, hm_decoded **out);
int hm_decoded_batch(const hm_decoded *d, hm_batch *out);
const int32_t *hm_decoded_status(const hm_decoded *d);
uint32_t hm_decoded_n_strings(const hm_decoded *d);
const char *hm_decoded_string(const hm_decoded *d, uint32_t i, size_t *len);
const char *hm_decoded_actor(const hm_decoded *d, uint32_t doc, uint32_t rank, size_t *len);
const char *hm_decoded_obj(const hm_decoded *d, uint32_t doc, uint32_t obj, size_t *len);
const char *hm_decoded_reg(const hm_decoded *d, uint32_t doc, uint32_t reg, uint32_t *obj, size_t *len);
void hm_decoded_free(hm_decoded *d);

typedef struct hm_docset hm_docset;
typedef struct hm_text hm_text;
typedef struct {
    uint32_t threads;
    uint32_t flags;
} hm_docset_config;
#define HM_DOCSET_NO_PATCHES 1u
#define HM_DOCSET_BINARY 2u
#define HM_DOCSET_NET_DIFFS 4u

int  hm_docset_create(hm_engine *e, const hm_docset_config *cfg, hm_docset **out);
void hm_docset_destroy(hm_docset *ds);
hm_engine *hm_docset_engine(hm_docset *ds);
int  hm_docset_open(hm_docset *ds, uint32_t n, uint32_t *out_first);
int  hm_docset_apply(hm_docset *ds, const uint8_t *data, const uint64_t *block_off, const uint32_t *doc_block,
                     const uint32_t *docs, uint32_t n_docs, hm_text **out);
const char *hm_text_data(const hm_text *t, size_t *len);
const hm_doc_result *hm_text_results(const hm_text *t, uint32_t *n);
void hm_text_free(hm_text *t);

typedef struct {
    uint32_t a_stride;
    uint32_t n_changes, n_ops, n_actors, n_objs, n_regs, hist_len, n_queued;
} hm_docset_doc_info_t;
int hm_docset_doc_info(hm_docset *ds, uint32_t doc, hm_docset_doc_info_t *out);
int hm_docset_history_prefix(hm_docset *ds, uint32_t doc, uint32_t n, uint32_t *out_log_index);
int hm_docset_clock_update(hm_docset *ds, uint32_t n, const uint32_t *docs, uint8_t *out_written, uint8_t *out_differs,
                           hm_text **out_stored);
int hm_docset_blocked(hm_docset *ds, uint32_t *out_docs, uint32_t cap, uint32_t *out_n);
int hm_docset_waiting(hm_docset *ds, uint32_t n, const uint32_t *docs, hm_text **out);
int hm_docset_view(hm_docset *ds, uint32_t doc, hm_text **out);
int hm_docset_stats(const hm_docset *ds, uint64_t *out8);
int hm_docset_routing(const hm_docset *ds, uint64_t *out3);
int hm_docset_handles(const hm_docset *ds, uint32_t a_stride, uint32_t *out_opened, uint32_t *out_free);

#define HM_COMM_ID_BYTES 128
#define HM_CLOCK_NOT_HELD 0xFFFFFFFFu

typedef struct {
    uint64_t doc_key;
    uint64_t actor_key;
    uint32_t seq;
    uint32_t flags;
} hm_clock_rec;

typedef struct hm_comm hm_comm;
int  hm_comm_unique_id(uint8_t *out );
int  hm_comm_create(hm_engine *e, int world, int rank, const uint8_t *unique_id, hm_comm **out);
void hm_comm_destroy(hm_comm *c);
int  hm_comm_group_start(void);
int  hm_comm_group_end(void);

size_t hm_clock_records_scratch_bytes(uint32_t n_docs, uint32_t a_stride);
int hm_clock_records_device(hm_engine *e, const uint64_t *doc_keys, const uint64_t *actor_keys,
                            const uint32_t *clock, const uint32_t *base, uint32_t n_docs, uint32_t a_stride,
                            hm_clock_rec *out, uint32_t *out_count, void *scratch, void *stream);

int hm_clock_count_allgather(hm_comm *c, uint64_t n_local, uint64_t *d_counts, void *stream);
int hm_clock_allgather(hm_comm *c, const hm_clock_rec *d_recs, const uint64_t *counts, hm_clock_rec *d_out,
                       void *stream);
int hm_clock_min_allreduce(hm_comm *c, uint32_t *d_seq, uint64_t n, void *stream);

int hm_comm_create_local(hm_engine *const *engines, int n, hm_comm **out);
int hm_clock_exchange_host(hm_comm *const *comms, int n, const hm_clock_rec *const *recs, const uint64_t *n_recs,
                           hm_clock_rec *out, uint64_t out_cap, uint64_t *out_total);
int hm_clock_min_host(hm_comm *const *comms, int n, uint32_t *const *seq, uint64_t len);

#ifdef __cplusplus
}
#endif
#endif
```

Baseline: 29.30 billion changes/s.

## Cut VGPR pressure in small merge kernel to raise waves per EU

Adds a "diet" mode for small, non-list merge kernels. In this mode the lane id is re-materialised opaquely at each stage, async loads use an SGPR base with immediate offsets, per-lane masking of prefetched rows is removed, and kernel arguments are pinned in scalar registers. The default waves-per-EU launch bound goes from 4 to 5, with the wide variants kept at 4. The aim is higher occupancy to hide memory latency, at the risk of register spills under the tighter bound and extra v_mov instructions. A debug API is also added to report small-kernel occupancy.

```diff
diff --git a/hypermerge_amd/csrc/engine.cpp b/hypermerge_amd/csrc/engine.cpp
--- a/hypermerge_amd/csrc/engine.cpp
+++ b/hypermerge_amd/csrc/engine.cpp
@@ -228,6 +228,26 @@
     } catch (...) {
         return fail(e, HM_ERR_DEVICE, "exception in hm_merge_device");
     }
+}
+
+int hm_debug_small_occupancy(hm_engine *e, const hm_batch *hb, uint32_t *out6) {
+    if (!e || !hb || !out6) return HM_ERR_INVALID;
+    if (hipSetDevice(e->device) != hipSuccess) return fail(e, HM_ERR_DEVICE, "hipSetDevice");
+    hm_batch b = *hb;
+    if (!b.max_changes && !b.max_ops && !b.max_regs && !b.max_objs && hb->docs) {
+        for (uint32_t d = 0; d < b.n_docs; d++) {
+            b.max_ops = std::max(b.max_ops, hb->docs[d].n_ops);
+            b.max_regs = std::max(b.max_regs, hb->docs[d].n_regs);
+            b.max_objs = std::max(b.max_objs, hb->docs[d].n_objs);
+            b.max_deps = std::max(b.max_deps, hb->docs[d].n_deps);
+            b.doc_flags |= hb->docs[d].flags;
+        }
+    }
+    const Caps c = launch_caps(&b);
+    out6[0] = hm_small_occupancy(c.opl, c.cls, c.lists, c.counters);
+    out6[1] = (uint32_t)e->num_cus;
+    out6[2] = c.opl; out6[3] = c.cls; out6[4] = c.lists ? 1u : 0u; out6[5] = c.counters ? 1u : 0u;
+    return HM_OK;
 }
 
 int hm_merge_host(hm_engine *e, const hm_batch *hb, const hm_results *ho) {
diff --git a/hypermerge_amd/csrc/merge_kernels.h b/hypermerge_amd/csrc/merge_kernels.h
--- a/hypermerge_amd/csrc/merge_kernels.h
+++ b/hypermerge_amd/csrc/merge_kernels.h
@@ -29,10 +29,10 @@
 };
 #ifdef __HIPCC__
 __device__ __forceinline__ bool hm_doc_row_ok(const SmallParams &p, const hm_doc_row &d) {
-    return (unsigned long long)d.change_off + d.n_changes <= p.lim_changes &&
-           (unsigned long long)d.dep_off + d.n_deps <= p.lim_deps &&
-           (unsigned long long)d.op_off + d.n_ops <= p.lim_ops &&
-           (unsigned long long)d.reg_off + d.n_regs <= p.lim_regs && d.n_actors <= p.a_stride;
+    return ((unsigned long long)d.change_off + d.n_changes <= p.lim_changes) &
+           ((unsigned long long)d.dep_off + d.n_deps <= p.lim_deps) &
+           ((unsigned long long)d.op_off + d.n_ops <= p.lim_ops) &
+           ((unsigned long long)d.reg_off + d.n_regs <= p.lim_regs) & (d.n_actors <= p.a_stride);
 }
 #endif
 #ifdef __HIPCC__
diff --git a/hypermerge_amd/csrc/merge_kernels.hip b/hypermerge_amd/csrc/merge_kernels.hip
--- a/hypermerge_amd/csrc/merge_kernels.hip
+++ b/hypermerge_amd/csrc/merge_kernels.hip
@@ -46,6 +46,9 @@
 #ifndef HM_KARG_RELOAD
 #define HM_KARG_RELOAD 1
 #endif
+#ifndef HM_KARG_BATCH
+#define HM_KARG_BATCH 1
+#endif
 #ifndef HM_HIST_DP
 #define HM_HIST_DP 1
 #endif
@@ -83,7 +86,10 @@
 #define HM_OPAQUE_LANE 1
 #endif
 #ifndef HM_WAVES_PER_EU
-#define HM_WAVES_PER_EU 4
+#define HM_WAVES_PER_EU 5
+#endif
+#ifndef HM_WAVES_PER_EU_WIDE
+#define HM_WAVES_PER_EU_WIDE 4
 #endif
 #define WAVE 64
 #define NA_MAX 8
@@ -152,6 +158,11 @@
     return threadIdx.x;
 #endif
 }
+template <bool FRESH> __device__ __forceinline__ uint32_t lane_id() {
+    if constexpr (FRESH) return fresh_lane();
+    else return threadIdx.x;
+}
+template <int OPL, bool LISTS, int CLS> struct Diet { static constexpr bool on = OPL <= 2 && !LISTS && CLS != 1; };
 __device__ __forceinline__ void wave_sync() {
     __builtin_amdgcn_fence(__ATOMIC_SEQ_CST, "wavefront");
     __builtin_amdgcn_wave_barrier();
@@ -274,12 +285,12 @@
 
 
 __device__ __forceinline__ uint32_t fidx(uint32_t a, uint32_t s) { return (s & 63) * NA_MAX + (a & (NA_MAX - 1)); }
-__device__ __forceinline__ void clear_first(LDS uint32_t *first) {
+__device__ __forceinline__ void clear_first(LDS uint32_t *first, uint32_t lane) {
     static_assert(NA_MAX * 64 == 2 * WAVE * 4, "first-table size");
     LDS uint4 *f4 = (LDS uint4 *)first;
     const uint4 ones = make_uint4(~0u, ~0u, ~0u, ~0u);
-    f4[threadIdx.x] = ones;
-    f4[threadIdx.x + WAVE] = ones;
+    f4[lane] = ones;
+    f4[lane + WAVE] = ones;
 }
 
 __device__ __forceinline__ uint32_t tie_order(uint32_t pc) { return (pc & 1) ? (0x10000u - pc) : (0x20000u + pc); }
@@ -508,13 +519,15 @@
 template <int OPL>
 __device__ __forceinline__ void async_check(const SmallParams &p, const hm_doc_row &doc, const Rows &got) {
     const Rows want = load_rows<OPL>(p, doc);
+    const uint32_t lane = threadIdx.x;
     auto ne4 = [](uint4 a, uint4 b) { return a.x != b.x || a.y != b.y || a.z != b.z || a.w != b.w; };
     auto ne2 = [](uint2 a, uint2 b) { return a.x != b.x || a.y != b.y; };
-    bool bad = ne4(want.c01, got.c01) || ne2(want.c2, got.c2) || ne4(want.a0, got.a0) || ne4(want.b0, got.b0) ||
-               ne2(want.d0, got.d0) || ne2(want.d1, got.d1);
-    if (OPL > 1) bad = bad || ne4(want.a1, got.a1) || ne4(want.b1, got.b1);
-    if (OPL > 2) bad = bad || ne4(want.a2, got.a2) || ne4(want.b2, got.b2);
-    if (OPL > 3) bad = bad || ne4(want.a3, got.a3) || ne4(want.b3, got.b3);
+    auto op_ne = [&](uint32_t k, uint4 wa, uint4 wb, uint4 ga, uint4 gb) { return k < doc.n_ops && (ne4(wa, ga) || ne4(wb, gb)); };
+    bool bad = ne4(want.c01, got.c01) || ne2(want.c2, got.c2) || op_ne(lane, want.a0, want.b0, got.a0, got.b0) ||
+               (lane < doc.n_deps && ne2(want.d0, got.d0)) || (lane + WAVE < doc.n_deps && ne2(want.d1, got.d1));
+    if (OPL > 1) bad = bad || op_ne(lane + WAVE, want.a1, want.b1, got.a1, got.b1);
+    if (OPL > 2) bad = bad || op_ne(lane + 2 * WAVE, want.a2, want.b2, got.a2, got.b2);
+    if (OPL > 3) bad = bad || op_ne(lane + 3 * WAVE, want.a3, want.b3, got.a3, got.b3);
     const unsigned long long m = __ballot(bad);
     if (threadIdx.x == 0) {
         atomicAdd(&hm_async_checked, 1ull);
@@ -531,87 +544,71 @@
 #else
 #define HM_AL_POL ""
 #endif
-__device__ __forceinline__ u32x2 aload2(const void *p) {
+template <int IMM> __device__ __forceinline__ u32x2 aload2(const void *base, uint32_t off) {
     u32x2 v;
-    asm volatile("global_load_dwordx2 %0, %1, off" HM_AL_POL : "=v"(v) : "v"(p) : "memory");
+    asm volatile("global_load_dwordx2 %0, %1, %2 offset:%3" HM_AL_POL : "=v"(v) : "v"(off), "s"(base), "n"(IMM) : "memory");
     return v;
 }
-__device__ __forceinline__ u32x4 aload4(const void *p) {
+template <int IMM> __device__ __forceinline__ u32x4 aload4(const void *base, uint32_t off) {
     u32x4 v;
-    asm volatile("global_load_dwordx4 %0, %1, off" HM_AL_POL : "=v"(v) : "v"(p) : "memory");
+    asm volatile("global_load_dwordx4 %0, %1, %2 offset:%3" HM_AL_POL : "=v"(v) : "v"(off), "s"(base), "n"(IMM) : "memory");
     return v;
 }
-template <int OPL>
-__device__ __forceinline__ AsyncRows load_rows_async(const SmallParams &p, const hm_doc_row &doc) {
-    const uint32_t lane = threadIdx.x;
+template <int OPL, bool LISTS>
+__device__ __forceinline__ AsyncRows load_rows_async(const SmallParams &p, const hm_doc_row &doc, uint32_t lane) {
     AsyncRows r;
     r.c0 = r.c1 = r.c2 = r.d0 = r.d1 = u32x2{0u, 0u};
     r.a0 = r.b0 = r.a1 = r.b1 = r.a2 = r.b2 = r.a3 = r.b3 = u32x4{0u, 0u, 0u, 0u};
+    static_assert(sizeof(hm_change_row) == 24 && sizeof(hm_op_row) == 32 && sizeof(hm_dep_row) == 8, "row sizes");
+    auto row = [&](uint32_t k, uint32_t n) { return k < n ? k : n - 1u; };
     if (doc.n_changes) {
-        const uint32_t i = lane < doc.n_changes ? lane : doc.n_changes - 1u;
-        const uint2 *cs = reinterpret_cast<const uint2 *>(p.changes + doc.change_off + i);
-        r.c0 = aload2(cs); r.c1 = aload2(cs + 1); r.c2 = aload2(cs + 2);
+        const hm_change_row *cs = p.changes + doc.change_off;
+        const uint32_t o = row(lane, doc.n_changes) * 24u;
+        r.c0 = aload2<0>(cs, o); r.c1 = aload2<8>(cs, o); r.c2 = aload2<16>(cs, o);
     }
     if (doc.n_ops) {
-        const uint32_t i0 = lane < doc.n_ops ? lane : doc.n_ops - 1u;
-        const uint4 *o0 = reinterpret_cast<const uint4 *>(p.ops + doc.op_off + i0);
-        r.a0 = aload4(o0); r.b0 = aload4(o0 + 1);
+        const hm_op_row *os = p.ops + doc.op_off;
+        const uint32_t o0 = row(lane, doc.n_ops) * 32u;
+        r.a0 = aload4<0>(os, o0); r.b0 = aload4<16>(os, o0);
         if (OPL > 1) {
-            const uint32_t i1 = lane + WAVE < doc.n_ops ? lane + WAVE : doc.n_ops - 1u;
-            const uint4 *o1 = reinterpret_cast<const uint4 *>(p.ops + doc.op_off + i1);
-            r.a1 = aload4(o1); r.b1 = aload4(o1 + 1);
+            const uint32_t o1 = row(lane + WAVE, doc.n_ops) * 32u;
+            r.a1 = aload4<0>(os, o1); r.b1 = aload4<16>(os, o1);
         }
         if (OPL > 2) {
-            const uint32_t i2 = lane + 2 * WAVE < doc.n_ops ? lane + 2 * WAVE : doc.n_ops - 1u;
-            const uint4 *o2 = reinterpret_cast<const uint4 *>(p.ops + doc.op_off + i2);
-            r.a2 = aload4(o2); r.b2 = aload4(o2 + 1);
+            const uint32_t o2 = row(lane + 2 * WAVE, doc.n_ops) * 32u;
+            r.a2 = aload4<0>(os, o2); r.b2 = aload4<16>(os, o2);
         }
         if (OPL > 3) {
-            const uint32_t i3 = lane + 3 * WAVE < doc.n_ops ? lane + 3 * WAVE : doc.n_ops - 1u;
-            const uint4 *o3 = reinterpret_cast<const uint4 *>(p.ops + doc.op_off + i3);
-            r.a3 = aload4(o3); r.b3 = aload4(o3 + 1);
+            const uint32_t o3 = row(lane + 3 * WAVE, doc.n_ops) * 32u;
+            r.a3 = aload4<0>(os, o3); r.b3 = aload4<16>(os, o3);
         }
     }
     if (doc.n_deps) {
-        const uint32_t i0 = lane < doc.n_deps ? lane : doc.n_deps - 1u, i1 = lane + WAVE < doc.n_deps ? lane + WAVE : doc.n_deps - 1u;
-        r.d0 = aload2(p.deps + doc.dep_off + i0); r.d1 = aload2(p.deps + doc.dep_off + i1);
+        const hm_dep_row *dp = p.deps + doc.dep_off;
+        r.d0 = aload2<0>(dp, row(lane, doc.n_deps) * 8u); r.d1 = aload2<0>(dp, row(lane + WAVE, doc.n_deps) * 8u);
     }
     return r;
 }
-template <int OPL>
-__device__ __forceinline__ Rows take_rows_async(AsyncRows &r, const hm_doc_row &doc, bool padded) {
+template <int OPL, bool DIET>
+__device__ __forceinline__ Rows take_rows_async(AsyncRows &r, const hm_doc_row &doc) {
 #define HM_AW2 "+v"(r.c0), "+v"(r.c1), "+v"(r.c2), "+v"(r.a0), "+v"(r.b0), "+v"(r.a1), "+v"(r.b1), "+v"(r.d0), "+v"(r.d1)
 #define HM_AW3 HM_AW2, "+v"(r.a2), "+v"(r.b2)
 #define HM_AW4 HM_AW3, "+v"(r.a3), "+v"(r.b3)
-    if constexpr (OPL <= 2) {
-        if (padded) asm volatile("s_waitcnt vmcnt(%9)" : HM_AW2 : "n"(HM_ASYNC_STORES) : "memory");
-        else asm volatile("s_waitcnt vmcnt(0)" : HM_AW2 :: "memory");
-    } else if constexpr (OPL == 3) {
-        if (padded) asm volatile("s_waitcnt vmcnt(%11)" : HM_AW3 : "n"(HM_ASYNC_STORES) : "memory");
-        else asm volatile("s_waitcnt vmcnt(0)" : HM_AW3 :: "memory");
-    } else {
-        if (padded) asm volatile("s_waitcnt vmcnt(%13)" : HM_AW4 : "n"(HM_ASYNC_STORES) : "memory");
-        else asm volatile("s_waitcnt vmcnt(0)" : HM_AW4 :: "memory");
-    }
+    if constexpr (OPL <= 2) asm volatile("s_waitcnt vmcnt(%9)" : HM_AW2 : "n"(HM_ASYNC_STORES) : "memory");
+    else if constexpr (OPL == 3) asm volatile("s_waitcnt vmcnt(%11)" : HM_AW3 : "n"(HM_ASYNC_STORES) : "memory");
+    else asm volatile("s_waitcnt vmcnt(%13)" : HM_AW4 : "n"(HM_ASYNC_STORES) : "memory");
 #undef HM_AW4
 #undef HM_AW3
 #undef HM_AW2
-    const uint32_t lane = threadIdx.x;
+    const bool c = lane_id<DIET>() < doc.n_changes;
     Rows o;
-    const bool c = lane < doc.n_changes, k0 = lane < doc.n_ops, k1 = lane + WAVE < doc.n_ops;
     o.c01 = c ? make_uint4(r.c0.x, r.c0.y, r.c1.x, r.c1.y) : make_uint4(0u, 0u, 0u, 0u);
     o.c2 = c ? make_uint2(r.c2.x, r.c2.y) : make_uint2(0u, 0u);
-    o.a0 = k0 ? make_uint4(r.a0.x, r.a0.y, r.a0.z, r.a0.w) : make_uint4(0u, 0u, 0u, 0u);
-    o.b0 = k0 ? make_uint4(r.b0.x, r.b0.y, r.b0.z, r.b0.w) : make_uint4(0u, 0u, 0u, 0u);
-    o.a1 = k1 ? make_uint4(r.a1.x, r.a1.y, r.a1.z, r.a1.w) : make_uint4(0u, 0u, 0u, 0u);
-    o.b1 = k1 ? make_uint4(r.b1.x, r.b1.y, r.b1.z, r.b1.w) : make_uint4(0u, 0u, 0u, 0u);
-    const bool k2 = lane + 2 * WAVE < doc.n_ops, k3 = lane + 3 * WAVE < doc.n_ops;
-    o.a2 = k2 ? make_uint4(r.a2.x, r.a2.y, r.a2.z, r.a2.w) : make_uint4(0u, 0u, 0u, 0u);
-    o.b2 = k2 ? make_uint4(r.b2.x, r.b2.y, r.b2.z, r.b2.w) : make_uint4(0u, 0u, 0u, 0u);
-    o.a3 = k3 ? make_uint4(r.a3.x, r.a3.y, r.a3.z, r.a3.w) : make_uint4(0u, 0u, 0u, 0u);
-    o.b3 = k3 ? make_uint4(r.b3.x, r.b3.y, r.b3.z, r.b3.w) : make_uint4(0u, 0u, 0u, 0u);
-    o.d0 = lane < doc.n_deps ? make_uint2(r.d0.x, r.d0.y) : make_uint2(0u, 0u);
-    o.d1 = lane + WAVE < doc.n_deps ? make_uint2(r.d1.x, r.d1.y) : make_uint2(0u, 0u);
+    o.a0 = make_uint4(r.a0.x, r.a0.y, r.a0.z, r.a0.w); o.b0 = make_uint4(r.b0.x, r.b0.y, r.b0.z, r.b0.w);
+    o.a1 = make_uint4(r.a1.x, r.a1.y, r.a1.z, r.a1.w); o.b1 = make_uint4(r.b1.x, r.b1.y, r.b1.z, r.b1.w);
+    o.a2 = make_uint4(r.a2.x, r.a2.y, r.a2.z, r.a2.w); o.b2 = make_uint4(r.b2.x, r.b2.y, r.b2.z, r.b2.w);
+    o.a3 = make_uint4(r.a3.x, r.a3.y, r.a3.z, r.a3.w); o.b3 = make_uint4(r.b3.x, r.b3.y, r.b3.z, r.b3.w);
+    o.d0 = make_uint2(r.d0.x, r.d0.y); o.d1 = make_uint2(r.d1.x, r.d1.y);
     return o;
 }
 #endif
@@ -630,10 +627,10 @@
     L.opval[k] = ((u64)b.w << 32) | b.z;
     if (LISTS) L.opelem[k] = a.w;
 }
-template <int OPL, bool LISTS>
+template <int OPL, bool LISTS, bool DIET>
 __device__ __forceinline__ void stage_rows(const SmallParams &p, const SmallLds &L, const hm_doc_row &doc, const Rows &r,
                                            uint32_t cap_deps) {
-    const uint32_t lane = threadIdx.x, m = doc.n_ops;
+    const uint32_t lane = lane_id<DIET>(), m = doc.n_ops;
     stage_op<LISTS>(L, lane, m, r.a0, r.b0);
     if (OPL > 1) stage_op<LISTS>(L, lane + WAVE, m, r.a1, r.b1);
     if (OPL > 2) stage_op<LISTS>(L, lane + 2 * WAVE, m, r.a2, r.b2);
@@ -683,10 +680,10 @@
     return r;
 }
 
-template <int OPL, bool LISTS>
+template <int OPL, bool LISTS, bool DIET>
 __device__ __forceinline__ Outcome merge_doc_small(const SmallParams &p, const SmallLds &L, const hm_doc_row &doc,
                                                    const uint2 w0, const uint2 w1, const uint2 w2, DocState &st) {
-    const uint32_t lane = threadIdx.x;
+    uint32_t lane = lane_id<DIET>();
     const uint32_t n = doc.n_changes, A = doc.n_actors, m = doc.n_ops, R = doc.n_regs, O = doc.n_objs;
     st.hist = -1; st.H = 0; st.total = 0; st.doc_lists = false;
 
@@ -695,7 +692,7 @@
     if (HM_PRIO_K1) __builtin_amdgcn_s_setprio(HM_PRIO_K1);
     const bool act = lane < n;
     const hm_change_row c = change_of(w0, w1, w2);
-    clear_first(L.first);
+    clear_first(L.first, lane);
     if (lane < NA_MAX) { L.base[lane] = 0xFFFFFFFFu; L.bclock[lane] = 0; L.headv[lane] = 0; L.chain[lane] = 0; }
     if (lane == 0) { *L.errkey = ~0ull; L.flags[0] = 0; L.flags[1] = 0; *L.cov = 0; }
     const uint32_t dep_lo = doc.dep_off, ndep = doc.n_deps;
@@ -728,6 +725,7 @@
     wave_sync();
 
     STAMP(L, 1);
+    if constexpr (DIET) lane = fresh_lane();
     if (HM_ABLATE & 16) return OUT_UNSUPPORTED;
     {
         bool bad_dep = false;
@@ -783,6 +781,7 @@
     wave_sync();
 
     STAMP(L, 2);
+    if constexpr (DIET) lane = fresh_lane();
     if (HM_ABLATE & 32) return OUT_UNSUPPORTED;
     int32_t hist = -1;
     uint32_t H = 0;
@@ -1003,6 +1002,7 @@
     } else {
         uint32_t need_lo = 0, need_hi = 0;
         if (act) {
+#pragma unroll 1
             for (uint32_t j = 0; j < c.n_deps; j++) {
                 const uint32_t inf = L.depinfo[my_dep0 + j];
                 const uint32_t a = (inf >> 16) & (NA_MAX - 1), rel = (inf >> 8) & 0x7F;
@@ -1011,7 +1011,7 @@
             const uint32_t ps = seq - 1;
             need_set(need_lo, need_hi, a8, ps != 0 ? (ps >= mybase ? ps - mybase + 1 : 0x7Fu) : 0u);
         }
-        clear_first(L.first);
+        clear_first(L.first, lane);
         wave_sync();
         uint32_t crel_lo = 0, crel_hi = 0;
         u64 queued = 0;
@@ -1076,6 +1076,7 @@
 
     if (HM_PRIO_HIST && queued_doc) __builtin_amdgcn_s_setprio(0);
     STAMP(L, 3);
+    if constexpr (DIET) lane = fresh_lane();
     if (HM_ABLATE & 512) return OUT_UNSUPPORTED;
     if (act) L.hist_of[lane] = hist;
     if (act && hist >= 0) L.h2a[hist] = (uint8_t)lane;
@@ -1140,6 +1141,7 @@
     if (hv) L.anc[lane] = anc;
     wave_sync();
     STAMP(L, 4);
+    if constexpr (DIET) lane = fresh_lane();
     if (HM_ABLATE & 64) return OUT_UNSUPPORTED;
     const u64 covered = *L.cov;
     bool suspect = false;
@@ -1171,6 +1173,7 @@
     wave_sync();
 
     STAMP(L, 5);
+    if constexpr (DIET) lane = fresh_lane();
     if (HM_PRIO_FOLD && !HM_PRIO_K2) __builtin_amdgcn_s_setprio(0);
     if (HM_PRIO_K2) __builtin_amdgcn_s_setprio(HM_PRIO_K2);
     if (HM_ABLATE & 2) return OUT_UNSUPPORTED;
@@ -1211,6 +1214,7 @@
         }
     }
     STAMP(L, 6);
+    if constexpr (DIET) lane = fresh_lane();
     if (HM_ABLATE & 128) return OUT_UNSUPPORTED;
     if (__ballot(malformed)) return OUT_UNSUPPORTED;
     if (!p.counters && __ballot(counter_ops)) lds_or(L.flags, FL_UNSUPPORTED);
@@ -1253,6 +1257,7 @@
     if (*L.flags & FL_UNSUPPORTED) return OUT_UNSUPPORTED;
 
     STAMP(L, 7);
+    if constexpr (DIET) lane = fresh_lane();
     if (HM_PRIO_K2 && !HM_PRIO_RANK) __builtin_amdgcn_s_setprio(0);
     if (HM_PRIO_RANK) __builtin_amdgcn_s_setprio(HM_PRIO_RANK);
     if (HM_ABLATE & 4) return OUT_UNSUPPORTED;
@@ -1336,6 +1341,7 @@
     wave_sync();
     if (HM_PRIO_RANK) __builtin_amdgcn_s_setprio(0);
     STAMP(L, 8);
+    if constexpr (DIET) lane = fresh_lane();
     if (HM_ABLATE & 256) return OUT_UNSUPPORTED;
     if constexpr (LISTS) {
         if (doc_lists) {
@@ -1386,8 +1392,9 @@
     return OUT_OK;
 }
 
-__device__ __forceinline__ uint32_t min_cmp_of(const SmallParams &p, const SmallLds &L, const hm_doc_row &doc, uint32_t mc) {
-    const uint32_t lane = threadIdx.x, S = p.a_stride;
+__device__ __forceinline__ uint32_t min_cmp_of(const SmallParams &p, const SmallLds &L, const hm_doc_row &doc, uint32_t mc,
+                                               uint32_t lane) {
+    const uint32_t S = p.a_stride;
     const uint32_t bc = (lane < S && lane < doc.n_actors) ? L.bclock[lane] : 0u;
     const bool aGTE = __ballot(lane < S && bc < mc) == 0;
     const bool bGTE = __ballot(lane < S && mc < bc) == 0;
@@ -1395,9 +1402,8 @@
 }
 
 template <int OPL> struct SurvRows { hm_surv_result r[OPL]; };
-template <int OPL>
-__device__ __forceinline__ SurvRows<OPL> surv_rows(const SmallParams &p, const SmallLds &L, const DocState &st) {
-    const uint32_t lane = threadIdx.x;
+template <int OPL, bool LISTS>
+__device__ __forceinline__ SurvRows<OPL> surv_rows(const SmallParams &p, const SmallLds &L, const DocState &st, uint32_t lane) {
     SurvRows<OPL> o;
 #pragma unroll
     for (int t = 0; t < OPL; t++) {
@@ -1428,57 +1434,58 @@
     *reinterpret_cast<uint32_t *>(dst) = v;
 #endif
 }
-template <int OPL, bool LISTS>
+__device__ __forceinline__ void put_status_row(hm_doc_result *dres, uint32_t status, uint32_t err_change, uint32_t err_op) {
+    uint32_t zero = 0u;
+    asm volatile("" : "+v"(status), "+v"(err_change), "+v"(err_op), "+v"(zero));
+    hm_doc_result r;
+    r.status = (int32_t)status; r.err_change = err_change; r.err_op = err_op;
+    r.hist_len = zero; r.n_queued = zero; r.n_surv = zero; r.min_cmp = zero; r.pad = zero;
+    *dres = r;
+}
+template <int OPL, bool LISTS, bool DIET>
 __device__ __forceinline__ void write_outputs(const SmallParams &p, const SmallLds &L, uint32_t d, uint32_t ds,
                                               const hm_doc_row &doc, Outcome oc, const DocState &st, uint32_t mcmp,
-                                              const SurvRows<OPL> &sv) {
-    const uint32_t lane = threadIdx.x;
+                                              const SurvRows<OPL> &sv, uint32_t lane) {
     const uint32_t S = p.a_stride;
     const uint32_t n = doc.n_changes, A = doc.n_actors, R = doc.n_regs;
     hm_doc_result *dres = p.res_docs + ds;
     if (oc == OUT_ERROR) {
         const u64 ek = *L.errkey;
         if (lane == 0) {
-            hm_doc_result r = {};
-            r.status = (int32_t)(ek & 0xFF);
-            r.err_change = (uint32_t)((ek >> 8) & 0xFFFF);
-            const uint32_t opp1 = (uint32_t)((ek >> 24) & 0xFFFF);
-            r.err_op = opp1 ? opp1 - 1 : HM_NONE;
-            if (r.status == HM_ERR_UNSUPPORTED) { r.err_change = HM_NONE; r.err_op = HM_NONE; }
-            *dres = r;
+            const uint32_t status = (uint32_t)(ek & 0xFF), opp1 = (uint32_t)((ek >> 24) & 0xFFFF);
+            const bool uns = status == HM_ERR_UNSUPPORTED;
+            put_status_row(dres, status, uns ? HM_NONE : (uint32_t)((ek >> 8) & 0xFFFF), (uns || !opp1) ? HM_NONE : opp1 - 1);
         }
         return;
     }
     if (oc == OUT_INVALID) {
-        if (lane == 0) {
-            hm_doc_result r = {};
-            r.status = HM_ERR_INVALID; r.err_change = HM_NONE; r.err_op = HM_NONE;
-            *dres = r;
-        }
-        for (uint32_t a = lane; a < S; a += WAVE) {
-            p.res_clock[(size_t)ds * S + a] = 0u; p.res_heads[(size_t)ds * S + a] = 0u;
-            p.res_back_clock[(size_t)ds * S + a] = 0u;
-        }
+        if (lane == 0) put_status_row(dres, (uint32_t)HM_ERR_INVALID, HM_NONE, HM_NONE);
+        uint32_t *ck = p.res_clock + (size_t)ds * S, *hd = p.res_heads + (size_t)ds * S, *bk = p.res_back_clock + (size_t)ds * S;
+        for (uint32_t a = lane; a < S; a += WAVE) { ck[a] = 0u; hd[a] = 0u; bk[a] = 0u; }
         return;
     }
     if (oc == OUT_UNSUPPORTED) {
         if (lane == 0) {
-            hm_doc_result r = {};
-            r.status = HM_DEFERRED; r.err_change = HM_NONE; r.err_op = HM_NONE;
-            *dres = r;
+            put_status_row(dres, (uint32_t)HM_DEFERRED, HM_NONE, HM_NONE);
 #if !HM_ABLATE
             p.deferred[atomicAdd(p.n_deferred, 1u)] = d;
 #endif
         }
         return;
     }
+#if HM_KARG_RELOAD
+    if constexpr (DIET && HM_KARG_BATCH)
+        asm volatile("" :: "s"(p.res_docs), "s"(p.res_clock), "s"(p.res_back_clock), "s"(p.res_heads), "s"(p.res_hist),
+                     "s"(p.res_all_deps), "s"(p.res_regs), "s"(p.res_surv));
+#endif
+    hm_reg_result *regs = p.res_regs + doc.reg_off;
     for (uint32_t r = lane; r < R; r += WAVE) {
         const int32_t li = (LISTS && st.doc_lists) ? (int32_t)L.insmin[r] : -1;
-        st16(p.res_regs + doc.reg_off + r, make_uint4(L.survcnt[r], L.regoff[r], (uint32_t)li, L.regobj[r]));
+        st16(regs + r, make_uint4(L.survcnt[r], L.regoff[r], (uint32_t)li, L.regobj[r]));
     }
     if (lane < n) {
         const u64 an = st.hist >= 0 ? L.anc[st.hist] : 0ull;
-        uint32_t *row = p.res_all_deps + (size_t)(doc.change_off + lane) * S;
+        uint32_t *row = (p.res_all_deps + (size_t)doc.change_off * S) + lane * S;
         if (S == 8 || S == 4) {
             uint32_t v[NA_MAX];
 #pragma unroll
@@ -1489,18 +1496,17 @@
             for (uint32_t a = 0; a < S; a++) row[a] = a < NA_MAX ? (uint32_t)__popcll(an & L.chain[a]) : 0u;
         }
     }
+    uint32_t *ck = p.res_clock + (size_t)ds * S, *hd = p.res_heads + (size_t)ds * S, *bk = p.res_back_clock + (size_t)ds * S;
     if (lane < S) {
         const bool ar = lane < A;
-        p.res_clock[(size_t)ds * S + lane] = ar ? (uint32_t)__popcll(L.chain[lane]) : 0u;
-        p.res_heads[(size_t)ds * S + lane] = ar ? L.headv[lane] : 0u;
-        p.res_back_clock[(size_t)ds * S + lane] = ar ? L.bclock[lane] : 0u;
-    }
-    for (uint32_t a = WAVE + lane; a < S; a += WAVE) {
-        p.res_clock[(size_t)ds * S + a] = 0u; p.res_heads[(size_t)ds * S + a] = 0u; p.res_back_clock[(size_t)ds * S + a] = 0u;
-    }
+        ck[lane] = ar ? (uint32_t)__popcll(L.chain[lane]) : 0u;
+        hd[lane] = ar ? L.headv[lane] : 0u;
+        bk[lane] = ar ? L.bclock[lane] : 0u;
+    }
+    for (uint32_t a = WAVE + lane; a < S; a += WAVE) { ck[a] = 0u; hd[a] = 0u; bk[a] = 0u; }
     const bool act = lane < n;
     const u64 q = __ballot(act && st.hist == -1);
-    if (act) st4(p.res_hist + doc.change_off + lane, (uint32_t)st.hist);
+    if (act) st4((p.res_hist + doc.change_off) + lane, (uint32_t)st.hist);
     if (lane == 0) {
         hm_doc_result r = {};
         r.status = HM_OK; r.err_change = HM_NONE; r.err_op = HM_NONE;
@@ -1511,7 +1517,7 @@
 #pragma unroll
     for (int t = 0; t < OPL; t++) {
         const uint32_t q = lane + WAVE * t;
-        if (q < st.total) st16(p.res_surv + doc.op_off + q, make_uint4(sv.r[t].op, sv.r[t].vtag, (uint32_t)sv.r[t].value,
+        if (q < st.total) st16((p.res_surv + doc.op_off) + q, make_uint4(sv.r[t].op, sv.r[t].vtag, (uint32_t)sv.r[t].value,
                                                                        (uint32_t)(sv.r[t].value >> 32)));
     }
 }
@@ -1527,19 +1533,21 @@
     return c;
 }
 template <int OPL>
-__device__ __forceinline__ void pad_stores(const SmallParams &p, const hm_doc_row &doc, const DocState &st, uint32_t ds) {
+__device__ __forceinline__ void pad_stores(const SmallParams &p, const hm_doc_row &doc, const DocState &st, uint32_t ds, bool ok) {
     uint32_t *pad = &p.res_docs[ds].pad;
     const uint32_t zero = 0u;
-    for (uint32_t c = out_stores_min<OPL>(p, doc, st); c < HM_ASYNC_STORES; c++)
+    for (uint32_t c = ok ? out_stores_min<OPL>(p, doc, st) : 0u; c < HM_ASYNC_STORES; c++)
         asm volatile("global_store_dword %0, %1, off" :: "v"(pad), "v"(zero) : "memory");
 }
 #endif
 
 template <int OPL, bool LISTS, int CLS>
-__global__ __launch_bounds__(WAVE) __attribute__((amdgpu_waves_per_eu(OPL >= 3 ? (LISTS ? (OPL == 3 ? HM_WAVES_PER_EU_LIST3 : HM_WAVES_PER_EU_OPL4 - 1) : HM_WAVES_PER_EU_OPL4) : HM_WAVES_PER_EU)))
+__global__ __launch_bounds__(WAVE) __attribute__((amdgpu_waves_per_eu(OPL >= 3 ? (LISTS ? (OPL == 3 ? HM_WAVES_PER_EU_LIST3 : HM_WAVES_PER_EU_OPL4 - 1) : HM_WAVES_PER_EU_OPL4)
+                                              : (!LISTS && CLS != 1 ? HM_WAVES_PER_EU : HM_WAVES_PER_EU_WIDE))))
 void merge_small_kernel(SmallParams p) {
     extern __shared__ __align__(16) uint8_t lds_raw[];
     typedef SizeClass<CLS> C;
+    constexpr bool DIET = Diet<OPL, LISTS, CLS>::on;
     SmallLds L;
     small_carve((LDS uint8_t *)lds_raw, WAVE * OPL, C::NR, C::NO, C::ND, LISTS, true, &L);
     p.cap_regs = C::NR; p.cap_objs = C::NO; p.cap_deps = C::ND;
@@ -1558,7 +1566,7 @@
     uint2 w0, w1, w2;
     {
         const Rows r = load_rows<OPL>(p, doc);
-        stage_rows<OPL, LISTS>(p, L, doc, r, C::ND);
+        stage_rows<OPL, LISTS, DIET>(p, L, doc, r, C::ND);
         w0 = make_uint2(r.c01.x, r.c01.y); w1 = make_uint2(r.c01.z, r.c01.w); w2 = r.c2;
     }
     wave_sync();
@@ -1566,14 +1574,17 @@
 #if HM_KARG_RELOAD
         asm volatile("" : "+s"(kp));
         const SmallParams &p = *(const SmallParams *)kp;
+        if constexpr (DIET && HM_KARG_BATCH)
+            asm volatile("" :: "s"(p.n_docs), "s"(p.a_stride), "s"(p.general_only), "s"(p.docs), "s"(p.min_clock), "s"(p.doc_slot));
 #endif
         const uint32_t dn = d + gridDim.x;
         const bool more = dn < p.n_docs;
         bool dokn = true;
         hm_doc_row docn = {};
         static_assert(sizeof(hm_doc_row) == 12 * sizeof(uint32_t), "doc row words");
+        const uint32_t lane0 = lane_id<DIET>();
         uint32_t docw = 0;
-        if (more && threadIdx.x < 12) docw = reinterpret_cast<const uint32_t *>(p.docs + dn)[threadIdx.x];
+        if (more && lane0 < 12) docw = reinterpret_cast<const uint32_t *>(p.docs + dn)[lane0];
         auto take_docn = [&]() {
             uint32_t w[12];
 #pragma unroll
@@ -1596,24 +1607,33 @@
         DocState st;
         const uint32_t ds = hm_slot(p, d);
         uint32_t mc = 0;
-        if (p.min_clock && threadIdx.x < p.a_stride) mc = p.min_clock[(size_t)ds * p.a_stride + threadIdx.x];
+        if (p.min_clock && lane0 < p.a_stride) mc = (p.min_clock + (size_t)ds * p.a_stride)[lane0];
         if (p.min_clock && p.a_stride > WAVE) {
             uint32_t extra = 0;
             for (uint32_t a = WAVE + threadIdx.x; a < p.a_stride; a += WAVE) extra |= p.min_clock[(size_t)ds * p.a_stride + a];
             if (__ballot(extra != 0) && threadIdx.x == NA_MAX) mc |= 1u;
         }
-        const Outcome oc = !dok ? OUT_INVALID : in_env ? merge_doc_small<OPL, LISTS>(p, L, doc, w0, w1, w2, st) : OUT_UNSUPPORTED;
+        const Outcome oc = !dok ? OUT_INVALID : in_env ? merge_doc_small<OPL, LISTS, DIET>(p, L, doc, w0, w1, w2, st) : OUT_UNSUPPORTED;
         STAMP(L, 9);
-        uint32_t mcmp = oc == OUT_OK ? min_cmp_of(p, L, doc, mc) : 0u;
+        const uint32_t lane_io = lane_id<DIET>();
+        uint32_t mcmp = oc == OUT_OK ? min_cmp_of(p, L, doc, mc, lane_io) : 0u;
 #if HM_FENCE_MCMP
         asm volatile("" : "+s"(mcmp) :: "memory");
 #endif
+#if HM_ASYNC_NEXT
+        asm volatile("" : "+v"(docw));
+#endif
 #if !HM_PREFETCH_EARLY
         if (more) {
+#if HM_KARG_RELOAD
+            if constexpr (DIET && HM_KARG_BATCH)
+                asm volatile("" :: "s"(p.changes), "s"(p.deps), "s"(p.ops), "s"(p.a_stride), "s"(p.lim_changes), "s"(p.lim_deps),
+                             "s"(p.lim_ops), "s"(p.lim_regs));
+#endif
             take_docn();
             dokn = check_doc(p, docn);
 #if HM_ASYNC_NEXT
-            if constexpr (ASY) anext = load_rows_async<OPL>(p, docn);
+            if constexpr (ASY) anext = load_rows_async<OPL, LISTS>(p, docn, lane_io);
             else
 #endif
             next = load_rows<OPL>(p, docn);
@@ -1621,33 +1641,33 @@
 #endif
         STAMP(L, 12);
         if (HM_PRIO_IO) __builtin_amdgcn_s_setprio(HM_PRIO_IO);
-        const SurvRows<OPL> sv = surv_rows<OPL>(p, L, st);
+        const SurvRows<OPL> sv = surv_rows<OPL, LISTS>(p, L, st, lane_io);
 #if HM_STAGE_FIRST
         wave_sync();
-        if (more) stage_rows<OPL, LISTS>(p, L, docn, next, C::ND);
+        if (more) stage_rows<OPL, LISTS, DIET>(p, L, docn, next, C::ND);
         STAMP(L, 11);
-        write_outputs<OPL, LISTS>(p, L, d, ds, doc, oc, st, mcmp, sv);
+        write_outputs<OPL, LISTS, DIET>(p, L, d, ds, doc, oc, st, mcmp, sv, lane_io);
         if (HM_PRIO_IO) __builtin_amdgcn_s_setprio(0);
         wave_sync();
         STAMP(L, 10);
         if (!more) break;
 #else
-        write_outputs<OPL, LISTS>(p, L, d, ds, doc, oc, st, mcmp, sv);
+        write_outputs<OPL, LISTS, DIET>(p, L, d, ds, doc, oc, st, mcmp, sv, lane_io);
 #if HM_ASYNC_NEXT
-        if constexpr (ASY) { if (more && oc == OUT_OK) pad_stores<OPL>(p, doc, st, ds); }
+        if constexpr (ASY) { if (more) pad_stores<OPL>(p, doc, st, ds, oc == OUT_OK); }
 #endif
         wave_sync();
         STAMP(L, 10);
         if (!more) break;
 #if HM_ASYNC_NEXT
         if constexpr (ASY) {
-            next = take_rows_async<OPL>(anext, docn, oc == OUT_OK);
+            next = take_rows_async<OPL, DIET>(anext, docn);
 #if HM_ASYNC_CHECK
             async_check<OPL>(p, docn, next);
 #endif
         }
 #endif
-        stage_rows<OPL, LISTS>(p, L, docn, next, C::ND);
+        stage_rows<OPL, LISTS, DIET>(p, L, docn, next, C::ND);
         if (HM_PRIO_IO) __builtin_amdgcn_s_setprio(0);
         wave_sync();
         STAMP(L, 11);
diff --git a/hypermerge_amd/engine.py b/hypermerge_amd/engine.py
--- a/hypermerge_amd/engine.py
+++ b/hypermerge_amd/engine.py
@@ -23,7 +23,7 @@
            "hm_clock_allgather", "hm_clock_min_allreduce", "hm_comm_create_local", "hm_clock_exchange_host",
            "hm_clock_min_host", "hm_decode_blocks", "hm_decoded_batch", "hm_decoded_status", "hm_decoded_n_strings",
            "hm_decoded_string", "hm_decoded_actor", "hm_decoded_obj", "hm_decoded_reg", "hm_decoded_free",
-           "hm_store_set_incremental", "hm_store_last_routing", "hm_store_last_kernel_ms", "hm_store_inc_states", "hm_debug_async_check", "hm_doc_open_n", "hm_doc_reset", "hm_store_read_regs", "hm_store_read_history",
+           "hm_store_set_incremental", "hm_store_last_routing", "hm_store_last_kernel_ms", "hm_store_inc_states", "hm_debug_async_check", "hm_debug_small_occupancy", "hm_doc_open_n", "hm_doc_reset", "hm_store_read_regs", "hm_store_read_history",
            "hm_cursors_create", "hm_cursors_destroy", "hm_cursors_reserve", "hm_cursors_update", "hm_cursors_get",
            "hm_cursors_entry", "hm_cursors_docs_with_actors", "hm_docset_create", "hm_docset_destroy",
            "hm_docset_engine", "hm_docset_open", "hm_docset_apply", "hm_text_data", "hm_text_results", "hm_text_free",
@@ -88,7 +88,7 @@
             "hm_decoded_status": [vp], "hm_decoded_n_strings": [vp], "hm_decoded_string": [vp, u32, vp],
             "hm_decoded_actor": [vp, u32, u32, vp], "hm_decoded_free": [vp],
             "hm_decoded_obj": [vp, u32, u32, vp], "hm_decoded_reg": [vp, u32, u32, vp, vp],
-            "hm_store_set_incremental": [vp, ctypes.c_int], "hm_store_last_routing": [vp, vp], "hm_store_last_kernel_ms": [vp, vp], "hm_store_inc_states": [vp, vp], "hm_debug_async_check": [vp, ctypes.c_int],
+            "hm_store_set_incremental": [vp, ctypes.c_int], "hm_store_last_routing": [vp, vp], "hm_store_last_kernel_ms": [vp, vp], "hm_store_inc_states": [vp, vp], "hm_debug_async_check": [vp, ctypes.c_int], "hm_debug_small_occupancy": [vp, vp, vp],
             "hm_doc_open_n": [vp, u32, vp], "hm_doc_reset": [vp, vp, u32], "hm_store_read_regs": [vp, u32, vp, vp, vp, vp, u32, vp],
             "hm_store_read_history": [vp, u32, vp, vp, vp, vp, vp, vp],
             "hm_cursors_create": [vp, u32, vp], "hm_cursors_destroy": [vp], "hm_cursors_reserve": [vp, u32],
@@ -189,6 +189,12 @@
                                                    ctypes.c_void_p(out_ptr), ctypes.c_void_p(stream) if stream else None),
                     "hm_missing_deps_device")
 
+    def small_occupancy(self, batch: Batch) -> Sequence[int]:
+        out = (ctypes.c_uint32 * 6)()
+        cb = batch.c_struct()
+        self._check(self._L.hm_debug_small_occupancy(self._h, ctypes.byref(cb), out), "hm_debug_small_occupancy")
+        return tuple(int(x) for x in out)
+
     def last_kernel_ms(self) -> Sequence[float]:
         buf = (ctypes.c_float * 4)()
         n = self._L.hm_last_kernel_ms(self._h, buf, 4)
diff --git a/include/hypermerge_amd.h b/include/hypermerge_amd.h
--- a/include/hypermerge_amd.h
+++ b/include/hypermerge_amd.h
@@ -201,6 +201,7 @@
 int hm_store_inc_states(hm_store *s, uint32_t *out);
 
 int hm_debug_async_check(unsigned long long *out2, int reset);
+int hm_debug_small_occupancy(hm_engine *e, const hm_batch *host_batch, uint32_t *out6);
 
 typedef struct {
     uint32_t n_changes, n_deps, n_ops, n_regs, n_objs, n_actors;
```

Result: faster. 31.44 billion changes/s (median of 6 runs) (+7.3%).
